# kostas1515/iif

Measured on AMD Instinct MI355X. Metric: images/sec ResNet50+IIF ImageNet-LT bs=256/GPU, higher is better.
Workload: dtype bf16

## Files before the change

iif_amd/_lib.py:

```python
import ctypes
import os

import torch

_HERE = os.path.dirname(os.path.abspath(__file__))
LIB_PATH = os.environ.get("IIF_AMD_LIB") or os.path.join(_HERE, "csrc", "libiif_amd.so")

IIF_F32, IIF_BF16 = 0, 1
VARIANT_CODE = {"raw": 0, "smooth": 1, "rel": 2, "normit": 3, "gombit": 4, "base2": 5, "base10": 6}
_ERR = {-1: "IIF_EINVAL (bad argument)", -2: "IIF_EUNSUPPORTED (shape/alignment)", -3: "IIF_ELAUNCH (HIP error)"}

_c = ctypes
_P, _I, _L, _F = _c.c_void_p, _c.c_int, _c.c_int64, _c.c_float

SIGNATURES = {
    "iif_build_table": [_P, _I, _I, _I, _P],
    "iif_set_cu_budget": [_I],
    "iif_get_cu_budget": [],
    "iif_persistent_grid_blocks": [_I],
    "iif_ce_fwd_bwd": [_P, _I, _L, _P, _P, _P, _F, _P, _P, _L, _F, _I, _I, _P, _P, _P, _L, _P, _P, _P],
    "iif_sigmoid_focal_fwd_bwd": [_P, _I, _L, _P, _P, _F, _P, _F, _I, _F, _F, _I, _I, _P, _P, _P, _L, _P, _P, _P],
    "iif_scale_logits": [_P, _I, _L, _P, _I, _I, _P, _L, _P],
    "iif_softmax": [_P, _I, _L, _P, _I, _I, _P, _L, _P],
    "iif_topk_hits": [_P, _I, _L, _P, _P, _I, _I, _P, _I, _P, _P],
    "iif_eval_accumulate": [_P, _I, _L, _P, _P, _I, _I, _P, _I, _P, _I, _P, _P, _P, _P],
    "iif_scale_by_device_scalar": [_P, _I, _L, _P, _P, _P],
    "iif_mix_rows": [_P, _I, _P, _F, _I, _L, _P, _P],
    "iif_conv_igemm": [_P, _P, _P, _P, _P, _P, _P],
    "iif_conv_wgrad": [_P, _P, _P, _P, _P, _L, _I, _P],
    "iif_conv_wgrad_plan": [_P, _I, _L, _I, _P],
    "iif_conv_igemm_bnstats": [_P, _P, _P, _P, _P, _P, _P, _L, _P, _P],
    "iif_bn_finalize_stats": [_P, _I, _L, _I, _P, _P, _F, _F, _P, _P, _P, _P, _L, _P],
    "iif_bn_finalize_stats_fused": [_P, _I, _L, _I, _P, _P, _F, _F, _P, _P, _P, _P, _L, _P, _P],
    "iif_bn_finalize_stats_sums": [_P, _I, _L, _I, _P, _P, _F, _F, _P, _P, _P, _P, _L, _P, _P, _I, _I, _P, _P],
    "iif_bn_backward_partials_fused": [_P, _P, _P, _I, _L, _I, _P, _P, _P, _I, _P, _P, _P, _P, _L, _P, _P],
    "iif_bn_partial_sums": [_P, _I, _I, _P, _P],
    "iif_bn_stats_sums": [_P, _I, _L, _I, _P, _P, _L, _P],
    "iif_bn_backward_sums": [_P, _P, _P, _P, _I, _L, _I, _P, _P, _P, _L, _P],
    "iif_bn_backward_apply_sums": [_P, _P, _P, _P, _I, _L, _I, _P, _P, _P, _P, _c.c_double, _P, _P, _P, _P, _P, _P],
    "iif_bn_workspace_bytes": [_L, _I],
    "iif_bn_forward_stats": [_P, _I, _L, _I, _P, _P, _F, _F, _P, _P, _P, _P, _L, _P],
    "iif_bn_apply": [_P, _I, _L, _I, _P, _P, _P, _I, _P, _P, _P],
    "iif_bn_backward": [_P, _P, _P, _P, _I, _L, _I, _P, _P, _P, _P, _P, _P, _P, _L, _P],
    "iif_maxpool_forward": [_P, _I, _I, _I, _I, _I, _I, _I, _I, _P, _P, _P],
    "iif_maxpool_backward": [_P, _P, _I, _I, _I, _I, _I, _I, _I, _I, _P, _P],
    "iif_avgpool_forward": [_P, _I, _I, _I, _I, _P, _P],
    "iif_avgpool_backward": [_P, _I, _I, _I, _I, _P, _P],
    "iif_im2col_nchw": [_P, _I, _I, _I, _I, _I, _I, _I, _I, _I, _I, _P, _P],
    "iif_cast": [_P, _I, _P, _I, _L, _P],
    "iif_weight_transpose": [_P, _I, _I, _I, _I, _I, _I, _P, _P],
    "iif_shortcut_a_forward": [_P, _I, _I, _I, _I, _I, _I, _P, _P],
    "iif_shortcut_a_backward_acc": [_P, _I, _I, _I, _I, _I, _I, _P, _P],
    "iif_colsum_f32": [_P, _I, _I, _L, _P, _P],
    "iif_sgd_step": [_P, _P, _P, _L, _F, _P, _F, _F, _I, _F, _P],
    "iif_stream_plan": [_I, _L, _I, _I, _P],
    "iif_rmsprop_step": [_P, _P, _P, _P, _P, _L, _F, _P, _F, _F, _F, _F, _I, _F, _P],
    "iif_group_pack": [_P, _I, _I, _I, _I, _I, _I, _I, _I, _P, _P],
    "iif_group_pack_batched": [_P, _I, _I, _I, _P],
    "iif_wgrad1x1_stacked": [_P, _P, _P, _L, _I, _I, _I, _I, _P, _P, _L, _I, _P],
    "iif_group_unpack_grad": [_P, _I, _I, _I, _I, _I, _I, _P, _P],
    "iif_space_to_depth_nchw": [_P, _I, _I, _I, _I, _I, _I, _P, _P],
    "iif_stem_s2d_pack": [_P, _I, _I, _I, _I, _I, _I, _P, _P],
    "iif_stem_s2d_unpack_grad": [_P, _I, _I, _I, _I, _I, _P, _P],
    "iif_se_squeeze": [_P, _I, _I, _I, _I, _P, _P],
    "iif_se_apply": [_P, _I, _I, _I, _I, _P, _P, _P, _P, _P, _P, _P],
    "iif_se_backward_sums": [_P, _P, _P, _I, _I, _I, _I, _P, _P, _P],
    "iif_se_backward_form": [_P, _I, _I, _I, _I, _P, _P, _P, _P],
    "iif_se_excite_forward": [_P, _P, _I, _I, _I, _I, _P, _I, _P, _I, _P, _P, _P, _P],
    "iif_se_excite_backward": [_P, _P, _P, _I, _I, _I, _I, _P, _I, _P, _I, _P, _P, _P, _P, _P, _P, _P, _I, _P, _I, _P],
    "iif_rownorm_forward": [_P, _P, _I, _I, _L, _F, _F, _F, _P, _L, _P, _P],
    "iif_rownorm_backward": [_P, _P, _P, _P, _I, _I, _L, _L, _F, _F, _F, _P, _L, _P],
    "iif_weight_transpose_batched": [_P, _P, _I, _I, _I, _P, _P],
    "iif_conv_igemm_masked_res": [_P, _P, _P, _P, _P, _P, _P],
    "iif_conv_reload_env": [],
    "iif_conv_igemm_stats_only": [_P, _P, _P, _P, _L, _P, _P],
    "iif_conv_igemm_bn_relu": [_P, _P, _P, _P, _P, _P, _P, _P],
    "iif_conv_fwdbn_ok": [_P],
    "iif_conv_affine_ok": [_P, _I, _I],
    "iif_conv_affine_route": [_P, _I, _I, _I],
    "iif_conv_route": [_P, _c.c_uint, _I, _P, _I],
    "iif_conv_igemm_affine": [_P, _P, _P, _P, _P, _P, _P, _P, _P],
    "iif_bn_fold": [_P, _I, _F, _P],
    "iif_conv_igemm_stats_acc": [_P, _P, _P, _P, _L, _P, _P],
    "iif_conv_igemm_bn_relu2": [_P, _P, _P, _P, _P, _P, _P, _P, _P],
    "iif_conv_igemm_dgrad_masksum": [_P, _P, _P, _P, _P, _P, _P, _P, _P, _P, _L, _P, _P],
    "iif_conv_pro_ok": [_P, _I],
    "iif_conv_igemm_bnstats_pro": [_P, _P, _P, _P, _P, _P, _P, _P, _P, _L, _P, _P],
    "iif_conv_dgrad_rx_ok": [_P, _I],
    "iif_conv_igemm_dgrad_masksum_rx": [_P, _P, _P, _P, _P, _P, _P, _I, _P, _I, _P, _P, _P, _L, _P, _P],
    "iif_conv_dgrad_rx_pg_ok": [_P, _I],
    "iif_conv_igemm_dgrad_masksum_rx_pg": [_P, _P, _P, _P, _P, _P, _P, _I, _P, _I, _P, _P, _P, _L, _P, _P, _L, _I, _P, _P],
    "iif_slab_sum": [_P, _L, _I, _I, _I, _I, _P, _P],
    "iif_conv_igemm_dgrad2_bnbwd": [_P, _P, _P, _I, _P, _P, _P, _P, _P, _P, _P, _L, _P, _P],
    "iif_bn3_algebra_prep": [_P, _I, _P, _I, _P, _I, _P, _P, _I, _I, _L, _P, _P, _P, _P, _I, _P, _P, _L, _P, _P, _P],
    "iif_bn3_algebra_prep_scratch_floats": [_I, _I],
    "iif_bn3_algebra_dw": [_P, _I, _P, _I, _P, _I, _P, _P, _I, _I, _P, _I, _P],
    "iif_conv_pack_fragments": [_P, _P, _I, _I, _P, _P],
    "iif_conv_pack_fragments_g16": [_P, _P, _I, _I, _P, _P],
    "iif_conv3x3_frag_ok": [_P],
    "iif_mask_gather": [_P, _I, _P, _I, _I, _I, _P, _P, _P],
    "iif_mask_bce_fwd_bwd": [_P, _I, _P, _P, _I, _I, _I, _F, _P, _P, _P, _P, _P],
    "iif_class_accumulate": [_P, _P, _I, _I, _P, _P, _P],
    "iif_fasa_update": [_P, _P, _I, _I, _L, _I, _F, _P, _P, _P, _P],
    "iif_fasa_generate": [_P, _P, _P, _P, _P, _P, _I, _I, _P, _P, _P, _P, _P],
    "iif_fasa_update_rows": [_P, _P, _I, _I, _L, _I, _F, _P, _P, _P, _P, _P],
    "iif_fasa_generate_padded": [_P, _P, _P, _P, _P, _P, _I, _I, _I, _F, _P, _P, _P, _P, _P],
    "iif_head_loss_cums_fwd": [_P, _I, _L, _P, _P, _P, _P, _L, _F, _I, _I, _P, _L, _P, _P, _P, _P, _P, _P, _P, _P, _P],
    "iif_conv_igemm_dgrad_bnbwd": [_P, _P, _P, _P, _P, _P, _P, _P, _P, _P, _L, _P, _P],
    "iif_bn_backward_partials": [_P, _P, _P, _I, _L, _I, _P, _P, _P, _I, _P, _P, _P, _P, _L, _P],
    "iif_maxpool_bn_forward": [_P, _I, _P, _I, _I, _I, _I, _I, _I, _I, _P, _P, _P, _P],
    "iif_bn_backward_relu_recompute": [_P, _P, _I, _L, _I, _P, _P, _P, _P, _P, _P, _L, _P],
    "iif_bn_backward_relu_recompute_pooled": [_P, _P, _I, _L, _I, _P, _P, _P, _P, _P, _P, _L, _P, _P, _L, _P],
    "iif_bn_backward_pool_fused": [_P, _P, _P, _P, _I, _I, _I, _I, _I, _I, _I, _P, _P, _P, _P, _P, _P, _L, _P],
    "iif_rowmap_forward": [_P, _I, _I, _I, _L, _I, _F, _F, _P, _I, _L, _P, _P],
    "iif_rowmap_backward": [_P, _I, _P, _P, _I, _I, _I, _L, _L, _I, _F, _F, _P, _I, _L, _P],
    "iif_transpose_f32": [_P, _I, _I, _L, _P, _L, _P],
    "iif_dot_window_f32": [_P, _P, _I, _I, _L, _L, _F, _P, _P, _P],
    "iif_cifar_augment": [_P, _L, _P, _P, _L, _L, _c.c_uint64, _L, _L, _c.c_uint32, _P, _P, _P, _P, _P],
    "iif_lt_augment": [_P, _L, _P, _P, _L, _I, _P, _c.c_uint32, _P, _P],
    "iif_lt_augment_policy": [_P, _L, _P, _P, _L, _I, _P, _P, _P, _P],
    "iif_jpeg_decode": [_P, _L, _P, _L, _P, _L, _P, _L, _I, _P, _P],
    "iif_seesaw_fwd_bwd": [_P, _I, _L, _P, _P, _P, _I, _F, _F, _F, _F, _I, _F, _I, _I, _P, _P, _P, _P, _L, _P, _P, _P],
    "iif_seesaw_activation": [_P, _I, _L, _I, _I, _P, _L, _P],
    "iif_seesaw_accuracy": [_P, _I, _L, _P, _I, _I, _P, _P, _P],
    "iif_seesaw_scale_grad": [_P, _L, _I, _I, _P, _P, _I, _P, _L, _P],
    "iif_bce_det_fwd_bwd": [_P, _I, _L, _P, _P, _L, _P, _P, _P, _F, _I, _I, _P, _P, _P, _L, _P, _P],
    "iif_bbox_reg_fwd": [_P, _I, _L, _P, _I, _I, _P, _P, _F, _F, _L, _I, _P, _P, _P, _P, _P],
    "iif_bbox_reg_scatter_grad": [_P, _P, _I, _I, _I, _P, _P, _I, _L, _P],
    "iif_head_loss_fwd": [_P, _I, _L, _P, _P, _P, _P, _L, _F, _I, _I, _P, _L, _P, _P, _P, _P, _P, _P],
    "iif_head_loss_bwd": [_P, _I, _L, _P, _P, _F, _P, _P],
    "iif_head_bce_loss_fwd": [_P, _I, _L, _P, _P, _P, _L, _F, _I, _I, _P, _L, _P, _P, _P, _P, _P],
    "iif_seesaw_head_fwd": [_P, _I, _L, _P, _P, _P, _F, _F, _F, _F, _I, _I, _P, _L, _P, _P, _P, _P, _P, _P],
    "iif_seesaw_head_bwd": [_P, _L, _I, _I, _P, _P, _P, _F, _P, _L, _P],
    "iif_bbox_overlaps": [_P, _L, _L, _P, _L, _L, _I, _I, _F, _P, _P],
    "iif_max_iou_assign": [_P, _L, _L, _P, _L, _L, _P, _L, _L, _F, _F, _F, _F, _F, _I, _I, _I, _P, _P, _P, _P, _P, _L, _P],
    "iif_bbox2delta": [_P, _L, _P, _L, _L, _P, _P, _P, _P],
    "iif_delta2bbox": [_P, _L, _P, _L, _L, _I, _P, _P, _F, _I, _F, _I, _F, _F, _P, _P],
    "iif_random_sample": [_P, _P, _L, _L, _L, _c.c_double, _P, _P, _P, _P, _P, _L, _P],
    "iif_anchor_targets": [_P, _L, _L, _P, _P, _L, _P, _L, _L, _P, _P, _L, _F, _I, _P, _P, _P, _P, _P, _P, _P],
    "iif_roi_targets": [_P, _L, _L, _P, _P, _P, _L, _L, _P, _P, _P, _L, _L, _I, _L, _F, _I, _P, _P, _P, _P, _P, _P, _P, _P, _P],
    "iif_roi_stage_targets": [_P, _I, _P, _L, _L, _L, _P, _P, _L, _F, _F, _F, _F, _I, _I, _I, _L, _L, _c.c_double, _L, _F, _I, _P, _P,
                              _P, _P, _P, _P, _P, _P, _P, _P, _P, _P, _P, _P],
    "iif_refine_bboxes": [_P, _L, _P, _P, _L, _I, _I, _P, _P, _I, _L, _P, _P, _P, _F, _I, _F, _I, _P, _P, _P],
    "iif_grid_anchors": [_P, _P, _P],
    "iif_grid_valid_flags": [_P, _P, _P, _P],
    "iif_rpn_stage_workspace_bytes": [_I, _L, _L],
    "iif_rpn_stage_targets": [_P, _P, _I, _P, _I, _F, _P, _P, _F, _F, _F, _F, _I, _I, _L, _L, _c.c_double, _P, _P, _P, _P, _P, _P, _P,
                              _P, _P, _L, _P],
    "iif_rpn_stage_dense": [_P, _I, _P, _P, _P, _P, _L, _L, _L, _F, _P, _P, _P, _P, _P],
    "iif_rpn_loss_fwd": [_P, _P, _I, _P, _P, _P, _P, _L, _L, _P, _F, _F, _F, _F, _P, _P, _P],
    "iif_rpn_loss_bwd": [_P, _P, _I, _P, _P, _P, _P, _L, _L, _P, _F, _F, _F, _F, _P, _P, _P],
    "iif_rpn_sampled_pixels": [_P, _I, _P, _P, _P, _P, _L, _L, _P, _P, _P],
    "iif_rpn_head_sampled_workspace_bytes": [_I, _I, _I, _I],
    "iif_rpn_head_sampled_bwd": [_P, _P, _I, _I, _P, _P, _P, _P, _P, _P, _I, _I, _P, _P, _P, _P, _P, _P, _P, _L, _P],
    "iif_roi_extract_forward": [_P, _I, _I, _I, _P, _L, _L, _I, _I, _I, _I, _F, _F, _P, _I, _P, _P],
    "iif_roi_extract_backward": [_P, _I, _I, _I, _P, _L, _L, _I, _I, _I, _I, _F, _F, _P, _I, _P, _L, _P],
    "iif_mask_targets": [_P, _I, _P, _L, _P, _L, _I, _I, _I, _P, _P],
    "iif_paste_masks": [_P, _I, _I, _P, _P, _L, _L, _I, _I, _I, _I, _I, _F, _P, _P],
    "iif_rle_workspace_bytes": [_L, _I, _I],
    "iif_paste_rle_count": [_P, _I, _I, _P, _P, _L, _L, _I, _I, _I, _I, _I, _F, _P, _L, _P, _P],
    "iif_paste_rle_fill": [_P, _I, _I, _P, _P, _L, _L, _I, _I, _I, _I, _I, _F, _P, _L, _P, _L, _P, _P, _P],
    "iif_mask_rle_count": [_P, _L, _L, _L, _I, _I, _P, _L, _P, _P],
    "iif_mask_rle_fill": [_P, _L, _L, _L, _I, _I, _P, _L, _P, _L, _P, _P, _P],
    "iif_rle_to_string": [_P, _L, _P, _L, _P],
    "iif_mask_predict_fwd": [_P, _I, _P, _L, _P, _P, _P, _I, _I, _I, _I, _P, _P, _P, _P, _P, _P],
    "iif_mask_predict_bwd_input": [_P, _P, _P, _L, _P, _I, _I, _I, _I, _P, _I, _P],
    "iif_mask_predict_bwd_weight": [_P, _I, _P, _P, _P, _I, _I, _I, _I, _P, _P, _P, _P],
    "iif_mask_predict_loss_fwd": [_P, _I, _P, _L, _P, _P, _P, _I, _I, _I, _I, _I, _P, _P, _P, _P, _P],
    "iif_mask_predict_loss_bwd_input": [_P, _P, _P, _P, _L, _P, _I, _I, _I, _I, _P, _I, _P],
    "iif_mask_predict_loss_bwd_weight": [_P, _I, _P, _P, _P, _P, _I, _I, _I, _I, _P, _P, _P, _P],
    "iif_normed_mask_predict_fwd": [_P, _I, _P, _L, _P, _P, _P, _I, _I, _I, _I, _F, _F, _F, _I, _P, _P, _P, _P, _P, _P, _P, _P],
    "iif_normed_mask_predict_bwd_input": [_P, _I, _P, _P, _P, _P, _P, _P, _L, _P, _I, _I, _I, _I, _F, _F, _P, _P],
    "iif_normed_mask_predict_bwd_weight": [_P, _I, _P, _P, _P, _P, _P, _L, _P, _I, _I, _I, _I, _F, _F, _P, _P, _P, _P],
    "iif_mask_tail_fwd": [_P, _I, _P, _P, _P, _L, _P, _P, _P, _I, _I, _I, _I, _I, _I, _P, _P, _P, _P, _P, _P],
    "iif_mask_tail_bwd_rows": [_P, _I, _P, _P, _P, _P, _P, _I, _I, _I, _I, _I, _I, _P, _P, _P],
    "iif_mask_tail_bwd_input": [_P, _P, _P, _P, _L, _P, _P, _I, _I, _I, _I, _I, _I, _P, _I, _P],
    "iif_mask_tail_splits": [_I, _I, _I],
    "iif_mask_tail_bwd_params": [_P, _I, _P, _P, _P, _L, _P, _P, _I, _I, _I, _I, _I, _I, _P, _P, _P, _P],
    "iif_mask_tail_bwd_classes": [_P, _P, _I, _I, _I, _P, _P, _P],
    "iif_mask_tail_loss_fwd": [_P, _I, _P, _P, _P, _L, _P, _P, _P, _I, _I, _I, _I, _I, _I, _I, _P, _P, _P, _P, _P],
    "iif_mask_tail_loss_bwd_rows": [_P, _I, _P, _P, _P, _P, _P, _P, _I, _I, _I, _I, _I, _I, _P, _P, _P],
    "iif_mask_tail_loss_bwd_input": [_P, _P, _P, _P, _P, _L, _P, _P, _I, _I, _I, _I, _I, _I, _P, _I, _P],
    "iif_mask_tail_loss_bwd_params": [_P, _I, _P, _P, _P, _P, _L, _P, _P, _I, _I, _I, _I, _I, _I, _P, _P, _P, _P],
    "iif_nms": [_P, _L, _P, _P, _L, _I, _F, _I, _F, _L, _P, _P, _P, _P, _L, _P],
    "iif_rpn_proposals": [_P, _I, _I, _P, _I, _I, _F, _F, _I, _P, _P, _F, _I, _F, _I, _P, _P, _P, _P, _P, _P, _P, _P, _L, _P],
    "iif_multiclass_nms": [_P, _L, _I, _P, _L, _P, _P, _I, _L, _L, _F, _F, _I, _L, _L, _P, _P, _P, _P, _P, _P, _L, _P],
}



class ConvDesc(ctypes.Structure):
    _fields_ = [(k, ctypes.c_int32) for k in ("n", "hs", "ws", "cs", "hd", "wd", "cd", "r", "s", "stride", "pad",
                                               "transposed", "ldw", "dtype", "dst_dtype", "groups")] + [("wgt_frag", ctypes.c_void_p),
                                                                                                          ("wgt_frag_kind", ctypes.c_int32)]


class RoiLevel(ctypes.Structure):
    _fields_ = [("ptr", ctypes.c_void_p), ("H", ctypes.c_int32), ("W", ctypes.c_int32), ("spatial_scale", ctypes.c_float)]


class MaskImage(ctypes.Structure):
    _fields_ = [("ptr", ctypes.c_void_p), ("G", ctypes.c_int32), ("H", ctypes.c_int32), ("W", ctypes.c_int32),
                ("ld_row", ctypes.c_int64), ("ld_mask", ctypes.c_int64)]


class RoiImage(ctypes.Structure):
    _fields_ = [("gt_bboxes", ctypes.c_void_p), ("ld_gt", ctypes.c_int64), ("gt_labels", ctypes.c_void_p), ("G", ctypes.c_int32),
                ("img_index", ctypes.c_int32)]


def roi_images(gt_bboxes_list, gt_labels_list=None):
    B = len(gt_bboxes_list)
    images = (RoiImage * B)()
    held = []
    for b, g in enumerate(gt_bboxes_list):
        G = int(g.shape[0])
        g = g.detach()
        if G and (g.stride(1) != 1 or (G > 1 and g.stride(0) < 4)):
            g = g.contiguous()
        held.append(g)
        l = None
        if gt_labels_list is not None:
            l = gt_labels_list[b].reshape(-1).to(torch.int64).contiguous()
            held.append(l)
        images[b].gt_bboxes = ptr(g) if G else None
        images[b].ld_gt = g.stride(0) if G > 1 else 4
        images[b].gt_labels = ptr(l) if (G and l is not None) else None
        images[b].G = G
        images[b].img_index = b
    return images, held


class RpnGrid(ctypes.Structure):
    _fields_ = [("num_levels", ctypes.c_int32)] + [(k, ctypes.c_int32 * 8) for k in ("W", "H", "num_base", "stride_w", "stride_h")] + [
        ("base", ctypes.c_float * 4 * 16 * 8)]


class RpnLossLevel(ctypes.Structure):
    _fields_ = [(k, ctypes.c_void_p) for k in ("scores", "deltas", "grad_scores", "grad_deltas")] + [
        (k, ctypes.c_int64 * 4) for k in ("score_strides", "delta_strides", "grad_score_strides", "grad_delta_strides")]


class RpnHeadLevel(ctypes.Structure):
    _fields_ = [(k, ctypes.c_void_p) for k in ("feat", "grad_feat", "grad_scores", "grad_deltas")] + [
        (k, ctypes.c_int64 * 4) for k in ("feat_strides", "grad_feat_strides", "grad_score_strides", "grad_delta_strides")]


class RpnLevel(ctypes.Structure):
    _fields_ = [("scores", ctypes.c_void_p), ("deltas", ctypes.c_void_p), ("anchors", ctypes.c_void_p),
                ("score_strides", ctypes.c_int64 * 4), ("delta_strides", ctypes.c_int64 * 4), ("ld_anchors", ctypes.c_int64),
                ("A", ctypes.c_int32), ("H", ctypes.c_int32), ("W", ctypes.c_int32), ("reserved", ctypes.c_int32)]


class PackDesc(ctypes.Structure):
    _fields_ = [("src_off", ctypes.c_int64), ("dst_off", ctypes.c_int64)] + [(k, ctypes.c_int32) for k in (
        "rows", "taps", "k", "ld", "block_start", "reserved")]


_lib = None


class IIFNativeError(RuntimeError):
    pass


def lib():
    global _lib
    if _lib is None:
        if not os.path.exists(LIB_PATH):
            raise IIFNativeError(
                "libiif_amd.so not found at %s — build it with `python -c 'import __graft_entry__ as g; g.build()'` "
                "or `make -C iif_amd/csrc`; iif_amd has no CPU/PyTorch fallback." % LIB_PATH)
        l = ctypes.CDLL(LIB_PATH)
        l.iif_version.restype = _c.c_char_p
        l.iif_version.argtypes = []
        for name, argtypes in SIGNATURES.items():
            fn = getattr(l, name)
            fn.argtypes = argtypes
            fn.restype = _L if name in ("iif_bn_workspace_bytes", "iif_bn3_algebra_prep_scratch_floats", "iif_rle_workspace_bytes",
# ... 44 lines not shown
```

iif_amd/csrc/common.h:

```cpp
#pragma once
#include <hip/hip_runtime.h>
#include <stdint.h>
#include <type_traits>
#include "../../include/iif_amd.h"

#define IIF_WAVE 64

#define IIF_LAUNCH_CHECK()                          \
    do {                                            \
        hipError_t e__ = hipGetLastError();         \
        if (e__ != hipSuccess) return IIF_ELAUNCH;  \
    } while (0)

constexpr long long kDmaRange = 0x7f000000LL;

enum { IIF_ROUTE_NONE = 0, IIF_ROUTE_TILE = 1, IIF_ROUTE_TILE_2STAGE = 2, IIF_ROUTE_TILE_GENERAL = 3, IIF_ROUTE_TILE256 = 4,
       IIF_ROUTE_HALO = 5, IIF_ROUTE_FRAG = 6, IIF_ROUTE_FRAG_G16 = 7, IIF_ROUTE_STREAM1X1 = 8, IIF_ROUTE_REGW1X1 = 9,
       IIF_ROUTE_REGW3X3 = 10, IIF_ROUTE_REGSTAGE = 11, IIF_ROUTE_STEM = 12, IIF_ROUTE_TILE_MC = 13 };

typedef __attribute__((ext_vector_type(4))) float f32x4;
typedef __attribute__((ext_vector_type(4))) unsigned int u32x4;
typedef __attribute__((ext_vector_type(2))) unsigned int u32x2;
typedef __attribute__((ext_vector_type(8))) short s16x8;
typedef __attribute__((ext_vector_type(8))) __bf16 bf16x8;
// ... 13 lines not shown
__device__ __forceinline__ float wave_max(float v) {
#pragma unroll
    for (int o = 32; o > 0; o >>= 1) v = fmaxf(v, __shfl_xor(v, o, 64));
    return v;
}
__device__ __forceinline__ float wave_sum(float v) {
#pragma unroll
    for (int o = 32; o > 0; o >>= 1) v += __shfl_xor(v, o, 64);
    return v;
}
__device__ __forceinline__ int wave_sum_i(int v) {
#pragma unroll
    for (int o = 32; o > 0; o >>= 1) v += __shfl_xor(v, o, 64);
    return v;
}

static inline hipStream_t as_stream(void* s) { return (hipStream_t)s; }
static inline int64_t cdiv64(int64_t a, int64_t b) { return (a + b - 1) / b; }
static inline bool aligned(const void* p, int a) { return (reinterpret_cast<uintptr_t>(p) % a) == 0; }
static inline bool aligned_to(const void* p, unsigned n) { return aligned(p, (int)n); }


struct ConvCall {
    const iif_conv_desc* d; const void* src; const void* wgt; void* dst; const void* res; const unsigned char* res_bits; const float* bias;
    float* bn_partial; int64_t bn_cap; int32_t* n_partials; void* stream;
    const void* bw_x; const unsigned char* bw_bits; const float* bw_stats;
    int mask_store; const void* src2; int cs2; const float* sbias; int no_store;
    const float* aff; const float* aff2; unsigned char* relu_out;
    int aff_any;
    const void* rx_src2; const void* rx_w3; int rx_k2, rx_ldw3;
    const float* pro_stats; void* pro_out; unsigned char* pro_bits; float* pro_csum;
    float* pg_slab; long long pg_cap; int pg_ld; int* pg_count;
};

struct ConvSel {
    int N, Hs, Ws, Cs, Hd, Wd, Cd, R, S, sshift, pad, transposed, ldw, M, groups, spitch, dpitch, Cs2, esz;
    bool outf32;
    long long src_bytes, wgt_bytes;
    bool res, res_bits, bias, bn_partial, bw_x, bw_bits, bw_stats, src2, sbias, aff, aff2, relu_out, rx_src2, rx_w3, pro_stats, pg_slab,
         pg_count, wfrag;
    bool res_is_dst, pg_unaligned;
    int mask_store, no_store, wfrag_kind, rx_k2, rx_ldw3, pg_ld, bn_row0;
    long long bn_cap, pg_cap;
    int ntaps, in_shift, scatter;
};

struct ConvRoute {
    int family;
    int inst;
    int cls;
    int mtiles, ntiles;
    unsigned grid, grid_y, block;
    int rows, slabs;
};

inline int iif_claim_rows(const ConvSel& a, ConvRoute* r, int rows) {
    r->rows = 0;
    if (!a.bn_partial) return IIF_OK;
    if ((long long)(a.bn_row0 + rows) * 2 * a.dpitch > a.bn_cap) return IIF_EINVAL;
    r->rows = rows;
    return IIF_OK;
}


bool iif_stem4x4_geometry(const ConvSel& a);
int iif_stem4x4_select(const ConvSel& a, ConvRoute* r);
int iif_stem4x4_launch(const ConvRoute& r, const ConvCall& c, const ConvSel& a, hipStream_t st);

enum { IIF_REGW_PLAIN = 0, IIF_REGW_FWDBN = 2, IIF_REGW_STATS = 3 };
bool iif_dense1x1(const ConvSel& a);
bool iif_regw1x1_ok(int M, int K, int N, int epi);
bool iif_regw1x1_rx_ok(int M, int K, int N, int k2);
bool iif_regw1x1_pg_ok(int M, int K, int N, int k2);
bool iif_regw1x1_pro_ok(int M, int K, int N);
bool iif_regw1x1_fwdbn_ok(int M, int K, int N);
int iif_regw1x1_select(const ConvSel& a, int mode, ConvRoute* r);
int iif_regw1x1_launch(const ConvRoute& r, const ConvCall& c, const ConvSel& a, hipStream_t st);
int iif_regw3x3_select(const ConvSel& a, ConvRoute* r);
int iif_regw3x3_launch(const ConvRoute& r, const ConvCall& c, const ConvSel& a, const signed char* tap_dy, const signed char* tap_dx,
                       const unsigned char* tap_w, hipStream_t st);

struct ConvSwitches {
    bool no_stream, force_stream, regstage, no_v2, no_halo, force_halo, v2_force, no_regw, no_regw_fwdbn, no_bm256_2src,
         regw_k512_cw16, regw_no_x2, regw_k512_no_epi;
    static ConvSwitches read();
};
extern ConvSwitches g_sw;

int iif_persistent_cus();
int iif_persistent_grid(int unit);
```

iif_amd/csrc/conv_igemm.hip:

```cpp
#include <stdlib.h>

#include "common.h"
#ifndef IIF_CONV_AUX_SRC
#define IIF_CONV_AUX_SRC 0
#endif

namespace {

template <typename T> struct ET;
template <> struct ET<unsigned short> { static constexpr int PE = 8, KE = 32; };
template <> struct ET<float> { static constexpr int PE = 4, KE = 16; };

struct ConvArgs {
    const unsigned char* src; const unsigned char* wgt; unsigned char* dst; const unsigned char* res;
    const unsigned char* wfrag;
    int wfrag_kind;
    const float* bias;
    const unsigned char* res_bits;
    const unsigned char* bw_x; const unsigned char* bw_bits; const float* bw_stats;
    int mask_store;
    const unsigned char* src2; int Cs2;
    const float* sbias;
    const unsigned char* rx_src2; const unsigned char* rx_w3; int rx_k2, rx_ldw3;
    float* pg_slab; long long pg_cap; int pg_ld; int* pg_count;
// ... 1853 lines not shown
    if (d->n <= 0 || d->hs <= 0 || d->ws <= 0 || d->cs <= 0 || d->hd <= 0 || d->wd <= 0 || d->cd <= 0 ||
        d->r <= 0 || d->s <= 0 || d->pad < 0)
        return IIF_EINVAL;
    if (d->stride != 1 && d->stride != 2) return IIF_EUNSUPPORTED;
    if (d->dtype != IIF_F32 && d->dtype != IIF_BF16) return IIF_EINVAL;
    if (d->dst_dtype != d->dtype && d->dst_dtype != IIF_F32) return IIF_EINVAL;
    const int pe = d->dtype == IIF_F32 ? 4 : 8;
    if (d->cs % pe != 0 || d->ldw % pe != 0 || d->ldw < d->r * d->s * d->cs + (a->src2 ? a->Cs2 : 0)) return IIF_EUNSUPPORTED;
    const bool bf16 = d->dtype == IIF_BF16 && d->dst_dtype == IIF_BF16;
    if (aff_any) {
        if (!affine_geometry_ok(d) || a->bias || a->bn_partial || a->res_bits || a->bw_x) return IIF_EUNSUPPORTED;
    } else if (a->src2 || a->sbias || a->mask_store || a->no_store || a->aff || a->pro_stats) {
        if (!bf16 || d->r != 1 || d->s != 1 || d->stride != 1 || d->pad != 0 || d->groups > 1 || (d->cd % 8) || a->bias || (d->cs % 32))
            return IIF_EUNSUPPORTED;
        if (a->src2 && ((a->Cs2 % 32) || a->Cs2 <= 0 || src2_unaligned)) return IIF_EUNSUPPORTED;
        if (a->mask_store && (!a->bw_bits || !a->bn_partial)) return IIF_EINVAL;
        if (a->no_store && (!a->bn_partial || a->res || a->bw_x)) return IIF_EINVAL;
        if (a->aff && (a->bn_partial || a->res_bits || a->bw_x || a->no_store)) return IIF_EINVAL;
    }
    if (unaligned) return IIF_EUNSUPPORTED;
    if ((int64_t)d->n * d->hd * d->wd > 0x7fffff00LL || (int64_t)d->n * d->hs * d->ws > 0x7fffff00LL) return IIF_EUNSUPPORTED;
    sel_geometry(d, a);
    if (a->bn_partial && !(bf16 && (d->cd % 8) == 0 && !a->bias && (a->bw_x || a->mask_store || !a->res) && !g_sw.regstage &&
                           a->src_bytes < kDmaRange))
        return IIF_EUNSUPPORTED;
    if (a->groups > 65535) return IIF_EUNSUPPORTED;
    return select_conv(*a, p);
}

ConvSel sel_of(const ConvCall& c) {
    ConvSel a{};
    a.res = c.res; a.res_bits = c.res_bits; a.bias = c.bias; a.bn_partial = c.bn_partial;
    a.bw_x = c.bn_partial && c.bw_x; a.bw_bits = c.bn_partial && c.bw_bits; a.bw_stats = c.bn_partial && c.bw_stats;
    a.src2 = c.src2; a.sbias = c.sbias; a.aff = c.aff; a.aff2 = c.aff2; a.relu_out = c.relu_out;
    a.rx_src2 = c.rx_src2; a.rx_w3 = c.rx_w3; a.pro_stats = c.pro_stats; a.pg_slab = c.pg_slab; a.pg_count = c.pg_count;
    a.res_is_dst = c.res == c.dst; a.pg_unaligned = reinterpret_cast<uintptr_t>(c.pg_slab) & 15;
    a.mask_store = c.mask_store; a.no_store = c.no_store; a.Cs2 = c.cs2; a.rx_k2 = c.rx_k2; a.rx_ldw3 = c.rx_ldw3; a.pg_ld = c.pg_ld;
    a.bn_cap = c.bn_cap; a.pg_cap = c.pg_cap;
    return a;
}

int conv_entry(const ConvCall& c) {
    const iif_conv_desc* d = c.d;
    if (!d || !c.src || !c.wgt || !c.dst) return IIF_EINVAL;
    if (c.n_partials) *c.n_partials = 0;
    if (c.pg_count) *c.pg_count = 0;
    ConvSel s = sel_of(c);
    ConvPlan p;
    const bool unaligned = (reinterpret_cast<uintptr_t>(c.src) | reinterpret_cast<uintptr_t>(c.wgt) | reinterpret_cast<uintptr_t>(c.dst) |
                            reinterpret_cast<uintptr_t>(c.res)) & 15;
    if (const int rc = conv_select(d, &s, unaligned, reinterpret_cast<uintptr_t>(c.src2) & 15, c.aff_any, &p)) return rc;
    hipStream_t st = as_stream(c.stream);
    for (int i = 0; i < p.n; ++i) {
        const ConvRoute& r = p.r[i];
        const int rc = d->dtype == IIF_BF16 ? (s.outf32 ? launch_route<unsigned short, true>(c, s, r, st)
                                                        : launch_route<unsigned short, false>(c, s, r, st))
                                            : launch_route<float, true>(c, s, r, st);
        if (rc != IIF_OK) return rc;
        s.bn_row0 += r.rows;
        if (c.n_partials) *c.n_partials = s.bn_row0;
        if (c.pg_count) *c.pg_count = r.slabs;
    }
    return IIF_OK;
}

}

ConvSwitches g_sw = ConvSwitches::read();
ConvSwitches ConvSwitches::read() {
    ConvSwitches c;
    c.no_stream = getenv("IIF_CONV_NO_STREAM1X1") != nullptr;
    c.force_stream = getenv("IIF_CONV_STREAM1X1_FORCE") != nullptr;
    c.regstage = getenv("IIF_CONV_REGSTAGE") != nullptr;
    c.no_v2 = getenv("IIF_CONV_NO_V2") != nullptr;
    c.no_halo = getenv("IIF_CONV_NO_HALO") != nullptr;
    c.v2_force = getenv("IIF_CONV_V2_FORCE") != nullptr;
    c.force_halo = getenv("IIF_CONV_HALO_FORCE") != nullptr;
    c.no_regw = getenv("IIF_CONV_NO_REGW") != nullptr;
    c.no_regw_fwdbn = getenv("IIF_CONV_NO_REGW_FWDBN") != nullptr;
    c.no_bm256_2src = getenv("IIF_CONV_NO_BM256_2SRC") != nullptr;
    c.regw_k512_cw16 = getenv("IIF_REGW_K512_CW16") != nullptr;
    c.regw_no_x2 = getenv("IIF_REGW_NO_X2") != nullptr;
    c.regw_k512_no_epi = getenv("IIF_REGW_K512_NO_EPI") != nullptr;
    return c;
}

extern "C" int iif_conv_pack_fragments(const void* src_base, const iif_pack_desc* table, int n_desc, int total_blocks,
                                       void* dst_base, void* stream) {
    if (!src_base || !table || !dst_base || n_desc <= 0 || total_blocks <= 0) return IIF_EINVAL;
    if ((reinterpret_cast<uintptr_t>(src_base) | reinterpret_cast<uintptr_t>(dst_base)) & 15) return IIF_EUNSUPPORTED;
    hipLaunchKernelGGL(pack_fragments_kernel, dim3((unsigned)total_blocks), dim3(256), 0, as_stream(stream),
                       (const unsigned short*)src_base, table, n_desc, (unsigned short*)dst_base);
    IIF_LAUNCH_CHECK();
    return IIF_OK;
}

extern "C" int iif_conv_pack_fragments_g16(const void* src_base, const iif_pack_desc* table, int n_desc, int total_blocks,
                                           void* dst_base, void* stream) {
    if (!src_base || !table || !dst_base || n_desc <= 0 || total_blocks <= 0) return IIF_EINVAL;
    if ((reinterpret_cast<uintptr_t>(src_base) | reinterpret_cast<uintptr_t>(dst_base)) & 15) return IIF_EUNSUPPORTED;
    hipLaunchKernelGGL(pack_fragments_g16_kernel, dim3((unsigned)total_blocks), dim3(256), 0, as_stream(stream),
                       (const unsigned short*)src_base, table, n_desc, (unsigned short*)dst_base);
    IIF_LAUNCH_CHECK();
    return IIF_OK;
}

extern "C" int iif_conv_reload_env(void) {
    g_sw = ConvSwitches::read();
    return IIF_OK;
}

namespace {
bool query_dense1x1(const iif_conv_desc* d, int transposed, ConvSel* a) {
    if (!d || d->dtype != IIF_BF16 || d->dst_dtype != IIF_BF16) return false;
    *a = ConvSel{};
    sel_geometry(d, a);
    return iif_dense1x1(*a) && a->transposed == transposed;
}
}

extern "C" int iif_conv3x3_frag_ok(const iif_conv_desc* d) {
    if (!d || g_sw.no_v2 || g_sw.regstage) return 0;
    if (d->dtype != IIF_BF16 || d->dst_dtype != IIF_BF16 || d->r != 3 || d->s != 3 || d->stride != 1 || d->pad != 1) return 0;
    if (d->hs != d->hd || d->ws != d->wd) return 0;
    const int g = d->groups > 1 ? d->groups : 1;
    if (g > 1 && (d->cs != 64 || d->cd != 64)) return 0;
    if ((int64_t)d->n * d->hs * d->ws * d->cs * g * 2 >= kDmaRange) return 0;
    return v2_geometry_ok(d->n, d->hd, d->wd, d->cs, d->cd, g) ? 1 : 0;
}

extern "C" int iif_conv_dgrad_rx_ok(const iif_conv_desc* d, int c2) {
    ConvSel a;
    return query_dense1x1(d, 1, &a) && iif_regw1x1_rx_ok(a.M, a.Cs, a.Cd, c2) ? 1 : 0;
}

extern "C" int iif_conv_dgrad_rx_pg_ok(const iif_conv_desc* d, int c2) {
    ConvSel a;
    return query_dense1x1(d, 1, &a) && iif_regw1x1_pg_ok(a.M, a.Cs, a.Cd, c2) ? 1 : 0;
}

extern "C" int iif_conv_fwdbn_ok(const iif_conv_desc* d) {
    ConvSel a;
    return query_dense1x1(d, 0, &a) && !g_sw.no_regw_fwdbn && iif_regw1x1_fwdbn_ok(a.M, a.Cs, a.Cd) ? 1 : 0;
}

extern "C" int iif_conv_pro_ok(const iif_conv_desc* d, int stats_only) {
    ConvSel a;
    if (!query_dense1x1(d, 0, &a)) return 0;
    return (stats_only ? (!g_sw.no_regw_fwdbn && iif_regw1x1_fwdbn_ok(a.M, a.Cs, a.Cd)) : iif_regw1x1_pro_ok(a.M, a.Cs, a.Cd)) ? 1 : 0;
}

extern "C" int iif_conv_affine_ok(const iif_conv_desc* d, int has_res, int has_res_affine) {
    if (has_res_affine && !has_res) return 0;
    return affine_geometry_ok(d) ? 1 : 0;
}

extern "C" int iif_conv_affine_route(const iif_conv_desc* d, int has_res, int has_res_affine, int has_relu_bits) {
    if (!iif_conv_affine_ok(d, has_res, has_res_affine)) return IIF_ROUTE_NONE;
    ConvSel a{};
    a.aff = true; a.res = has_res; a.aff2 = has_res_affine; a.relu_out = has_relu_bits;
    ConvPlan p;
    return conv_select(d, &a, false, false, 1, &p) == IIF_OK ? p.r[0].family : IIF_ROUTE_NONE;
}

extern "C" int iif_conv_route(const iif_conv_desc* d, unsigned operands, int cs2, int32_t* out, int cap) {
    if (!d || cap < 0 || (cap > 0 && !out)) return IIF_EINVAL;
// ... 201 lines not shown
```

iif_amd/csrc/conv_wgrad.hip:

```cpp
#include <stdlib.h>
#include <type_traits>

#include "common.h"
#include "wgrad_plan.h"
#ifndef IIF_WG_AUX_X
#define IIF_WG_AUX_X 0
#endif
#ifndef IIF_WG_AUX_Y
#define IIF_WG_AUX_Y 0
#endif

namespace {

struct WgArgs {
    const unsigned char* x; const unsigned char* dy; float* out;
    int N, Hs, Ws, Cs, Hd, Wd, Cd, R, S, sshift, pad, ldw, M, K;
    int ktiles, ntiles, steps_per_split, nsteps, nsplits;
    int xpitch, ypitch, groups;
    int64_t slab;
};

template <typename T> struct WT;
template <> struct WT<unsigned short> {
    static constexpr int PE = 8, ROWS = 32;
// ... 139 lines not shown
                const unsigned char* base = Y + (4 * g + q) * PY + (wk * (BC / 2) + kj * 16 + 4 * p) * 2;
                yp[kj].lo = tr_read(base); yp[kj].hi = tr_read(base + 16 * PY);
            }
            tr_fence<0>();
#pragma unroll
            for (int ni = 0; ni < 4; ++ni) xf[ni] = tr_join(xp[ni]);
#pragma unroll
            for (int kj = 0; kj < KJ; ++kj) yf[kj] = tr_join(yp[kj]);
#pragma unroll
            for (int ni = 0; ni < 4; ++ni)
#pragma unroll
                for (int kj = 0; kj < KJ; ++kj)
                    acc[ni][kj] = __builtin_amdgcn_mfma_f32_16x16x32_bf16(
                        __builtin_bit_cast(bf16x8, xf[ni]), __builtin_bit_cast(bf16x8, yf[kj]), acc[ni][kj], 0, 0, 0);
        } else {
#pragma unroll
            for (int qq = 0; qq < 4; ++qq) {
                float xf[4], yf[KJ];
#pragma unroll
                for (int ni = 0; ni < 4; ++ni)
                    xf[ni] = *reinterpret_cast<const float*>(X + (4 * qq + g) * PX + (wn * 64 + ni * 16 + li) * 4);
#pragma unroll
                for (int kj = 0; kj < KJ; ++kj)
                    yf[kj] = *reinterpret_cast<const float*>(Y + (4 * qq + g) * PY + (wk * (BC / 2) + kj * 16 + li) * 4);
#pragma unroll
                for (int ni = 0; ni < 4; ++ni)
#pragma unroll
                    for (int kj = 0; kj < KJ; ++kj)
                        acc[ni][kj] = __builtin_amdgcn_mfma_f32_16x16x4f32(xf[ni], yf[kj], acc[ni][kj], 0, 0, 0);
            }
        }
        if (more) store_step((step + 1 - step0) & 1);
        __syncthreads();
    }

    float* out = a.out + (int64_t)split * a.slab;
#pragma unroll
    for (int kj = 0; kj < KJ; ++kj) {
        const int k = k0 + wk * (BC / 2) + kj * 16 + li;
        if (k >= a.Cd) continue;
#pragma unroll
        for (int ni = 0; ni < 4; ++ni) {
            const int n = n0 + wn * 64 + ni * 16 + g * 4;
            if (n >= a.K) continue;
            *reinterpret_cast<f32x4*>(out + (int64_t)k * a.ldw + n) = acc[ni][kj];
        }
    }
}

typedef __attribute__((address_space(3))) void lds_void_w;

#ifdef IIF_CONV_STAMPS
__device__ unsigned long long* g_wstamps = nullptr;
#define IIF_WSTAMP(var)                                                                            \
    do {                                                                                           \
        __builtin_amdgcn_sched_barrier(0);                                                         \
        asm volatile("s_memtime %0\n\ts_waitcnt lgkmcnt(0)" : "=s"(var)::"memory");               \
        __builtin_amdgcn_sched_barrier(0);                                                         \
    } while (0)
#endif

template <typename T, int COLS> struct Swz {
    static constexpr int RB = COLS * (int)sizeof(T);
    static __device__ __forceinline__ int logical(int p, int row) {
        if constexpr (sizeof(T) == 2) {
            const int key = RB >= 256 ? (row & 7) : ((row >> 1) & 3);
            return (((p >> 1) ^ key) << 1) | (p & 1);
        } else {
            return (((p >> 2) ^ (row & 1)) << 2) | (p & 3);
        }
    }
    static __device__ __forceinline__ int addr(int row, int colb) {
        if constexpr (sizeof(T) == 2) {
            const int key = RB >= 256 ? (row & 7) : ((row >> 1) & 3);
            return row * RB + ((((colb >> 5) ^ key)) << 5) + (colb & 31);
        } else {
            return row * RB + ((((colb >> 6) ^ (row & 1))) << 6) + (colb & 63);
        }
    }
};

template <int N> __device__ __forceinline__ void wait_vmcnt() { asm volatile("s_waitcnt vmcnt(%0)" ::"n"(N) : "memory"); }

template <typename T, int BC, int WK = 2, int NST = 3>
__global__ void __launch_bounds__(128 * WK) conv_wgrad_dma_kernel(WgArgs a, unsigned x_bytes, unsigned dy_bytes) {
    constexpr int PE = WT<T>::PE, ROWS = WT<T>::ROWS;
    constexpr int BNW = 128;
    constexpr int NWV = 2 * WK;
    constexpr int CW = BC / WK;
    using SX = Swz<T, BNW>;
    using SY = Swz<T, BC>;
    constexpr int XB = ROWS * SX::RB, YB = ROWS * SY::RB, STAGE = XB + YB;
    constexpr int LPRX = SX::RB / 16, RPIX = 64 / LPRX, NIX = ROWS / RPIX / NWV;
    constexpr int LPRY = SY::RB / 16, RPIY = 64 / LPRY, NIY = ROWS / RPIY / NWV;
    constexpr int LPS = NIX + NIY;
    constexpr int KJ = CW / 16;
    constexpr unsigned OOB = 0xfffffff0u;
    static_assert((NIX == 1 || NIX == 2) && (NIY == 1 || NIY == 2), "tile geometry");
    static_assert(NST >= 3 && NST <= 7 && (NST - 2) * LPS <= 63, "ring depth");
    __shared__ __attribute__((aligned(1024))) unsigned char smem[NST * STAGE];

    const int tid = threadIdx.x, lane = tid & 63;
    const int wave = __builtin_amdgcn_readfirstlane(tid >> 6);
    const int wn = wave / WK, wk = wave % WK;
    const int tiles = a.ktiles * a.ntiles;
    const int xcd = blockIdx.x & 7, jj = blockIdx.x >> 3;
    const int split = (jj / tiles) * 8 + xcd, tile = jj % tiles;
    if (split >= a.nsplits) return;
    const int kt = tile % a.ktiles, ntile = tile / a.ktiles;
    const int k0 = kt * BC, n0 = ntile * BNW;
    const int step0 = split * a.steps_per_split;
    int step1 = step0 + a.steps_per_split;
    if (step1 > a.nsteps) step1 = a.nsteps;

    const auto rs_x = __builtin_amdgcn_make_buffer_rsrc(const_cast<unsigned char*>(a.x), 0, x_bytes, 0x00020000);
    const auto rs_y = __builtin_amdgcn_make_buffer_rsrc(const_cast<unsigned char*>(a.dy), 0, dy_bytes, 0x00020000);
    const int grp = blockIdx.y;
    const unsigned gx = (unsigned)(grp * a.Cs) * (unsigned)sizeof(T), gy = (unsigned)(grp * a.Cd) * (unsigned)sizeof(T);

    int xr[NIX], py[NIX], px[NIX], pb[NIX], pm[NIX], ttr[NIX], tts[NIX], tch[NIX];
    bool nval[NIX];
    const int HW = a.Hd * a.Wd, HWs = a.Hs * a.Ws;
#pragma unroll
    for (int i = 0; i < NIX; ++i) {
        xr[i] = RPIX * (NIX * wave + i) + lane / LPRX;
        const int lc = SX::logical(lane % LPRX, xr[i]);
        const int ncol = n0 + lc * PE;
        nval[i] = ncol < a.K;
        const int tap = ncol / a.Cs;
        tch[i] = ncol - tap * a.Cs;
        ttr[i] = tap / a.S; tts[i] = tap - ttr[i] * a.S;
        const int m = step0 * ROWS + xr[i];
        pm[i] = m;
        const int n = m / HW, rem = m - n * HW;
        py[i] = rem / a.Wd; px[i] = rem - py[i] * a.Wd; pb[i] = n * HWs;
    }
    int yr[NIY];
    unsigned ycol[NIY];
#pragma unroll
    for (int i = 0; i < NIY; ++i) {
        yr[i] = RPIY * (NIY * wave + i) + lane / LPRY;
        const int lc = SY::logical(lane % LPRY, yr[i]);
        const int kcol = k0 + lc * PE;
        ycol[i] = kcol < a.Cd ? (unsigned)kcol * (unsigned)sizeof(T) : OOB;
    }

    auto issue = [&](int stage, int step) {
        unsigned char* X = smem + stage * STAGE;
        unsigned char* Y = X + XB;
#pragma unroll
        for (int i = 0; i < NIX; ++i) {
            const int ys = (py[i] << a.sshift) - a.pad + ttr[i], xs = (px[i] << a.sshift) - a.pad + tts[i];
            const bool ok = nval[i] && pm[i] < a.M && (unsigned)ys < (unsigned)a.Hs && (unsigned)xs < (unsigned)a.Ws;
            const unsigned off = ok ? ((unsigned)(pb[i] + ys * a.Ws + xs) * (unsigned)a.xpitch + (unsigned)tch[i]) * (unsigned)sizeof(T) + gx : OOB;
            __builtin_amdgcn_raw_ptr_buffer_load_lds(rs_x, (lds_void_w*)(X + (NIX * wave + i) * 1024), 16, off, 0, 0, IIF_WG_AUX_X);
        }
#pragma unroll
        for (int i = 0; i < NIY; ++i) {
            const int m = step * ROWS + yr[i];
            const unsigned off = (ycol[i] != OOB && m < a.M) ? (unsigned)m * (unsigned)a.ypitch * (unsigned)sizeof(T) + ycol[i] + gy : OOB;
            __builtin_amdgcn_raw_ptr_buffer_load_lds(rs_y, (lds_void_w*)(Y + (NIY * wave + i) * 1024), 16, off, 0, 0, IIF_WG_AUX_Y);
        }
    };
    auto advance = [&]() {
#pragma unroll
        for (int i = 0; i < NIX; ++i) {
            pm[i] += ROWS;
            px[i] += ROWS;
            while (px[i] >= a.Wd) {
                px[i] -= a.Wd;
                if (++py[i] == a.Hd) { py[i] = 0; pb[i] += HWs; }
            }
        }
    };

    f32x4 acc[4][KJ];
#pragma unroll
    for (int ni = 0; ni < 4; ++ni)
#pragma unroll
        for (int kj = 0; kj < KJ; ++kj) acc[ni][kj] = f32x4{0.f, 0.f, 0.f, 0.f};

    const int g = lane >> 4, li = lane & 15;
    const int nst = step1 - step0;
#pragma unroll
    for (int s_ = 0; s_ < NST - 1; ++s_)
        if (s_ < nst) {
            if (s_ > 0) advance();
            issue(s_, step0 + s_);
        }
    int stage = 0;
#ifdef IIF_CONV_STAMPS
    unsigned long long w_wait = 0, w_issue = 0, w_rest = 0, w0, w1, w2, w3, wb;
    IIF_WSTAMP(wb); w3 = wb;
#endif
    for (int t = 0; t < nst; ++t) {
#ifdef IIF_CONV_STAMPS
        IIF_WSTAMP(w0); w_rest += w0 - w3;
#endif
        {
            const int rem = nst - 1 - t;
            if (rem >= NST - 2) wait_vmcnt<(NST - 2) * LPS>();
            else if (NST > 3 && rem == 1) wait_vmcnt<LPS>();
            else if (NST > 4 && rem == 2) wait_vmcnt<2 * LPS>();
            else if (NST > 5 && rem == 3) wait_vmcnt<3 * LPS>();
            else if (NST > 6 && rem == 4) wait_vmcnt<4 * LPS>();
            else wait_vmcnt<0>();
        }
        __builtin_amdgcn_s_barrier();
#ifdef IIF_CONV_STAMPS
        IIF_WSTAMP(w1);
#endif
        if (t + NST - 1 < nst) { advance(); issue(stage == 0 ? NST - 1 : stage - 1, step0 + t + NST - 1); }
#ifdef IIF_CONV_STAMPS
        IIF_WSTAMP(w2); w_wait += w1 - w0; w_issue += w2 - w1; w3 = w2;
#endif
        const unsigned char* X = smem + stage * STAGE;
        const unsigned char* Y = X + XB;
        if constexpr (sizeof(T) == 2) {
            const int q = li >> 2, p = li & 3;
            TrPair xp[4], yp[KJ];
            s16x8 yf[KJ];
#pragma unroll
            for (int kj = 0; kj < KJ; ++kj) {
                const int colb = (wk * CW + kj * 16 + 4 * p) * 2;
                yp[kj].lo = tr_read(Y + SY::addr(4 * g + q, colb)); yp[kj].hi = tr_read(Y + SY::addr(16 + 4 * g + q, colb));
            }
#pragma unroll
            for (int ni = 0; ni < 4; ++ni) {
                const int colb = (wn * 64 + ni * 16 + 4 * p) * 2;
                xp[ni].lo = tr_read(X + SX::addr(4 * g + q, colb)); xp[ni].hi = tr_read(X + SX::addr(16 + 4 * g + q, colb));
            }
#pragma unroll
            for (int ni = 0; ni < 4; ++ni) {
                if (ni == 0) tr_fence<6>(); else if (ni == 1) tr_fence<4>(); else if (ni == 2) tr_fence<2>(); else tr_fence<0>();
                if (ni == 0) {
#pragma unroll
                    for (int kj = 0; kj < KJ; ++kj) yf[kj] = tr_join(yp[kj]);
                }
                const s16x8 xf = tr_join(xp[ni]);
#pragma unroll
                for (int kj = 0; kj < KJ; ++kj)
                    acc[ni][kj] = __builtin_amdgcn_mfma_f32_16x16x32_bf16(
                        __builtin_bit_cast(bf16x8, xf), __builtin_bit_cast(bf16x8, yf[kj]), acc[ni][kj], 0, 0, 0);
            }
        } else {
#pragma unroll
            for (int qq = 0; qq < 4; ++qq) {
                float xf[4], yf[KJ];
#pragma unroll
                for (int ni = 0; ni < 4; ++ni)
                    xf[ni] = *reinterpret_cast<const float*>(X + SX::addr(4 * qq + g, (wn * 64 + ni * 16 + li) * 4));
#pragma unroll
                for (int kj = 0; kj < KJ; ++kj)
                    yf[kj] = *reinterpret_cast<const float*>(Y + SY::addr(4 * qq + g, (wk * CW + kj * 16 + li) * 4));
#pragma unroll
                for (int ni = 0; ni < 4; ++ni)
#pragma unroll
                    for (int kj = 0; kj < KJ; ++kj)
                        acc[ni][kj] = __builtin_amdgcn_mfma_f32_16x16x4f32(xf[ni], yf[kj], acc[ni][kj], 0, 0, 0);
            }
        }
        stage = stage == NST - 1 ? 0 : stage + 1;
    }

#ifdef IIF_CONV_STAMPS
    IIF_WSTAMP(w0); w_rest += w0 - w3;
    if (g_wstamps && blockIdx.x < 512 && lane == 0 && wave < 4) {
        unsigned long long* o = g_wstamps + ((int64_t)blockIdx.x * 4 + wave) * 8;
        o[0] = w_wait; o[1] = 0; o[2] = w_issue; o[3] = w_rest; o[4] = 0; o[5] = w0 - wb; o[6] = (unsigned long long)nst; o[7] = wb;
    }
#endif
    float* out = a.out + (int64_t)split * a.slab + (int64_t)grp * a.Cd * a.ldw;
#pragma unroll
    for (int kj = 0; kj < KJ; ++kj) {
        const int k = k0 + wk * CW + kj * 16 + li;
        if (k >= a.Cd) continue;
#pragma unroll
        for (int ni = 0; ni < 4; ++ni) {
            const int n = n0 + wn * 64 + ni * 16 + g * 4;
            if (n >= a.K) continue;
            *reinterpret_cast<f32x4*>(out + (int64_t)k * a.ldw + n) = acc[ni][kj];
        }
    }
}

struct W1Args {
    const unsigned char* x; const unsigned char* dy; float* out;
    int M, Cs, Cd, ldw, ktiles, ntiles, steps_per_split, nsteps, nsplits;
    int64_t slab;
    const unsigned char* dy2; int Cd1, Cd2;
};

template <int OFF> __device__ __forceinline__ s16x4 tr_read_at(unsigned a) {
    s16x4 v;
    asm volatile("ds_read_b64_tr_b16 %0, %1 offset:%2" : "=v"(v) : "v"(a), "n"(OFF) : "memory");
    return v;
}

template <int BC, int BNW, int NWV>
__device__ __forceinline__ void wgrad1x1_body(const W1Args& a, unsigned x_bytes, unsigned dy_bytes) {
    constexpr int NWN = BNW / 64, WK = NWV / NWN, CW = BC / WK, KJ = CW / 16;
    using SX = Swz<unsigned short, BNW>;
    using SY = Swz<unsigned short, BC>;
    constexpr int RBX = SX::RB, RBY = SY::RB;
    constexpr int XB = 32 * RBX, YB = 32 * RBY, STAGE = XB + YB;
    constexpr int NPX = XB / 1024, NPY = YB / 1024;
    constexpr bool YPAD = NPY < NWV;
    constexpr int NIX = NPX / NWV, NIY = YPAD ? 1 : NPY / NWV, LPS = NIX + NIY;
    constexpr int LPRX = RBX / 16, RPIX = 64 / LPRX, LPRY = RBY / 16, RPIY = 64 / LPRY;
    constexpr unsigned OOB = 0xfffffff0u;
    static_assert(NIX >= 1 && NIY >= 1 && NIX * NWV == NPX && (YPAD || NIY * NWV == NPY) && KJ >= 1, "tile geometry");
    static_assert(2 * STAGE + 16 * RBY < 65536 && 2 * STAGE + 16 * RBX < 65536, "fragment reads use 16-bit immediates");
    __shared__ __attribute__((aligned(1024))) unsigned char smem[3 * STAGE + (YPAD ? 1024 : 0)];

    const int tid = threadIdx.x, lane = tid & 63;
    const int wave = __builtin_amdgcn_readfirstlane(tid >> 6);
    const int wn = wave / WK, wk = wave % WK;
    const int tiles = a.ktiles * a.ntiles;
    const int xcd = blockIdx.x & 7, jj = blockIdx.x >> 3;
    const int split = (jj / tiles) * 8 + xcd, tile = jj % tiles;
    if (split >= a.nsplits) return;
    const int k0 = (tile % a.ktiles) * BC, n0 = (tile / a.ktiles) * BNW;
    const int step0 = split * a.steps_per_split;
    int step1 = step0 + a.steps_per_split;
    if (step1 > a.nsteps) step1 = a.nsteps;
    const int nst = step1 - step0;

    const auto rs_x = __builtin_amdgcn_make_buffer_rsrc(const_cast<unsigned char*>(a.x), 0, x_bytes, 0x00020000);
    const bool second = a.dy2 != nullptr && k0 >= a.Cd1;
    const int ycols = a.dy2 == nullptr ? a.Cd : (second ? a.Cd2 : a.Cd1);
    const int yk0 = second ? k0 - a.Cd1 : k0;
    const auto rs_y = __builtin_amdgcn_make_buffer_rsrc(const_cast<unsigned char*>(second ? a.dy2 : a.dy), 0,
                                                        second ? (unsigned)a.M * (unsigned)a.Cd2 * 2u : dy_bytes, 0x00020000);

    unsigned offx[NIX], incx[NIX], offy[NIY], incy[NIY];
#pragma unroll
    for (int i = 0; i < NIX; ++i) {
        const int r = RPIX * (NIX * wave + i) + lane / LPRX;
        const int col = n0 + SX::logical(lane % LPRX, r) * 8;
        const bool ok = col < a.Cs;
        offx[i] = ok ? ((unsigned)(step0 * 32 + r) * (unsigned)a.Cs + (unsigned)col) * 2u : OOB;
        incx[i] = ok ? 64u * (unsigned)a.Cs : 0u;
    }
#pragma unroll
    for (int i = 0; i < NIY; ++i) {
        const int r = RPIY * (NIY * wave + i) + lane / LPRY;
        const int col = yk0 + SY::logical(lane % LPRY, r) * 8;
        const bool ok = col < ycols && (!YPAD || wave < NPY);
        offy[i] = ok ? ((unsigned)(step0 * 32 + r) * (unsigned)ycols + (unsigned)col) * 2u : OOB;
        incy[i] = ok ? 64u * (unsigned)ycols : 0u;
    }
    auto issue = [&](auto stage_c) {
        constexpr int S = decltype(stage_c)::value;
#pragma unroll
        for (int i = 0; i < NIX; ++i) {
            __builtin_amdgcn_raw_ptr_buffer_load_lds(rs_x, (lds_void_w*)(smem + S * STAGE + (NIX * wave + i) * 1024), 16, offx[i], 0, 0, IIF_WG_AUX_X);
            offx[i] += incx[i];
        }
#pragma unroll
        for (int i = 0; i < NIY; ++i) {
            unsigned char* dst = smem + S * STAGE + XB + (NIY * wave + i) * 1024;
            if (YPAD && wave >= NPY) dst = smem + 3 * STAGE;
            __builtin_amdgcn_raw_ptr_buffer_load_lds(rs_y, (lds_void_w*)dst, 16, offy[i], 0, 0, IIF_WG_AUX_Y);
            offy[i] += incy[i];
        }
    };

    const int g = lane >> 4, li = lane & 15, q = li >> 2, pp = li & 3;
    unsigned xo[4], yo[KJ];
    const unsigned sbase = (unsigned)(unsigned long long)(lds_cu8*)smem;
#pragma unroll
    for (int ni = 0; ni < 4; ++ni) xo[ni] = sbase + (unsigned)SX::addr(4 * g + q, (wn * 64 + ni * 16 + 4 * pp) * 2);
#pragma unroll
    for (int kj = 0; kj < KJ; ++kj) yo[kj] = sbase + (unsigned)(XB + SY::addr(4 * g + q, (wk * CW + kj * 16 + 4 * pp) * 2));

    f32x4 acc[4][KJ];
#pragma unroll
    for (int ni = 0; ni < 4; ++ni)
#pragma unroll
        for (int kj = 0; kj < KJ; ++kj) acc[ni][kj] = f32x4{0.f, 0.f, 0.f, 0.f};

    using S0 = std::integral_constant<int, 0>;
    using S1 = std::integral_constant<int, 1>;
    using S2 = std::integral_constant<int, 2>;
    auto step = [&](auto stage_c, auto refill_c, int t) {
        constexpr int S = decltype(stage_c)::value;
        if (t + 1 < nst) wait_vmcnt<LPS>(); else wait_vmcnt<0>();
        __builtin_amdgcn_s_barrier();
        if (t + 2 < nst) issue(refill_c);
        TrPair xp[4], yp[KJ];
        s16x8 yf[KJ];
#pragma unroll
        for (int kj = 0; kj < KJ; ++kj) {
            yp[kj].lo = tr_read_at<S * STAGE>(yo[kj]); yp[kj].hi = tr_read_at<S * STAGE + 16 * RBY>(yo[kj]);
        }
#pragma unroll
        for (int ni = 0; ni < 4; ++ni) {
            xp[ni].lo = tr_read_at<S * STAGE>(xo[ni]); xp[ni].hi = tr_read_at<S * STAGE + 16 * RBX>(xo[ni]);
        }
#pragma unroll
        for (int ni = 0; ni < 4; ++ni) {
            if (ni == 0) tr_fence<6>(); else if (ni == 1) tr_fence<4>(); else if (ni == 2) tr_fence<2>(); else tr_fence<0>();
            if (ni == 0) {
#pragma unroll
                for (int kj = 0; kj < KJ; ++kj) yf[kj] = tr_join(yp[kj]);
            }
            const s16x8 xf = tr_join(xp[ni]);
#pragma unroll
            for (int kj = 0; kj < KJ; ++kj)
                acc[ni][kj] = __builtin_amdgcn_mfma_f32_16x16x32_bf16(__builtin_bit_cast(bf16x8, xf), __builtin_bit_cast(bf16x8, yf[kj]),
                                                                      acc[ni][kj], 0, 0, 0);
        }
    };
    if (nst > 0) issue(S0{});
    if (nst > 1) issue(S1{});
    for (int t = 0; t < nst; t += 3) {
        step(S0{}, S2{}, t);
        if (t + 1 < nst) step(S1{}, S0{}, t + 1);
        if (t + 2 < nst) step(S2{}, S1{}, t + 2);
    }

    float* out = a.out + (int64_t)split * a.slab;
#pragma unroll
    for (int kj = 0; kj < KJ; ++kj) {
        const int k = k0 + wk * CW + kj * 16 + li;
        if (k >= a.Cd) continue;
#pragma unroll
        for (int ni = 0; ni < 4; ++ni) {
            const int n = n0 + wn * 64 + ni * 16 + g * 4;
            if (n >= a.Cs) continue;
            *reinterpret_cast<f32x4*>(out + (int64_t)k * a.ldw + n) = acc[ni][kj];
        }
    }
}

__global__ void __launch_bounds__(512) wgrad1x1_256x128_kernel(W1Args a, unsigned xb, unsigned yb) { wgrad1x1_body<256, 128, 8>(a, xb, yb); }
__global__ void __launch_bounds__(256) wgrad1x1_128x128_kernel(W1Args a, unsigned xb, unsigned yb) { wgrad1x1_body<128, 128, 4>(a, xb, yb); }
__global__ void __launch_bounds__(256) wgrad1x1_64x128_kernel(W1Args a, unsigned xb, unsigned yb) { wgrad1x1_body<64, 128, 4>(a, xb, yb); }
__global__ void __launch_bounds__(256) wgrad1x1_64x64_kernel(W1Args a, unsigned xb, unsigned yb) { wgrad1x1_body<64, 64, 4>(a, xb, yb); }
__global__ void __launch_bounds__(512) wgrad1x1_64x256_kernel(W1Args a, unsigned xb, unsigned yb) { wgrad1x1_body<64, 256, 8>(a, xb, yb); }

struct WgHaloArgs {
    const unsigned char* x; const unsigned char* dy; float* out;
    int N, H, W, Cs, Cd, ldw;
    int ci_tiles, co_tiles, steps_per_split, nsteps, nsplits, HB;
    int grouped;
    int64_t slab;
};

template <int XB, int YB, int D>
__global__ void __launch_bounds__(256) conv3x3_wgrad_halo_kernel(WgHaloArgs a, unsigned x_bytes, unsigned dy_bytes) {
    constexpr int RB = 128;
    constexpr int XR = 32 * XB, YR = 32 * YB;
    constexpr unsigned OOB = 0xfffffff0u;
    using SW = Swz<unsigned short, 64>;
    __shared__ __attribute__((aligned(1024))) unsigned char smem[(XR + YR) * RB];
    unsigned char* const XS = smem;
    unsigned char* const YS = smem + XR * RB;

    const int tid = threadIdx.x, lane = tid & 63;
    const int wave = __builtin_amdgcn_readfirstlane(tid >> 6);
    const int tiles = a.ci_tiles * a.co_tiles;
    const int xcd = blockIdx.x & 7, jj = blockIdx.x >> 3;
    const int split = (jj / tiles) * 8 + xcd, tile = jj % tiles;
    if (split >= a.nsplits) return;
    const int ci0 = a.grouped ? tile * 64 : (tile % a.ci_tiles) * 64, co0 = a.grouped ? tile * 64 : (tile / a.ci_tiles) * 64;
    const int step0 = split * a.steps_per_split;
    int step1 = step0 + a.steps_per_split;
    if (step1 > a.nsteps) step1 = a.nsteps;
    const int nst = step1 - step0;
    const int Wp = a.W + 2, PV = (a.H + 2) * Wp, HW = a.H * a.W;
    const int V0 = step0 * 32, LEAD = a.HB >> 4;

    const auto rs_x = __builtin_amdgcn_make_buffer_rsrc(const_cast<unsigned char*>(a.x), 0, x_bytes, 0x00020000);
    const auto rs_y = __builtin_amdgcn_make_buffer_rsrc(const_cast<unsigned char*>(a.dy), 0, dy_bytes, 0x00020000);

    const int lrow = 8 * wave + (lane >> 3);
    struct Cur { int n, yp, xp; };
    auto start = [&](int v) {
        Cur c; const int t = v + PV; c.n = t / PV - 1; const int rem = t - (c.n + 1) * PV; c.yp = rem / Wp; c.xp = rem - c.yp * Wp;
        return c;
    };
    auto advance = [&](Cur& c) {
        c.xp += 32;
        while (c.xp >= Wp) { c.xp -= Wp; if (++c.yp == a.H + 2) { c.yp = 0; ++c.n; } }
    };
    Cur cx = start(V0 - a.HB + lrow), cy = start(V0 + lrow);
    int xblk = 0, yblk = 0;
    auto issue_x = [&]() {
        const int prow = (xblk * 32 + lrow) & (XR - 1);
        const int lc = SW::logical(lane & 7, prow);
        const bool ok = (unsigned)cx.n < (unsigned)a.N && (unsigned)(cx.yp - 1) < (unsigned)a.H && (unsigned)(cx.xp - 1) < (unsigned)a.W;
        const unsigned off = ok ? ((unsigned)(cx.n * HW + (cx.yp - 1) * a.W + cx.xp - 1) * (unsigned)a.Cs + (unsigned)(ci0 + lc * 8)) * 2u : OOB;
        __builtin_amdgcn_raw_ptr_buffer_load_lds(rs_x, (lds_void_w*)(XS + ((xblk * 32 + 8 * wave) & (XR - 1)) * RB), 16, off, 0, 0, IIF_WG_AUX_X);
        advance(cx); ++xblk;
    };
    auto issue_y = [&]() {
        const int prow = (yblk * 32 + lrow) & (YR - 1);
        const int lc = SW::logical(lane & 7, prow);
        const bool ok = (unsigned)cy.n < (unsigned)a.N && (unsigned)(cy.yp - 1) < (unsigned)a.H && (unsigned)(cy.xp - 1) < (unsigned)a.W;
        const unsigned off = ok ? ((unsigned)(cy.n * HW + (cy.yp - 1) * a.W + cy.xp - 1) * (unsigned)a.Cd + (unsigned)(co0 + lc * 8)) * 2u : OOB;
        __builtin_amdgcn_raw_ptr_buffer_load_lds(rs_y, (lds_void_w*)(YS + ((yblk * 32 + 8 * wave) & (YR - 1)) * RB), 16, off, 0, 0, IIF_WG_AUX_Y);
        advance(cy); ++yblk;
    };

    f32x4 acc[9][4];
#pragma unroll
    for (int t = 0; t < 9; ++t)
#pragma unroll
        for (int kj = 0; kj < 4; ++kj) acc[t][kj] = f32x4{0.f, 0.f, 0.f, 0.f};

    for (int j = 0; j < LEAD; ++j) issue_x();
#pragma unroll
    for (int j = 0; j < D; ++j) { issue_x(); issue_y(); }

    const int g = lane >> 4, li = lane & 15, q = li >> 2, p = li & 3;
    int xo[9], yo[4];
#pragma unroll
    for (int tap = 0; tap < 9; ++tap)
        xo[tap] = SW::addr((a.HB + 4 * g + q + (tap / 3 - 1) * Wp + (tap % 3 - 1)) & (XR - 1), (16 * wave + 4 * p) * 2);
#pragma unroll
    for (int kj = 0; kj < 4; ++kj) yo[kj] = SW::addr(4 * g + q, (16 * kj + 4 * p) * 2);
#ifdef IIF_CONV_STAMPS
    unsigned long long w_wait = 0, w_issue = 0, w_rest = 0, w0, w1, w2, w3, wb;
    IIF_WSTAMP(wb); w3 = wb;
#endif
    for (int t = 0; t < nst; ++t) {
#ifdef IIF_CONV_STAMPS
        IIF_WSTAMP(w0); w_rest += w0 - w3;
#endif
        asm volatile("s_waitcnt vmcnt(%0)" ::"n"(2 * (D - 1)) : "memory");
        __builtin_amdgcn_s_barrier();
#ifdef IIF_CONV_STAMPS
        IIF_WSTAMP(w1);
#endif
        issue_x(); issue_y();
#ifdef IIF_CONV_STAMPS
        IIF_WSTAMP(w2); w_wait += w1 - w0; w_issue += w2 - w1; w3 = w2;
#endif
        const int xs = t * (32 * RB), ys = t * (32 * RB);
        TrPair yp[4], xp[9];
        s16x8 yf[4];
#pragma unroll
        for (int kj = 0; kj < 4; ++kj) {
            yp[kj].lo = tr_read(YS + ((yo[kj] + ys) & (YR * RB - 1))); yp[kj].hi = tr_read(YS + ((yo[kj] + ys + 16 * RB) & (YR * RB - 1)));
        }
#pragma unroll
        for (int tap = 0; tap < 9; ++tap) {
            xp[tap].lo = tr_read(XS + ((xo[tap] + xs) & (XR * RB - 1))); xp[tap].hi = tr_read(XS + ((xo[tap] + xs + 16 * RB) & (XR * RB - 1)));
        }
#pragma unroll
        for (int tap = 0; tap < 9; ++tap) {
            if (tap == 0) tr_fence<15>(); else if (tap == 1) tr_fence<14>(); else if (tap == 2) tr_fence<12>();
            else if (tap == 3) tr_fence<10>(); else if (tap == 4) tr_fence<8>(); else if (tap == 5) tr_fence<6>();
            else if (tap == 6) tr_fence<4>(); else if (tap == 7) tr_fence<2>(); else tr_fence<0>();
            if (tap == 0) {
#pragma unroll
                for (int kj = 0; kj < 4; ++kj) yf[kj] = tr_join(yp[kj]);
            }
            const s16x8 xf = tr_join(xp[tap]);
#pragma unroll
            for (int kj = 0; kj < 4; ++kj)
                acc[tap][kj] = __builtin_amdgcn_mfma_f32_16x16x32_bf16(__builtin_bit_cast(bf16x8, xf), __builtin_bit_cast(bf16x8, yf[kj]),
                                                                        acc[tap][kj], 0, 0, 0);
        }
    }
    asm volatile("s_waitcnt vmcnt(0)" ::: "memory");
#ifdef IIF_CONV_STAMPS
    IIF_WSTAMP(w0); w_rest += w0 - w3;
    if (g_wstamps && blockIdx.x < 512 && lane == 0 && wave < 4) {
        unsigned long long* o = g_wstamps + ((int64_t)blockIdx.x * 4 + wave) * 8;
        o[0] = w_wait; o[1] = 0; o[2] = w_issue; o[3] = w_rest; o[4] = 0; o[5] = w0 - wb; o[6] = (unsigned long long)nst; o[7] = wb;
    }
#endif

    float* out = a.out + (int64_t)split * a.slab;
#pragma unroll
    for (int kj = 0; kj < 4; ++kj) {
        const int k = co0 + kj * 16 + li;
#pragma unroll
        for (int tap = 0; tap < 9; ++tap) {
            const int n = a.grouped ? tap * 64 + wave * 16 + g * 4 : tap * a.Cs + ci0 + wave * 16 + g * 4;
            *reinterpret_cast<f32x4*>(out + (int64_t)k * a.ldw + n) = acc[tap][kj];
        }
    }
}

struct WgStemArgs {
    const unsigned char* x; const unsigned char* dy; float* out;
    int N, H, W, ldw, steps_per_split, nsteps, nsplits, LB, LEAD;
    int64_t slab;
};

__global__ void __launch_bounds__(256) conv4x4_s2d_wgrad_kernel(WgStemArgs a, unsigned x_bytes, unsigned dy_bytes) {
    constexpr int XRB = 32, YRB = 128;
    constexpr int XR = 512, YR = 128;
    constexpr int D = 2;
    constexpr unsigned OOB = 0xfffffff0u;
    using SW = Swz<unsigned short, 64>;
    __shared__ __attribute__((aligned(1024))) unsigned char smem[XR * XRB + YR * YRB];
    unsigned char* const XS = smem;
    unsigned char* const YS = smem + XR * XRB;

    const int tid = threadIdx.x, lane = tid & 63;
    const int wave = __builtin_amdgcn_readfirstlane(tid >> 6);
    const int xcd = blockIdx.x & 7, jj = blockIdx.x >> 3;
    const int split = jj * 8 + xcd;
    if (split >= a.nsplits) return;
    const int step0 = split * a.steps_per_split;
    int step1 = step0 + a.steps_per_split;
    if (step1 > a.nsteps) step1 = a.nsteps;
    const int nst = step1 - step0;
    const int Wp = a.W + 3, Hp = a.H + 3, PV = Hp * Wp, HW = a.H * a.W;
    const int V0 = step0 * 32;

    const auto rs_x = __builtin_amdgcn_make_buffer_rsrc(const_cast<unsigned char*>(a.x), 0, x_bytes, 0x00020000);
    const auto rs_y = __builtin_amdgcn_make_buffer_rsrc(const_cast<unsigned char*>(a.dy), 0, dy_bytes, 0x00020000);

    struct Cur { int n, yp, xp; };
    auto start = [&](int v) {
        const int t = v + 32 * PV;
        Cur c; c.n = t / PV - 32; const int rem = t - (c.n + 32) * PV; c.yp = rem / Wp; c.xp = rem - c.yp * Wp;
        return c;
    };
    auto advance = [&](Cur& c) {
        c.xp += 32;
        while (c.xp >= Wp) { c.xp -= Wp; if (++c.yp == Hp) { c.yp = 0; ++c.n; } }
    };
    const int xrow = lane >> 1, yrow = 8 * wave + (lane >> 3);
    Cur cx = start(V0 - 32 * a.LB + xrow), cy = start(V0 + yrow);
    int xblk = 0, yblk = 0;
    auto issue_x = [&]() {
        const bool ok = (unsigned)cx.n < (unsigned)a.N && (unsigned)(cx.yp - 2) < (unsigned)a.H && (unsigned)(cx.xp - 2) < (unsigned)a.W;
        const unsigned off = ok ? ((unsigned)(cx.n * HW + (cx.yp - 2) * a.W + cx.xp - 2) * 16u + (unsigned)((lane & 1) * 8)) * 2u : OOB;
        __builtin_amdgcn_raw_ptr_buffer_load_lds(rs_x, (lds_void_w*)(XS + ((xblk * 32) & (XR - 1)) * XRB), 16, off, 0, 0, IIF_WG_AUX_X);
        advance(cx); ++xblk;
    };
    auto issue_y = [&]() {
        const int prow = (yblk * 32 + yrow) & (YR - 1);
        const int lc = SW::logical(lane & 7, prow);
        const bool ok = (unsigned)cy.n < (unsigned)a.N && (unsigned)(cy.yp - 2) < (unsigned)a.H && (unsigned)(cy.xp - 2) < (unsigned)a.W;
        const unsigned off = ok ? ((unsigned)(cy.n * HW + (cy.yp - 2) * a.W + cy.xp - 2) * 64u + (unsigned)(lc * 8)) * 2u : OOB;
        __builtin_amdgcn_raw_ptr_buffer_load_lds(rs_y, (lds_void_w*)(YS + ((yblk * 32 + 8 * wave) & (YR - 1)) * YRB), 16, off, 0, 0, IIF_WG_AUX_Y);
        advance(cy); ++yblk;
    };

    f32x4 acc[4][4];
#pragma unroll
    for (int t = 0; t < 4; ++t)
#pragma unroll
        for (int kj = 0; kj < 4; ++kj) acc[t][kj] = f32x4{0.f, 0.f, 0.f, 0.f};

    if (wave == 0) for (int j = 0; j < a.LEAD; ++j) issue_x();
#pragma unroll
    for (int j = 0; j < D; ++j) { if (wave == 0) issue_x(); issue_y(); }

    const int g = lane >> 4, li = lane & 15, q = li >> 2, p = li & 3;
    int xo[4], yo[4];
#pragma unroll
    for (int s_ = 0; s_ < 4; ++s_)
        xo[s_] = ((32 * a.LB + 4 * g + q + (wave - 2) * Wp + (s_ - 2)) & (XR - 1)) * XRB + 4 * p * 2;
#pragma unroll
    for (int kj = 0; kj < 4; ++kj) yo[kj] = SW::addr(4 * g + q, (16 * kj + 4 * p) * 2);
    for (int t = 0; t < nst; ++t) {
        if (wave == 0) asm volatile("s_waitcnt vmcnt(%0)" ::"n"(2 * (D - 1)) : "memory");
        else asm volatile("s_waitcnt vmcnt(%0)" ::"n"(D - 1) : "memory");
        __builtin_amdgcn_s_barrier();
        if (wave == 0) issue_x();
        issue_y();
        const int xs = t * (32 * XRB), ys = t * (32 * YRB);
        TrPair yp[4], xp[4];
        s16x8 yf[4];
#pragma unroll
        for (int kj = 0; kj < 4; ++kj) {
            yp[kj].lo = tr_read(YS + ((yo[kj] + ys) & (YR * YRB - 1))); yp[kj].hi = tr_read(YS + ((yo[kj] + ys + 16 * YRB) & (YR * YRB - 1)));
        }
#pragma unroll
        for (int s_ = 0; s_ < 4; ++s_) {
            xp[s_].lo = tr_read(XS + ((xo[s_] + xs) & (XR * XRB - 1))); xp[s_].hi = tr_read(XS + ((xo[s_] + xs + 16 * XRB) & (XR * XRB - 1)));
        }
#pragma unroll
        for (int s_ = 0; s_ < 4; ++s_) {
            if (s_ == 0) tr_fence<6>(); else if (s_ == 1) tr_fence<4>(); else if (s_ == 2) tr_fence<2>(); else tr_fence<0>();
            if (s_ == 0) {
#pragma unroll
                for (int kj = 0; kj < 4; ++kj) yf[kj] = tr_join(yp[kj]);
            }
            const s16x8 xf = tr_join(xp[s_]);
#pragma unroll
            for (int kj = 0; kj < 4; ++kj)
                acc[s_][kj] = __builtin_amdgcn_mfma_f32_16x16x32_bf16(__builtin_bit_cast(bf16x8, xf), __builtin_bit_cast(bf16x8, yf[kj]),
                                                                       acc[s_][kj], 0, 0, 0);
        }
    }
    asm volatile("s_waitcnt vmcnt(0)" ::: "memory");

    float* out = a.out + (int64_t)split * a.slab;
#pragma unroll
    for (int kj = 0; kj < 4; ++kj) {
        const int k = kj * 16 + li;
#pragma unroll
        for (int s_ = 0; s_ < 4; ++s_) {
            const int n = (wave * 4 + s_) * 16 + g * 4;
            *reinterpret_cast<f32x4*>(out + (int64_t)k * a.ldw + n) = acc[s_][kj];
        }
    }
}

#ifdef IIF_NT_SLABS
#define IIF_SLAB_LD(p) __builtin_nontemporal_load(reinterpret_cast<const f32x4*>(p))
#else
#define IIF_SLAB_LD(p) (*reinterpret_cast<const f32x4*>(p))
#endif
__global__ void __launch_bounds__(256) wgrad_reduce_kernel(const float* ws, int splits, int chunk, int64_t slab, int Cd,
                                                           int ldw, int K, float* out, int64_t out_stride) {
    const int64_t total4 = (int64_t)Cd * ldw / 4;
    const int s0 = blockIdx.y * chunk;
    int s1 = s0 + chunk; if (s1 > splits) s1 = splits;
    float* dst = out + (int64_t)blockIdx.y * out_stride;
    for (int64_t i = (int64_t)blockIdx.x * 256 + threadIdx.x; i < total4; i += (int64_t)gridDim.x * 256) {
        const int64_t e = i * 4;
        const int n = (int)(e % ldw);
        if (n >= K) continue;
        f32x4 s = f32x4{0.f, 0.f, 0.f, 0.f};
        for (int j = s0; j < s1; j += 16) {
            f32x4 t[16];
#pragma unroll
            for (int q = 0; q < 16; ++q) t[q] = IIF_SLAB_LD(ws + (int64_t)(j + q < s1 ? j + q : s0) * slab + e);
#pragma unroll
            for (int q = 0; q < 16; ++q) {
                const f32x4 u = s + t[q];
                if (j + q < s1) s = (j + q == s0) ? t[q] : u;
            }
        }
        *reinterpret_cast<f32x4*>(dst + e) = s;
    }
}

using iif_plan::WgPlan;
using iif_plan::WgShape;

inline int reduce_slabs(float* ws, int64_t ws_bytes, int splits, int64_t slab, int rows, int ldw, int K, float* dw, hipStream_t st) {
    const iif_plan::ReducePlan r = iif_plan::reduce_plan(splits, slab, ws_bytes);
    const int blocks = r.blocks;
    if (r.stages == 2) {
        const int chunk = 16, nch = r.nch;
        float* stage = ws + (int64_t)splits * slab;
        hipLaunchKernelGGL(wgrad_reduce_kernel, dim3(blocks, nch), dim3(256), 0, st, ws, splits, chunk, slab, rows, ldw, K, stage, slab);
        IIF_LAUNCH_CHECK();
        hipLaunchKernelGGL(wgrad_reduce_kernel, dim3(blocks, 1), dim3(256), 0, st, stage, nch, nch, slab, rows, ldw, K, dw, (int64_t)0);
        IIF_LAUNCH_CHECK();
        return IIF_OK;
    }
    hipLaunchKernelGGL(wgrad_reduce_kernel, dim3(blocks, 1), dim3(256), 0, st, ws, splits, splits, slab, rows, ldw, K, dw, (int64_t)0);
    IIF_LAUNCH_CHECK();
    return IIF_OK;
}

inline WgShape shape_of(const WgArgs& a, int esz, int64_t x_bytes, int64_t dy_bytes, bool stacked = false, int cd2 = 0) {
    WgShape s{};
    s.N = a.N; s.Hs = a.Hs; s.Ws = a.Ws; s.Cs = a.Cs; s.Hd = a.Hd; s.Wd = a.Wd; s.Cd = a.Cd; s.R = a.R; s.S = a.S;
    s.sshift = a.sshift; s.pad = a.pad; s.ldw = a.ldw; s.M = a.M; s.K = a.K; s.groups = a.groups; s.xpitch = a.xpitch;
    s.ypitch = a.ypitch; s.esz = esz; s.cd2 = cd2; s.stacked = stacked; s.gram = a.x == a.dy && !stacked;
    s.x_bytes = x_bytes; s.dy_bytes = dy_bytes;
    return s;
}

inline int launch_wgrad_halo(const WgArgs& a, const WgPlan& p, float* dw, float* ws, int64_t ws_bytes, int64_t x_bytes,
                             int64_t dy_bytes, hipStream_t st) {
    WgHaloArgs h{};
    h.x = a.x; h.dy = a.dy; h.N = a.N; h.H = a.Hd; h.W = a.Wd; h.Cs = a.xpitch; h.Cd = a.ypitch; h.ldw = a.ldw;
    h.grouped = a.groups > 1;
    h.ci_tiles = p.ntiles; h.co_tiles = p.ktiles;
    h.HB = p.HB;
    h.nsteps = p.nsteps;
    const int splits = p.splits;
    h.steps_per_split = p.steps_per_split;
    h.slab = splits > 1 ? p.slab : 0;
    h.out = splits > 1 ? ws : dw;
    h.nsplits = splits;
    const dim3 grid((unsigned)p.blocks);
    hipLaunchKernelGGL((conv3x3_wgrad_halo_kernel<8, 4, 2>), grid, dim3(256), 0, st, h, (unsigned)x_bytes, (unsigned)dy_bytes);
    IIF_LAUNCH_CHECK();
    if (splits > 1) return reduce_slabs(ws, ws_bytes, splits, p.slab, p.rows, a.ldw, a.K, dw, st);
    return IIF_OK;
}

inline int launch_wgrad_stem(const WgArgs& a, const WgPlan& p, float* dw, float* ws, int64_t ws_bytes, int64_t x_bytes,
                             int64_t dy_bytes, hipStream_t st) {
    WgStemArgs h{};
    h.x = a.x; h.dy = a.dy; h.N = a.N; h.H = a.Hd; h.W = a.Wd; h.ldw = a.ldw;
    h.LB = p.LB;
    h.LEAD = p.LEAD;
    h.nsteps = p.nsteps;
    const int splits = p.splits;
    h.steps_per_split = p.steps_per_split;
    h.slab = splits > 1 ? p.slab : 0;
    h.out = splits > 1 ? ws : dw;
    h.nsplits = splits;
    hipLaunchKernelGGL(conv4x4_s2d_wgrad_kernel, dim3((unsigned)p.blocks), dim3(256), 0, st, h, (unsigned)x_bytes,
                       (unsigned)dy_bytes);
    IIF_LAUNCH_CHECK();
    if (splits > 1) return reduce_slabs(ws, ws_bytes, splits, p.slab, p.rows, a.ldw, a.K, dw, st);
    return IIF_OK;
}

inline int launch_wgrad_1x1(const WgArgs& g, const WgPlan& p, float* dw, float* ws, int64_t ws_bytes, int64_t x_bytes, int64_t dy_bytes,
                            hipStream_t st, const unsigned char* dy2 = nullptr, int cd2 = 0) {
    W1Args a{};
    a.x = g.x; a.dy = g.dy; a.M = g.M; a.Cs = g.Cs; a.Cd = g.Cd; a.ldw = g.ldw;
    a.dy2 = dy2; a.Cd1 = dy2 ? g.Cd - cd2 : g.Cd; a.Cd2 = cd2;
    const int bc = p.bc, bnw = p.bnw;
    a.ktiles = p.ktiles;
    a.ntiles = p.ntiles;
    a.nsteps = p.nsteps;
    const int splits = p.splits;
    const int64_t slab = p.slab;
    a.steps_per_split = p.steps_per_split;
    a.slab = splits > 1 ? slab : 0;
    a.out = splits > 1 ? ws : dw;
    a.nsplits = splits;
    const dim3 grid((unsigned)p.blocks);
    const unsigned xb = (unsigned)x_bytes, yb = (unsigned)dy_bytes;
    if (bc == 256) hipLaunchKernelGGL(wgrad1x1_256x128_kernel, grid, dim3(512), 0, st, a, xb, yb);
    else if (bc == 128) hipLaunchKernelGGL(wgrad1x1_128x128_kernel, grid, dim3(256), 0, st, a, xb, yb);
    else if (bnw == 256) hipLaunchKernelGGL(wgrad1x1_64x256_kernel, grid, dim3(512), 0, st, a, xb, yb);
    else if (bnw == 128) hipLaunchKernelGGL(wgrad1x1_64x128_kernel, grid, dim3(256), 0, st, a, xb, yb);
    else hipLaunchKernelGGL(wgrad1x1_64x64_kernel, grid, dim3(256), 0, st, a, xb, yb);
    IIF_LAUNCH_CHECK();
    if (splits > 1) return reduce_slabs(ws, ws_bytes, splits, slab, g.Cd, g.ldw, g.Cs, dw, st);
    return IIF_OK;
}

template <typename T>
int launch_wgrad(WgArgs a, float* dw, float* ws, int64_t ws_bytes, int splits_req, int64_t x_bytes, int64_t dy_bytes,
                 hipStream_t st) {
    if (!ws) ws_bytes = 0;
    const WgPlan p = iif_plan::wgrad_plan(shape_of(a, (int)sizeof(T), x_bytes, dy_bytes), ws_bytes, splits_req);
    if (p.rc != IIF_OK) return p.rc;
    if constexpr (sizeof(T) == 2) {
        if (p.family == IIF_WGRAD_NINETAP) return launch_wgrad_halo(a, p, dw, ws, ws_bytes, x_bytes, dy_bytes, st);
        if (p.family == IIF_WGRAD_STEM) return launch_wgrad_stem(a, p, dw, ws, ws_bytes, x_bytes, dy_bytes, st);
        if (p.family == IIF_WGRAD_1X1) return launch_wgrad_1x1(a, p, dw, ws, ws_bytes, x_bytes, dy_bytes, st);
    }
    const int bc = p.bc;
    a.ktiles = p.ktiles;
    a.ntiles = p.ntiles;
    a.nsteps = p.nsteps;
    const int tiles = p.tiles;
    const int splits = p.splits;
    const int64_t slab = p.slab;
    a.steps_per_split = p.steps_per_split;
    a.slab = splits > 1 ? slab : 0;
    a.out = splits > 1 ? ws : dw;
    a.nsplits = splits;
    const dim3 grid(tiles, splits);
    const dim3 grid1d((unsigned)(p.blocks / a.groups), (unsigned)a.groups);
    const bool dma = p.family == IIF_WGRAD_DMA;
    if (dma) {
        const unsigned xb = (unsigned)x_bytes, yb = (unsigned)dy_bytes;
        if (bc == 64) hipLaunchKernelGGL((conv_wgrad_dma_kernel<T, 64>), grid1d, dim3(256), 0, st, a, xb, yb);
        else if (bc == 256) {
            if constexpr (sizeof(T) == 2) hipLaunchKernelGGL((conv_wgrad_dma_kernel<T, 256, 4>), grid1d, dim3(512), 0, st, a, xb, yb);
        } else hipLaunchKernelGGL((conv_wgrad_dma_kernel<T, 128>), grid1d, dim3(256), 0, st, a, xb, yb);
    } else {
        if (bc == 64) hipLaunchKernelGGL((conv_wgrad_kernel<T, 64>), grid, dim3(256), 0, st, a);
        else hipLaunchKernelGGL((conv_wgrad_kernel<T, 128>), grid, dim3(256), 0, st, a);
    }
    IIF_LAUNCH_CHECK();
    if (splits > 1) return reduce_slabs(ws, ws_bytes, splits, slab, a.groups * a.Cd, a.ldw, a.K, dw, st);
    return IIF_OK;
}

int wgrad_args_of(const iif_conv_desc* d, int64_t workspace_bytes, WgArgs& a, int64_t& x_bytes, int64_t& dy_bytes) {
    if (d->n <= 0 || d->hs <= 0 || d->ws <= 0 || d->cs <= 0 || d->hd <= 0 || d->wd <= 0 || d->cd <= 0 ||
        d->r <= 0 || d->s <= 0 || d->pad < 0 || workspace_bytes < 0)
        return IIF_EINVAL;
    if (d->stride != 1 && d->stride != 2) return IIF_EUNSUPPORTED;
    if (d->dtype != IIF_F32 && d->dtype != IIF_BF16) return IIF_EINVAL;
    if (d->transposed) return IIF_EINVAL;
    const int pe = d->dtype == IIF_F32 ? 4 : 8;
    if (d->cs % pe != 0 || d->cd % pe != 0 || d->ldw % 4 != 0 || d->ldw < d->r * d->s * d->cs) return IIF_EUNSUPPORTED;
    const int64_t M = (int64_t)d->n * d->hd * d->wd;
    if (M > 0x7fffff00LL || (int64_t)d->n * d->hs * d->ws > 0x7fffff00LL) return IIF_EUNSUPPORTED;
    a.N = d->n; a.Hs = d->hs; a.Ws = d->ws; a.Cs = d->cs; a.Hd = d->hd; a.Wd = d->wd; a.Cd = d->cd;
    a.R = d->r; a.S = d->s; a.sshift = d->stride - 1; a.pad = d->pad; a.ldw = d->ldw; a.M = (int)M;
    a.K = d->r * d->s * d->cs;
    a.groups = d->groups > 1 ? d->groups : 1;
    a.xpitch = a.groups * d->cs; a.ypitch = a.groups * d->cd;
    if (a.groups > 65535) return IIF_EUNSUPPORTED;
    const int64_t esz = d->dtype == IIF_F32 ? 4 : 2;
    x_bytes = (int64_t)d->n * d->hs * d->ws * a.xpitch * esz;
    dy_bytes = M * a.ypitch * esz;
    return IIF_OK;
}

int stacked_args_of(int64_t m, int cs, int cd1, int cd2, int ldw, int64_t workspace_bytes, WgArgs& a) {
    if (m <= 0 || cs <= 0 || cd1 <= 0 || cd2 <= 0 || workspace_bytes < 0) return IIF_EINVAL;
    if (cs % 8 || cd1 % 128 || cd2 % 8 || ldw % 4 || ldw < cs) return IIF_EUNSUPPORTED;
    if (m > 0x7fffff00LL || m * cs * 2 >= 0x7f000000LL || m * cd1 * 2 >= 0x7f000000LL || m * cd2 * 2 >= 0x7f000000LL) return IIF_EUNSUPPORTED;
    a.N = 1; a.Hs = 1; a.Ws = (int)m; a.Cs = cs; a.Hd = 1; a.Wd = (int)m; a.Cd = cd1 + cd2;
    a.R = 1; a.S = 1; a.sshift = 0; a.pad = 0; a.ldw = ldw; a.M = (int)m; a.K = cs; a.groups = 1;
    a.xpitch = cs; a.ypitch = cd1;
    return IIF_OK;
}

}

extern "C" int iif_conv_wgrad(const iif_conv_desc* d, const void* x, const void* dy, float* dw, void* workspace,
                              int64_t workspace_bytes, int splits, void* stream) {
    if (!d || !x || !dy || !dw) return IIF_EINVAL;
    WgArgs a{};
    int64_t x_bytes = 0, dy_bytes = 0;
    const int rc = wgrad_args_of(d, workspace_bytes, a, x_bytes, dy_bytes);
    if (rc != IIF_OK) return rc;
    if ((reinterpret_cast<uintptr_t>(x) | reinterpret_cast<uintptr_t>(dy) | reinterpret_cast<uintptr_t>(dw) |
         reinterpret_cast<uintptr_t>(workspace)) & 15)
        return IIF_EUNSUPPORTED;
    a.x = (const unsigned char*)x; a.dy = (const unsigned char*)dy;
    hipStream_t st = as_stream(stream);
    if (d->dtype == IIF_BF16)
        return launch_wgrad<unsigned short>(a, dw, (float*)workspace, workspace_bytes, splits, x_bytes, dy_bytes, st);
    return launch_wgrad<float>(a, dw, (float*)workspace, workspace_bytes, splits, x_bytes, dy_bytes, st);
}

extern "C" int iif_wgrad1x1_stacked(const void* x, const void* dy, const void* dy2, int64_t m, int cs, int cd1, int cd2, int ldw,
                                    float* out, void* workspace, int64_t workspace_bytes, int splits, void* stream) {
    if (!x || !dy || !dy2 || !out) return IIF_EINVAL;
    WgArgs a{};
    const int rc = stacked_args_of(m, cs, cd1, cd2, ldw, workspace_bytes, a);
    if (rc != IIF_OK) return rc;
    if ((reinterpret_cast<uintptr_t>(x) | reinterpret_cast<uintptr_t>(dy) | reinterpret_cast<uintptr_t>(dy2) |
         reinterpret_cast<uintptr_t>(out) | reinterpret_cast<uintptr_t>(workspace)) & 15)
        return IIF_EUNSUPPORTED;
    a.x = (const unsigned char*)x; a.dy = (const unsigned char*)dy;
    if (!workspace) workspace_bytes = 0;
    const WgPlan p = iif_plan::wgrad_plan(shape_of(a, 2, m * cs * 2, m * cd1 * 2, true, cd2), workspace_bytes, splits);
    return launch_wgrad_1x1(a, p, out, (float*)workspace, workspace_bytes, m * cs * 2, m * cd1 * 2, as_stream(stream),
                            (const unsigned char*)dy2, cd2);
}

extern "C" int iif_conv_wgrad_plan(const iif_conv_desc* d, int cd2, int64_t workspace_bytes, int splits, int32_t* out) {
    if (!d || !out || cd2 < -1) return IIF_EINVAL;
    WgArgs a{};
    int64_t x_bytes = 0, dy_bytes = 0;
    int rc = wgrad_args_of(d, workspace_bytes, a, x_bytes, dy_bytes);
    if (rc != IIF_OK) return rc;
    const bool stacked = cd2 > 0;
    if (stacked) {
        if (d->dtype != IIF_BF16 || d->r != 1 || d->s != 1 || d->stride != 1 || d->pad != 0 || a.groups != 1 || d->hs != d->hd ||
            d->ws != d->wd)
            return IIF_EUNSUPPORTED;
        rc = stacked_args_of(a.M, d->cs, d->cd, cd2, d->ldw, workspace_bytes, a);
        if (rc != IIF_OK) return rc;
        x_bytes = (int64_t)a.M * d->cs * 2; dy_bytes = (int64_t)a.M * d->cd * 2;
    }
    WgShape s = shape_of(a, d->dtype == IIF_F32 ? 4 : 2, x_bytes, dy_bytes, stacked, stacked ? cd2 : 0);
    s.gram = cd2 == -1;
    if (s.gram && (d->cs != d->cd || d->hs != d->hd || d->ws != d->wd)) return IIF_EINVAL;
    const WgPlan p = iif_plan::wgrad_plan(s, workspace_bytes, splits);
    if (p.rc != IIF_OK) return p.rc;
    out[0] = p.family; out[1] = p.bc; out[2] = p.bnw; out[3] = p.tiles; out[4] = p.nsteps; out[5] = p.splits;
    out[6] = p.steps_per_split; out[7] = (int32_t)p.blocks; out[8] = p.stages; out[9] = p.nch;
    return IIF_OK;
}

extern "C" int iif_slab_sum(float* slabs, int64_t slab_floats, int n, int rows, int ld, int cols, float* out, void* stream) {
    if (!slabs || !out || n < 1 || rows < 1 || ld < cols || cols < 1 || (ld & 3) || (cols & 3)) return IIF_EINVAL;
    if ((reinterpret_cast<uintptr_t>(slabs) | reinterpret_cast<uintptr_t>(out)) & 15) return IIF_EINVAL;
    const int64_t slab = (int64_t)rows * ld;
    if ((int64_t)n * slab > slab_floats) return IIF_EINVAL;
    return reduce_slabs(slabs, slab_floats * 4, n, slab, rows, ld, cols, out, (hipStream_t)stream);
}

#ifdef IIF_CONV_STAMPS
extern "C" int iif_debug_set_wgrad_stamps(unsigned long long* buf) {
    return hipMemcpyToSymbol(HIP_SYMBOL(g_wstamps), &buf, sizeof(buf)) == hipSuccess ? IIF_OK : IIF_ELAUNCH;
}
#endif
```

iif_amd/ops.py:

```python
import collections
import ctypes

import torch

from . import _lib
from ._lib import ConvDesc, check, dtype_code, lib, ptr, require_gpu, stream_ptr


def _desc(n, hs, ws, cs, hd, wd, cd, r, s, stride, pad, transposed, ldw, dtype, dst_dtype, groups=1, w_frag=None):
    kind = 0
    if isinstance(w_frag, tuple):
        w_frag, kind = w_frag
    return ConvDesc(n, hs, ws, cs, hd, wd, cd, r, s, stride, pad, transposed, ldw, dtype, dst_dtype, groups,
                    ptr(w_frag) if w_frag is not None else None, kind)


def conv_out_hw(h, w, r, s, stride, pad):
    return (h + 2 * pad - r) // stride + 1, (w + 2 * pad - s) // stride + 1


def conv_forward(x, w, r, s, stride, pad, out=None, out_dtype=None, bias=None, res=None, groups=1, out_hw=None, w_frag=None):
    require_gpu(x, w, bias, res)
    n, h, wd_, cin = x.shape
    cout, ldw = w.shape
# ... 42 lines not shown
    if rc < 0:
        check(rc, "iif_conv_route")
    return [ConvLaunch(CONV_ROUTES[out[9 * i]], *out[9 * i + 1:9 * i + 9]) for i in range(rc)]


def conv_forward_affine(x, w, r, s, stride, pad, out, affine, res=None, res_affine=None, relu_bits=None, groups=1, w_frag=None):
    require_gpu(x, w, out, affine, res, res_affine, relu_bits)
    n, h, wd_, cin = x.shape
    cout, ldw = w.shape
    ho, wo = out.shape[1], out.shape[2]
    d = _desc(n, h, wd_, cin // groups, ho, wo, cout // groups, r, s, stride, pad, 0, ldw, dtype_code(x), dtype_code(out),
              groups, w_frag)
    check(lib().iif_conv_igemm_affine(ctypes.byref(d), ptr(x), ptr(w), ptr(out), ptr(res), ptr(res_affine), ptr(affine),
                                      ptr(relu_bits), stream_ptr()), "iif_conv_igemm_affine")
    return out


def bn_fold_table(entries, device):
    import struct
    blob = b""
    for (g, b, rm, rv, st) in entries:
        require_gpu(g, b, rm, rv, st)
        c = g.numel()
        assert b.numel() == c and rm.numel() == c and rv.numel() == c and st.numel() == 4 * c and st.is_contiguous()
        blob += struct.pack("<QQQQQii", g.data_ptr(), b.data_ptr(), rm.data_ptr(), rv.data_ptr(), st.data_ptr(), c, 0)
    return torch.frombuffer(bytearray(blob), dtype=torch.uint8).to(device)


def bn_fold(table, n_layers, eps=1e-5):
    check(lib().iif_bn_fold(ptr(table), n_layers, float(eps), stream_ptr()), "iif_bn_fold")


def conv_forward_bnstats(x, w, r, s, stride, pad, out, partial, groups=1, w_frag=None):
    n, h, wd_, cin = x.shape
    cout, ldw = w.shape
    ho, wo = out.shape[1], out.shape[2]
    d = _desc(n, h, wd_, cin // groups, ho, wo, cout // groups, r, s, stride, pad, 0, ldw, dtype_code(x), dtype_code(out),
              groups, w_frag)
    nt = ctypes.c_int32(0)
    check(lib().iif_conv_igemm_bnstats(ctypes.byref(d), ptr(x), ptr(w), ptr(out), 0, 0, ptr(partial), partial.numel(),
                                       ctypes.byref(nt), stream_ptr()), "iif_conv_igemm_bnstats")
    return nt.value


def bn_finalize_stats(partial, n_partials, m, c, gamma, beta, running_mean, running_var, stats, eps=1e-5, momentum=0.1,
                      scratch=None, tickets=None, extra_sums=None):
    if extra_sums is not None:
        rows2, n2, c2, out2 = extra_sums
        check(lib().iif_bn_finalize_stats_sums(ptr(partial), n_partials, m, c, ptr(gamma), ptr(beta), eps, momentum,
                                               ptr(running_mean), ptr(running_var), ptr(stats), ptr(scratch),
                                               0 if scratch is None else scratch.numel(), ptr(tickets), ptr(rows2), n2, c2, ptr(out2),
                                               stream_ptr()), "iif_bn_finalize_stats_sums", tickets)
        return stats
    if tickets is not None:
        check(lib().iif_bn_finalize_stats_fused(ptr(partial), n_partials, m, c, ptr(gamma), ptr(beta), eps, momentum,
                                                ptr(running_mean), ptr(running_var), ptr(stats), ptr(scratch),
                                                0 if scratch is None else scratch.numel(), ptr(tickets), stream_ptr()),
              "iif_bn_finalize_stats_fused", tickets)
        return stats
    check(lib().iif_bn_finalize_stats(ptr(partial), n_partials, m, c, ptr(gamma), ptr(beta), eps, momentum,
                                      ptr(running_mean), ptr(running_var), ptr(stats), ptr(scratch),
                                      0 if scratch is None else scratch.numel(), stream_ptr()),
          "iif_bn_finalize_stats")
    return stats


def conv_dgrad(dy, wt, r, s, stride, pad, in_hw, out=None, res=None, groups=1, res_bits=None, w_frag=None):
    require_gpu(dy, wt, res)
    n, ho, wo, cout = dy.shape
    cin, ldw = wt.shape
    h, w_ = in_hw
    if out is None:
        out = torch.empty((n, h, w_, cin), dtype=dy.dtype, device=dy.device)
    d = _desc(n, ho, wo, cout // groups, h, w_, cin // groups, r, s, stride, pad, 1, ldw, dtype_code(dy), dtype_code(out),
              groups, w_frag)
    if res_bits is not None:
        check(lib().iif_conv_igemm_masked_res(ctypes.byref(d), ptr(dy), ptr(wt), ptr(out), ptr(res), ptr(res_bits),
                                              stream_ptr()), "iif_conv_igemm_masked_res")
        return out
    check(lib().iif_conv_igemm(ctypes.byref(d), ptr(dy), ptr(wt), ptr(out), ptr(res), 0, stream_ptr()), "iif_conv_igemm(dgrad)")
    return out


def conv_wgrad(x, dy, r, s, stride, pad, ldw=None, out=None, workspace=None, splits=0, groups=1):
    require_gpu(x, dy, out, workspace)
    n, h, w_, cin = x.shape
    _, ho, wo, cout = dy.shape
    k = r * s * (cin // groups)
    ldw = ldw or k
    if out is None:
        out = torch.zeros((cout, ldw), dtype=torch.float32, device=x.device)
    elif not out.is_contiguous() or out.numel() < cout * ldw:
        raise ValueError("conv_wgrad: out must be a contiguous float32 [Cout, ldw] tensor (rows are written with pitch ldw)")
    d = _desc(n, h, w_, cin // groups, ho, wo, cout // groups, r, s, stride, pad, 0, ldw, dtype_code(x), _lib.IIF_F32, groups)
    wsb = 0 if workspace is None else workspace.numel() * workspace.element_size()
    check(lib().iif_conv_wgrad(ctypes.byref(d), ptr(x), ptr(dy), ptr(out), ptr(workspace), wsb, splits, stream_ptr()),
          "iif_conv_wgrad")
    return out


WGRAD_FAMILIES = ("regstage", "dma", "1x1", "ninetap", "stem")
WgradPlan = collections.namedtuple("WgradPlan", "family bc bnw tiles nsteps splits steps_per_split blocks stages chunks")


def conv_wgrad_plan(n, hs, ws, cs, hd, wd, cd, r, s, stride, pad, ldw, dtype, groups=1, workspace_bytes=0, splits=0, cd2=0):
    d = _desc(n, hs, ws, cs, hd, wd, cd, r, s, stride, pad, 0, ldw, _lib.IIF_F32 if dtype == torch.float32 else _lib.IIF_BF16,
              _lib.IIF_F32, groups)
    out = (ctypes.c_int32 * 10)()
    check(lib().iif_conv_wgrad_plan(ctypes.byref(d), cd2, workspace_bytes, splits, ctypes.addressof(out)), "iif_conv_wgrad_plan")
    return WgradPlan(WGRAD_FAMILIES[out[0]], *out[1:])


def wgrad1x1_stacked(x2d, dy2d, dy2_2d, out, workspace, splits=0):
    require_gpu(x2d, dy2d, dy2_2d, out, workspace)
    m, cs = x2d.shape
    cd1, cd2 = dy2d.shape[1], dy2_2d.shape[1]
    if not out.is_contiguous() or out.shape[0] < cd1 + cd2:
        raise ValueError("wgrad1x1_stacked: out must be a contiguous float32 [cd1 + cd2, ldw] tensor")
    wsb = 0 if workspace is None else workspace.numel() * workspace.element_size()
    check(lib().iif_wgrad1x1_stacked(ptr(x2d), ptr(dy2d), ptr(dy2_2d), m, cs, cd1, cd2, out.shape[1], ptr(out), ptr(workspace), wsb,
                                     splits, stream_ptr()), "iif_wgrad1x1_stacked")
    return out


def bn_workspace(m, c, device):
    nbytes = lib().iif_bn_workspace_bytes(m, c)
    return torch.empty(nbytes, dtype=torch.uint8, device=device)


def bn_forward_stats(x2d, gamma, beta, running_mean, running_var, stats, ws, eps=1e-5, momentum=0.1):
    m, c = x2d.shape
    check(lib().iif_bn_forward_stats(ptr(x2d), dtype_code(x2d), m, c, ptr(gamma), ptr(beta), eps, momentum,
                                     ptr(running_mean), ptr(running_var), ptr(stats), ptr(ws), ws.numel(),
                                     stream_ptr()), "iif_bn_forward_stats")
    return stats


def bn_apply(x2d, stats, y2d, relu=True, residual=None, residual_stats=None, relu_bits=None):
    m, c = x2d.shape
    check(lib().iif_bn_apply(ptr(x2d), dtype_code(x2d), m, c, ptr(stats), ptr(residual), ptr(residual_stats),
                             1 if relu else 0, ptr(y2d), ptr(relu_bits), stream_ptr()), "iif_bn_apply")
    return y2d


def bn_backward(gy, y_mask, x2d, stats, gamma, dgamma, dbeta, dx, ws, gmasked=None, relu_bits=None):
    m, c = x2d.shape
    check(lib().iif_bn_backward(ptr(gy), ptr(y_mask), ptr(relu_bits), ptr(x2d), dtype_code(x2d), m, c, ptr(stats),
                                ptr(gamma), ptr(dgamma), ptr(dbeta), ptr(dx), ptr(gmasked), ptr(ws), ws.numel(),
                                stream_ptr()), "iif_bn_backward")
    return dx


def bn_partial_sums(partial, n_partials, c, sums):
    check(lib().iif_bn_partial_sums(ptr(partial), n_partials, c, ptr(sums), stream_ptr()), "iif_bn_partial_sums")
    return sums


def bn_stats_sums(x2d, sums, ws):
    m, c = x2d.shape
    check(lib().iif_bn_stats_sums(ptr(x2d), dtype_code(x2d), m, c, ptr(sums), ptr(ws), ws.numel(), stream_ptr()), "iif_bn_stats_sums")
    return sums


def bn_backward_sums(gy, y_mask, x2d, stats, sums, ws, relu_bits=None):
    m, c = x2d.shape
    check(lib().iif_bn_backward_sums(ptr(gy), ptr(y_mask), ptr(relu_bits), ptr(x2d), dtype_code(x2d), m, c, ptr(stats), ptr(sums),
                                     ptr(ws), ws.numel(), stream_ptr()), "iif_bn_backward_sums")
    return sums


def bn_backward_apply_sums(gy, y_mask, x2d, stats, gamma, local_sums, total_sums, total_count, dgamma, dbeta, dx, coef, gmasked=None,
                           relu_bits=None):
    m, c = x2d.shape
    check(lib().iif_bn_backward_apply_sums(ptr(gy), ptr(y_mask), ptr(relu_bits), ptr(x2d), dtype_code(x2d), m, c, ptr(stats), ptr(gamma),
                                           ptr(local_sums), ptr(total_sums), float(total_count), ptr(dgamma), ptr(dbeta), ptr(dx),
                                           ptr(gmasked), ptr(coef), stream_ptr()), "iif_bn_backward_apply_sums")
    return dx


def maxpool_forward(x, k, stride, pad):
    n, h, w, c = x.shape
    ho, wo = (h + 2 * pad - k) // stride + 1, (w + 2 * pad - k) // stride + 1
    y = torch.empty((n, ho, wo, c), dtype=x.dtype, device=x.device)
    idx = torch.empty((n, ho, wo, c), dtype=torch.uint8, device=x.device)
    check(lib().iif_maxpool_forward(ptr(x), dtype_code(x), n, h, w, c, k, stride, pad, ptr(y), ptr(idx),
                                    stream_ptr()), "iif_maxpool_forward")
    return y, idx


def maxpool_backward(gy, idx, in_shape, k, stride, pad, out=None):
    n, h, w, c = in_shape
    dx = out if out is not None else torch.empty(in_shape, dtype=gy.dtype, device=gy.device)
    check(lib().iif_maxpool_backward(ptr(gy), ptr(idx), dtype_code(gy), n, h, w, c, k, stride, pad, ptr(dx),
                                     stream_ptr()), "iif_maxpool_backward")
    return dx


def avgpool_forward(x, out=None):
    n, h, w, c = x.shape
    y = out if out is not None else torch.empty((n, c), dtype=x.dtype, device=x.device)
    check(lib().iif_avgpool_forward(ptr(x), dtype_code(x), n, h * w, c, ptr(y), stream_ptr()), "iif_avgpool_forward")
# ... 441 lines not shown
```

iif_amd/resnet_engine.py:

```python
import math
import os
from typing import NamedTuple, Optional

import torch
import torch.nn as nn

from . import _lib, ops
from .loss_reduction import CE_WORKSPACE_WORDS

BN_EPS = 1e-5
BN_MOMENTUM = 0.1
S2D_CPAD = 16


def _round_up(v, m):
    return (v + m - 1) // m * m


class ConvParam(nn.Module):

    def __init__(self, cin, cout, k, stride, pad, groups=1):
        super().__init__()
        self.cin, self.cout, self.k, self.stride, self.pad, self.groups = cin, cout, k, stride, pad, groups
        self.cg = cin // groups
# ... 297 lines not shown
                if attr == "weight":
                    gv = gflat[:m.out_features]; m._g2d = gflat
                else:
                    gv = gflat.view(-1)[:m.out_features]; m._gb1d = gflat.view(-1)
            elif isinstance(m, CosNormParam):
                if attr == "weight":
                    gv = gflat[:m.out_features]; m._g2d = gflat
                else:
                    gv = gflat.view(-1)[:1]; m._gs1d = gflat.view(-1)
            elif isinstance(m, NormedLinearParam):
                if attr == "weight":
                    gv = gflat[:, :m.out_features]; m._g2d = gflat
                else:
                    gv = gflat.view(-1)[:m.out_features]
            else:
                gv = gflat.view(-1)
                if attr == "weight":
                    m._dgamma = gv
                else:
                    m._dbeta = gv
            self._grad_views.append(gv)
        self._param_list = [getattr(m, attr) for (m, attr, _, _) in specs]

    def _apply(self, fn, recurse=True):
        out = super()._apply(fn, recurse)
        dev = next(self.parameters()).device
        if next(self.parameters()).dtype != torch.float32:
            raise RuntimeError("NativeResNet keeps fp32 master weights; choose bf16 compute with compute_dtype=")
        self._flatten(dev)
        return out

    def _units(self):
        seq = [("stem", self.conv1, self.bn1)]
        for st in self._stages:
            for blk in st:
                seq.append(("block", blk))
        seq.append(("head", self._head))
        return seq

    def _plan(self, n, h, w):
        key = (n, h, w, self.compute_dtype)
        if key in self._plans:
            return self._plans[key]
        P = _Plan(self, n, h, w)
        self._plans[key] = P
        return P

    def forward(self, x):
        _lib.require_gpu(x)
        if x.dim() != 4 or x.shape[1] != 3:
            raise ValueError("expected an NCHW image batch [N,3,H,W], got %s" % (tuple(x.shape),))
        need_grad = torch.is_grad_enabled() and any(p.requires_grad for p in self._param_list)
        if need_grad:
            if not self.training:
                raise RuntimeError("NativeResNet: an eval-mode forward under autograd is not supported (the native backward "
                                   "is the training-mode one: batch statistics, transposed weights); wrap evaluation in "
                                   "torch.no_grad() as classification/train.py:97 does, or call model.train()")
            return _NetFunction.apply(self, x, *self._param_list)
        return self.run_forward(x, self.training).clone()

    def set_fused_eval(self, flag=True):
        self.fused_eval = bool(flag)
        return self

    def eval_route(self, n, h, w):
        return [(name, route) for (name, _, route) in _eval_routes(self, n, h, w)]

    def run_forward(self, x, training):
        self._join_side_work()
        plan = self._plan(x.shape[0], x.shape[2], x.shape[3])
        plan.forward(x, training)
        if training and not torch.is_grad_enabled():
            self._join_side_work()
        plan.generation += 1
        self._saved = plan if training else None
        return plan.logits[:, :self.num_classes]

    def _join_side_work(self):
        for plan in self._plans.values():
            ev = getattr(plan, "_prep_bwd_done", None)
            if ev is not None:
                torch.cuda.current_stream().wait_event(ev)
                plan._prep_bwd_done = None

    def state_dict(self, *args, **kwargs):
        self._join_side_work()
        return super().state_dict(*args, **kwargs)

    def load_state_dict(self, *args, **kwargs):
        self._join_side_work()
        return super().load_state_dict(*args, **kwargs)

    def run_backward(self, dlogits=None, reducer=None, generation=None):
        plan = self._saved
        if plan is None:
            raise RuntimeError("run_backward() without a preceding training-mode forward")
        if generation is not None and generation != (id(plan), plan.generation):
            raise RuntimeError("NativeResNet keeps the activations of ONE forward: backward() was called for a forward whose "
                               "activations a later forward has overwritten (gradient accumulation must run "
                               "forward -> backward per micro-batch)")
        if dlogits is not None:
            plan.dlogits[:, :self.num_classes].copy_(dlogits)
        plan.backward(reducer)

    def sgd_step(self, lr, momentum=0.9, weight_decay=1e-4, nesterov=False, grad_scale=1.0):
        self._join_side_work()
        self._claim_optimizer("sgd")
        lo = self.block_offsets()["head"] if self._head_only else 0
        ops.sgd_step(self._arena[lo:], self._grad_arena[lo:], self._mom_arena[lo:], lr, momentum, weight_decay, nesterov,
                     grad_scale)

    def rmsprop_step(self, lr, alpha=0.9, eps=0.0316, weight_decay=1e-4, momentum=0.9, centered=False, grad_scale=1.0):
        if not eps > 0:
            raise ValueError("rmsprop_step: eps must be > 0 (the arena's zero padding lanes would divide 0 by 0), got %r" % (eps,))
        self._join_side_work()
        self._claim_optimizer("rmsprop")
        self._alloc_rmsprop_state(centered)
        lo = self.block_offsets()["head"] if self._head_only else 0
        ops.rmsprop_step(self._arena[lo:], self._grad_arena[lo:], self._sq_arena[lo:], lr, alpha, eps, weight_decay, momentum,
                         momentum_buf=self._mom_arena[lo:],
                         grad_avg=self._gavg_arena[lo:] if centered else None, grad_scale=grad_scale)
        self._rms_steps[1 if self._head_only else 0] += 1

    def _claim_optimizer(self, kind):
        if self._optimizer_kind not in (None, kind):
            raise RuntimeError("this engine's optimizer state belongs to %s: a %s step would reuse its momentum arena with "
                               "another meaning (one NativeResNet serves one optimizer)" % (self._optimizer_kind, kind))
        self._optimizer_kind = kind

    def _alloc_rmsprop_state(self, centered):
        if self._sq_arena is None:
            self._sq_arena = torch.zeros_like(self._arena)
        if centered and self._gavg_arena is None:
            self._gavg_arena = torch.zeros_like(self._arena)

    def _rmsprop_param_steps(self):
        head = self.block_offsets()["head"]
        return [self._rms_steps[0] + (self._rms_steps[1] if self._offsets[(id(m), attr)][0] >= head else 0)
                for (m, attr, _, _) in self._param_specs()]

    def optimizer_state_dict(self, lr, momentum=0.9, weight_decay=1e-4, nesterov=False, initial_lr=None):
        if self._optimizer_kind == "rmsprop":
            raise RuntimeError("this engine has stepped with RMSprop: its state is rmsprop_state_dict(), not SGD's")
        views = self._arena_views(self._mom_arena)
        state = {i: {"momentum_buffer": v.detach().clone().contiguous().cpu()} for i, v in enumerate(views)}
        group = {"lr": lr, "momentum": momentum, "dampening": 0, "weight_decay": weight_decay, "nesterov": nesterov,
                 "maximize": False, "foreach": None, "differentiable": False, "fused": None,
                 "params": list(range(len(views)))}
        if initial_lr is not None:
            group["initial_lr"] = initial_lr
        return {"state": state, "param_groups": [group]}

    def rmsprop_state_dict(self, lr, alpha=0.9, eps=0.0316, weight_decay=1e-4, momentum=0.9, centered=False, initial_lr=None):
        if self._optimizer_kind == "sgd":
            raise RuntimeError("this engine has stepped with SGD: its state is optimizer_state_dict(), not RMSprop's")
        steps = self._rmsprop_param_steps()
        if any(steps) and centered and self._gavg_arena is None:
            raise RuntimeError("rmsprop_state_dict(centered=True) for an engine that stepped without centering")
        take = lambda a: [v.detach().clone().contiguous().cpu() for v in self._arena_views(a)] if any(steps) else None
        sq = take(self._sq_arena)
        mom = take(self._mom_arena) if momentum > 0 else None
        gavg = take(self._gavg_arena) if centered else None
        state = {}
        for i, k in enumerate(steps):
            if k == 0:
                continue
# ... 283 lines not shown
                    b["sc"] = E(n, last.ho, last.wo, blk.out_planes)
                if blk.se is not None:
                    Z = lambda *s: torch.zeros(s, dtype=torch.float32, device=dev)
                    c, hid = blk.se.c, blk.se.hidden
                    b["se"] = {"sums": Z(n, c), "q": Z(n, c), "h": Z(n, hid), "e": Z(n, c), "s1": Z(n, c), "s2": Z(n, c),
                               "o": Z(n, c), "w2t": Z(hid, c), "dz2": Z(n, c), "dz1": Z(n, hid)}
                self.blocks.append(b)
                cur = last.y
        self.final = cur
        head = net._head
        self.pooled = E(n, head.in_features)
        self.logits = torch.zeros((n, head.out_padded), dtype=torch.float32, device=dev)
        self.dlogits = torch.zeros((n, head.out_padded), dtype=torch.float32, device=dev)
        self.dlogits_t = torch.zeros((n, head.out_padded), dtype=dt, device=dev)
        self.loss_rows = torch.zeros(n, dtype=torch.float32, device=dev)
        self.loss_rescale = torch.ones(1, dtype=torch.float32, device=dev)
        self.loss_ticket = torch.zeros(CE_WORKSPACE_WORDS, dtype=torch.int32, device=dev)
        self.label_status = torch.zeros(1, dtype=torch.int32, device=dev)
        self.loss = torch.zeros((), dtype=torch.float32, device=dev)
        op, D = head.out_padded, head.in_features
        self.head_kind = ("linear" if isinstance(head, LinearParam) else
                          "norm" if isinstance(head, NormedLinearParam) else "cosine")
        F32 = lambda *s: torch.zeros(s, dtype=torch.float32, device=dev)
        if self.head_kind == "linear":
            self.head_wsrc = head._w2d
        else:
            self.head_wsrc = F32(op, D)
            self.head_wnorm = F32(op)
            self.head_ex = E(n, D)
            self.head_xnorm = F32(n)
            self.head_dwn = F32(op, D)
            self.head_dex = E(n, D)
            if self.head_kind == "norm":
                self.head_wT = F32(op, D)
                self.head_dwT = F32(op, D)
            if self.head_kind == "cosine" and head.lr_scale:
                self.head_s2 = F32(1)
        if self.head_kind == "linear" and dt != torch.float32:
            ho_, hr_, hp_ = net._offsets[(id(head), "weight")]
            self.head_w = self.lp_arena[ho_:ho_ + hr_ * hp_].view(hr_, hp_)
        else:
            self.head_w = self.head_wsrc if dt == torch.float32 else torch.empty((op, D), dtype=dt, device=dev)
        self.head_wt = None if self.head_kind == "linear" else torch.zeros((D, _round_up(op, 16)), dtype=dt, device=dev)
        self._finish_weight_plan()
        cmax = max(u.conv.cout for u in self.units)
        mmax = max(u.n * u.ho * u.wo for u in self.units)
        self.bn_ws = ops.bn_workspace(mmax, cmax, dev)
        self.bn_tickets = torch.zeros(64, dtype=torch.int32, device=dev)
        self.bn_tickets_side = torch.zeros(64, dtype=torch.int32, device=dev) if self.bn_tickets is not None else None
        self.bn_partial = torch.empty(max(((u.n * u.ho * u.wo + 127) // 128) * 2 * u.conv.cout for u in self.units),
                                      dtype=torch.float32, device=dev)
        self.bn_scratch = torch.empty(128 * cmax, dtype=torch.float32, device=dev)
        ds_units = [b["ds"] for b in self.blocks if "ds" in b]
        self.fwd_side = bool(ds_units) and dt == torch.bfloat16
        if self.fwd_side:
            self.bn_partial_side = torch.empty(max(((u.n * u.ho * u.wo + 127) // 128) * 2 * u.conv.cout for u in ds_units),
                                               dtype=torch.float32, device=dev)
            self.bn_scratch_side = torch.empty(128 * max(u.conv.cout for u in ds_units), dtype=torch.float32, device=dev)
        self.bw_partial = torch.empty(max(((u.n * u.ho * u.wo + 127) // 128 + 8) * 2 * u.conv.cout for u in self.units),
                                      dtype=torch.float32, device=dev)
        self.fuse_bwd = dt == torch.bfloat16 and not os.environ.get("IIF_NO_BWD_FUSE")
        self._bw_ready = None
        self.wg_lag = int(os.environ.get("IIF_WG_LAG", "2"))
        wmax = max(max(u.conv.cout * (u.dwp.shape[1] if u.dwp is not None else u.conv.ldw) for u in self.units),
                   head.out_padded * head.in_features)
        self.wg_ws = torch.empty(min(16 * wmax * 4, 512 << 20), dtype=torch.uint8, device=dev)
        self._grad_pool = {}
        self._bwd_ready = False
        side = os.environ.get("IIF_SIDE_STREAMS")
        if os.environ.get("IIF_NO_WGRAD_STREAM"):
            side = "0"
        if side is None:
            per_unit = sum(u.n * u.ho * u.wo * u.conv.cout for u in self.units) / max(len(self.units), 1)
            side = "1" if per_unit >= 5e6 else "0"
        self.wg_stream = None
        if dev.type == "cuda" and side != "0":
            self.wg_stream = torch.cuda.Stream(device=dev)
        self._wg_events = {}
        self.wg_streams = []
        if self.wg_stream is not None:
            nws = int(os.environ.get("IIF_WG_STREAMS", "1"))
            self.wg_streams = [self.wg_stream] + [torch.cuda.Stream(device=dev) for _ in range(max(nws, 1) - 1)]
        self.wg_wss = [self.wg_ws] + [torch.empty_like(self.wg_ws) for _ in self.wg_streams[1:]]
        self._wg_rr = 0
        self.stem_wgrad_main = self.wg_stream is not None
        self.wg_ws_stem = (torch.empty(64 << 20, dtype=torch.uint8, device=dev)
                           if (self.stem_wgrad_main and self.stem_s2d) else None)
        self.ds_stream = None
        if self.wg_stream is not None and ds_units and dt == torch.bfloat16 and not os.environ.get("IIF_NO_BWD_SIDE"):
            self.ds_stream = torch.cuda.Stream(device=dev)
            self.bn_ws_ds = ops.bn_workspace(max(u.n * u.ho * u.wo for u in ds_units), max(u.conv.cout for u in ds_units), dev)
        self.standard_routes = False
        table = _train_routes(net, n, h, w, dt, self.wg_stream is not None, self.ds_stream is not None)
        assert len(table) == len(self.blocks)
        self._c3_routes = {b["units"][-1]: r for b, (_, r) in zip(self.blocks, table)}
        F = lambda *sh: torch.zeros(sh, dtype=torch.float32, device=dev)
        self.c3 = {}
        self.ds_alg = {}
        for b in self.blocks:
            u3 = b["units"][-1]
            r, cv3 = self._c3_routes[u3], u3.conv
            S = self.c3[u3] = _Conv3State(self.bw_partial)
            if r.prologue:
                S.u2 = b["units"][1]
            if r.csum_rows:
                S.rows = F(((u3.n * u3.ho * u3.wo + 127) // 128 + 8) * 2 * cv3.cin)
                S.sums = F(2, cv3.cin)
            if r.gram == "producer":
                S.slabs = torch.empty((256 + 17) * (cv3.cout + cv3.cin) * cv3.ldw, dtype=torch.float32, device=dev)
            if r.ds_algebra:
                du = b["ds"]
                cv = du.conv
                C, c = cv.cout, cv.cin
                self.ds_alg[id(du)] = {
                    "P": F(C, cv.ldw), "coef": F(3, C), "bias": F(c), "wt": torch.zeros((c, C + c), dtype=dt, device=dev),
                    "scr": torch.empty(ops.lib().iif_bn3_algebra_prep_scratch_floats(C, c), dtype=torch.float32, device=dev),
                    "tickets": torch.zeros(64, dtype=torch.int32, device=dev), "gram": F(c, cv.ldw), "csum": F(2, c),
                    "rows": torch.empty(self.bw_partial.numel(), dtype=torch.float32, device=dev),
                    "ws": torch.empty(64 << 20, dtype=torch.uint8, device=dev),
                    "ws_sum": ops.bn_workspace(du.n * du.ho * du.wo, c, dev)}
                S.g_rows = self.ds_alg[id(du)]["rows"]
        self.a3 = None
        alg = [u for u, r in self._c3_routes.items() if r.backward != "standard"]
        if alg:
            cm = max(u.conv.cin for u in alg)
            Cm = max(u.conv.cout for u in alg)
            ldm = max(u.conv.ldw for u in alg)
            self.a3 = [{"P": F(Cm + cm, ldm), "coef": F(3, Cm), "bias": F(cm),
                        "wt": torch.zeros(cm * (Cm + cm), dtype=dt, device=dev),
                        "scr": torch.empty(max(ops.lib().iif_bn3_algebra_prep_scratch_floats(u.conv.cout, u.conv.cin)
                                               for u in alg), dtype=torch.float32, device=dev),
                        "tickets": torch.zeros(64, dtype=torch.int32, device=dev)}
                       for _ in range(self.wg_lag)]
            self.a3g = [{"gram": F(cm, ldm), "csum": F(2, cm), "ws_gram": torch.empty(64 << 20, dtype=torch.uint8, device=dev),
                         "ws_sum": ops.bn_workspace(max(u.n * u.ho * u.wo for u in alg), cm, dev), "ev": None, "ev_csum": None,
                         "csum_fwd": None}
                        for _ in range(self.wg_lag + 1)]
            self.a3_ws = torch.empty(64 << 20, dtype=torch.uint8, device=dev)

    def _route(self, u):
        r = self._c3_routes.get(u, _STANDARD)
        if self.standard_routes:
            keep = r.prologue and r.forward != "nostore"
            r = _Route(prologue=keep, csum_rows=keep and r.csum_rows)
        return r

    def _closing(self, pred):
        return {u for u, r in self._c3_routes.items() if pred(r)}

    alg3_units = property(lambda self: self._closing(lambda r: r.backward != "standard"))
    rx_units = property(lambda self: self._closing(lambda r: r.backward == "rx"))
    twopass_units = property(lambda self: self._closing(lambda r: r.forward == "twopass"))
    nostore_units = property(lambda self: self._closing(lambda r: r.forward == "nostore"))
    pg_units = property(lambda self: self._closing(lambda r: r.gram == "producer"))
    pro_units = property(lambda self: {u: (self.c3[u].u2, self.c3[u].rows) for u, r in self._c3_routes.items() if r.prologue})

    def _finish_weight_plan(self):
        net, entries, views, off = self.net, [], [], 0
        for u in self.units:
            cv = u.conv
            if cv.groups > 1 or u.is_patch_gemm:
                continue
            ldwt = _round_up(cv.k * cv.k * cv.cout, 16)
            entries.append((net._offsets[(id(cv), "weight")][0], off, cv.cout, cv.cin, cv.k * cv.k, cv.ldw, ldwt))
            views.append((u, off, cv.cin, ldwt))
            off += _round_up(cv.cin * ldwt, 64)
# ... 373 lines not shown
            _lib.check(_lib.lib().iif_maxpool_bn_forward(_lib.ptr(u.x), _lib.dtype_code(u.x), _lib.ptr(u.stats), u.n, u.ho, u.wo,
                                                         u.conv.cout, 3, 2, 1, _lib.ptr(self.pool_out), _lib.ptr(self.pool_idx),
                                                         _lib.ptr(None), _lib.stream_ptr()), "iif_maxpool_bn_forward")
        else:
            self._eval_unit(u, routes[id(u.conv)])
            if net.style == "imagenet":
                self._maxpool_fwd(u.y)
        for b in self.blocks:
            units = b["units"]
            last = units[-1]
            for uu in units[:-1]:
                self._eval_unit(uu, routes[id(uu.conv)])
            if "se" in b:
                self._conv_raw(last)
                self._se_forward(b, last, False, folded=True)
                continue
            if "ds" in b:
                du = b["ds"]
                self._conv_raw(du)
                self._eval_unit(last, routes[id(last.conv)], res=du.x, res_affine=du.stats)
            elif "sc" in b:
                ops.shortcut_a_forward(b["inp"], b["blk"].out_planes, out=b["sc"])
                self._eval_unit(last, routes[id(last.conv)], res=b["sc"])
            else:
                self._eval_unit(last, routes[id(last.conv)], res=b["inp"])
        self._head_forward()

    def _se_forward(self, b, last, training, folded=False):
        se, P = b["blk"].se, b["se"]
        w1, w2 = se.excitation[0]._w2d, se.excitation[2]._w2d
        ops.se_squeeze(last.x, P["sums"])
        ops.transpose_f32(w2[:, :se.hidden], P["w2t"])
        ops.se_excite_forward(P["sums"], last.stats, last.ho * last.wo, w1, P["w2t"], P["q"], P["h"], P["e"])
        res, rstats = b["inp"], None
        if "ds" in b:
            du = b["ds"]
            if folded:
                self._conv_raw(du)
            else:
                self._conv_bn(du, training)
            res, rstats = du.x, du.stats
        elif "sc" in b:
            ops.shortcut_a_forward(b["inp"], b["blk"].out_planes, out=b["sc"])
            res = b["sc"]
        ops.se_apply(last.x, last.stats, P["e"], last.y, last.bits, residual=res, residual_stats=rstats)

    def _se_backward(self, b, last, g, par):
        se, P = b["blk"].se, b["se"]
        l1, l2 = se.excitation[0], se.excitation[2]
        hw = last.ho * last.wo
        ops.se_backward_sums(g, last.bits, last.x, P["s1"], P["s2"])
        ops.se_excite_backward(P["s1"], P["s2"], last.stats, hw, l1._w2d, P["w2t"], P["e"], P["h"], P["q"], P["dz2"], P["dz1"],
                               P["o"], l1._g2d, l2._g2d)
        m = last.n * hw
        G = self._gbuf(("dx", m, last.conv.cout, par), (m, last.conv.cout)).view(last.n, last.ho, last.wo, last.conv.cout)
        return ops.se_backward_form(g, P["e"], P["o"], G)

    def _maxpool_fwd(self, y):
        n, h, w, c = y.shape
        _lib.check(_lib.lib().iif_maxpool_forward(_lib.ptr(y), _lib.dtype_code(y), n, h, w, c, 3, 2, 1,
                                                  _lib.ptr(self.pool_out), _lib.ptr(self.pool_idx), _lib.stream_ptr()),
                   "iif_maxpool_forward")

    def _gbuf(self, key, shape):
        t = self._grad_pool.get(key)
        if t is None or tuple(t.shape) != tuple(shape):
            t = torch.empty(shape, dtype=self.dt, device=self.dev)
            self._grad_pool[key] = t
        return t

    def _wgrad_async(self, fn, after=None):
        if self.wg_stream is None:
            fn(self.wg_ws, 0)
            return
        ev = torch.cuda.Event()
        ev.record()
        k = self._wg_rr
        self._wg_rr = (k + 1) % len(self.wg_streams)
        st = self.wg_streams[k]
        with torch.cuda.stream(st):
            st.wait_event(ev)
            if after is not None:
                st.wait_event(after)
            fn(self.wg_wss[k], -len(self.wg_streams) if len(self.wg_streams) > 1 else 0)

    def _wgrad_fence(self, tag):
        if self.wg_stream is None:
            return
        evs = []
        for st in self.wg_streams:
            ev = torch.cuda.Event()
            ev.record(st)
            evs.append(ev)
        self._wg_events[tag] = evs
        old = self._wg_events.pop(tag + self.wg_lag - 1, None)
        if old is not None:
            for ev in old:
                torch.cuda.current_stream().wait_event(ev)

    def _stem_wgrad(self, u, dx4):
        cv = u.conv
        if u.s2d:
            if self.stem_wgrad_main:
                ops.conv_wgrad(u.src, dx4, 4, 4, 1, 2, ldw=u.dwp.shape[1], out=u.dwp, workspace=self.wg_ws_stem)
                ops.stem_s2d_unpack_grad(u.dwp, cv.cout, cv.cin, cv.k, S2D_CPAD, cv._g2d)
                return

            def stem(ws, sp):
                ops.conv_wgrad(u.src, dx4, 4, 4, 1, 2, ldw=u.dwp.shape[1], out=u.dwp, workspace=ws, splits=sp)
                ops.stem_s2d_unpack_grad(u.dwp, cv.cout, cv.cin, cv.k, S2D_CPAD, cv._g2d)
            self._wgrad_async(stem)
        else:
            self._wgrad_async(lambda ws, sp: ops.conv_wgrad(u.src, dx4, 1, 1, 1, 0, ldw=cv.ldw, out=cv._g2d, workspace=ws, splits=sp))

    def stem_activation(self):
        u = self.stem
        if self.pool_fused:
            x2 = u.x.view(-1, u.conv.cout)
            ops.bn_apply(x2, u.stats, u.y.view(x2.shape), relu=True)
        return u.y

    def _unit_backward(self, u, gy, mask, gmasked=None, dgrad_out=None, dgrad_res=None, need_dgrad=True, par=0,
                       keep_gy=False, mask_bits=None, dgrad_res_bits=None, fuse_up=None, ws=None, dxkey="dx"):
        cv, bn = u.conv, u.bn
        m = u.n * u.ho * u.wo
        g2 = gy.view(m, cv.cout)
        bits = mask_bits if mask_bits is not None else (None if mask is None else u.bits)
        ws = self.bn_ws if ws is None else ws
        ready = None
        if ws is self.bn_ws:
            ready, self._bw_ready = self._bw_ready, None
        by_algebra = ready is not None and ready[0] is u and len(ready) == 3
        assert by_algebra or not self.fuse_bwd or self._route(u).forward == "stored", "standard BN backward of a never-stored output"
        sync = self.net._sync_bn
        if sync is not None:
            group, world = sync
            side = ws is not self.bn_ws
            local = self._sync_sums(cv.cout, side, 1)
            if ready is not None and ready[0] is u and gmasked is None:
                ops.bn_partial_sums(self.bw_partial, ready[1], cv.cout, local)
            else:
                ops.bn_backward_sums(g2, None if (mask is None or bits is not None) else mask.view(m, cv.cout), u.x.view(m, cv.cout), u.stats,
                                     local, ws, relu_bits=bits)
            total = self._sync_sums(cv.cout, side, 2)
            total.copy_(local)
            torch.distributed.all_reduce(total, group=group)
            dx = self._gbuf((dxkey, m, cv.cout, par), (m, cv.cout)) if (gmasked is not None or keep_gy) else g2
            coef = self._sync_coef(cv.cout, side)
            ops.bn_backward_apply_sums(g2, None if (mask is None or bits is not None) else mask.view(m, cv.cout), u.x.view(m, cv.cout),
                                       u.stats, bn.weight, local, total, float(m) * world, bn._dgamma, bn._dbeta, dx, coef,
                                       gmasked=None if gmasked is None else gmasked.view(m, cv.cout), relu_bits=bits)
        elif by_algebra:
            return self._bn3_algebra(u, gy, ready[1], par, self._cur_block, dgrad_out, fuse_up, ready[2])
        elif ready is not None and ready[0] is u and gmasked is None:
            dx = self._gbuf((dxkey, m, cv.cout, par), (m, cv.cout)) if keep_gy else g2
            ops.bn_backward_partials(g2, bits, u.x.view(m, cv.cout), u.stats, bn.weight, self.bw_partial, ready[1],
                                     bn._dgamma, bn._dbeta, dx, ws, tickets=self.bn_tickets)
        elif gmasked is not None or keep_gy:
            dx = self._gbuf((dxkey, m, cv.cout, par), (m, cv.cout))
            ops.bn_backward(g2, None if mask is None else mask.view(m, cv.cout), u.x.view(m, cv.cout), u.stats, bn.weight,
                            bn._dgamma, bn._dbeta, dx, ws,
                            gmasked=None if gmasked is None else gmasked.view(m, cv.cout), relu_bits=bits)
        else:
            dx = g2
            ops.bn_backward(g2, None if mask is None else mask.view(m, cv.cout), u.x.view(m, cv.cout), u.stats, bn.weight,
                            bn._dgamma, bn._dbeta, dx, ws, relu_bits=bits)
        dx4 = dx.view(u.n, u.ho, u.wo, cv.cout)
        if u.is_patch_gemm:
            self._stem_wgrad(u, dx4)
            return None
        if u.groups > 1:
            def grouped(ws, sp):
                ops.conv_wgrad(u.src, dx4, cv.k, cv.k, cv.stride, cv.pad, ldw=u.dwp.shape[1], out=u.dwp,
                               workspace=ws, groups=u.groups, splits=sp)
                ops.group_unpack_grad(u.dwp, cv.cout, cv.cg, cv.chunk, cv.k * cv.k, cv._g2d)
            self._wgrad_async(grouped)
        else:
            self._wgrad_async(lambda ws, sp: ops.conv_wgrad(u.src, dx4, cv.k, cv.k, cv.stride, cv.pad, ldw=cv.ldw, out=cv._g2d,
                                                            workspace=ws, splits=sp))
        if not need_dgrad:
            return None
        if (fuse_up is not None and self.fuse_bwd and (u.groups == 1 or cv.stride == 1) and dgrad_out is not None
                and _dma_ok(dx4)):
            up, up_bits = fuse_up
            route = self._route(up)
            if route.backward != "standard" and cv.k == 1 and cv.stride == 1 and up_bits is not None:
                S = self.c3[up]
                rows = S.g_rows
                if route.backward == "rx":
                    if route.gram == "producer":
                        nt, S.slab_count = ops.conv_dgrad_masksum_rx_pg(dx4, u.wt, (u.hi, u.wi), dgrad_out, up_bits, rows, up.src, up.w,
                                                                        up.stats, S.slabs, up.conv.ldw, res=dgrad_res, res_bits=dgrad_res_bits)
                    else:
                        nt = ops.conv_dgrad_masksum_rx(dx4, u.wt, (u.hi, u.wi), dgrad_out, up_bits, rows, up.src, up.w, up.stats,
                                                       res=dgrad_res, res_bits=dgrad_res_bits)
                    self._bw_ready = (up, nt, rows)
                    return dgrad_out
                nt = ops.conv_dgrad_masksum(dx4, u.wt, (u.hi, u.wi), dgrad_out, up_bits, rows, res=dgrad_res,
                                            res_bits=dgrad_res_bits, up_x=None if route.backward == "pure" else up.x,
                                            up_stats=None if route.backward == "pure" else up.stats)
                self._bw_ready = (up, nt, rows)
                return dgrad_out
            nt = ops.conv_dgrad_bnbwd(dx4, u.wt, cv.k, cv.k, cv.stride, cv.pad, (u.hi, u.wi), dgrad_out, up.x, up_bits, up.stats,
                                      self.bw_partial, res=dgrad_res, res_bits=dgrad_res_bits, w_frag=u.wtf, groups=u.groups)
            self._bw_ready = (up, nt)
            return dgrad_out
        return ops.conv_dgrad(dx4, u.wt, cv.k, cv.k, cv.stride, cv.pad, (u.hi, u.wi), out=dgrad_out, res=dgrad_res,
                              groups=u.groups, res_bits=dgrad_res_bits, w_frag=u.wtf)

    def _bn3_gram_async(self, u, bi):
        A = self.a3g[bi % (self.wg_lag + 1)]
        cv = u.conv
        a2 = u.src
        A["csum_fwd"] = None
        route, S = self._route(u), self.c3[u]
        stacked = route.gram in ("stacked", "producer")
        if route.csum_rows and S.rows_count > 0:
            A["csum_fwd"] = S.sums
            if stacked:
                A["ev"] = A["ev_csum"] = None
                return

        def csum():
            if A["csum_fwd"] is None:
                ops.bn_stats_sums(a2.view(-1, cv.cin), A["csum"].view(-1)[:2 * cv.cin].view(2, cv.cin), A["ws_sum"])

        def gram():
            if not stacked:
                ops.conv_wgrad(a2, a2, 1, 1, 1, 0, ldw=cv.ldw, out=A["gram"].view(-1)[:cv.cin * cv.ldw].view(cv.cin, cv.ldw),
                               workspace=A["ws_gram"])
        st = self.ds_stream if self.ds_stream is not None else self.wg_stream
        if st is None:
            csum(); gram()
            A["ev"] = A["ev_csum"] = None
            return
        ev = torch.cuda.Event()
        ev.record()
        with torch.cuda.stream(st):
            st.wait_event(ev)
            csum()
            A["ev_csum"] = torch.cuda.Event()
            A["ev_csum"].record()
            gram()
            done = torch.cuda.Event()
            done.record()
        A["ev"] = done

    def _bn3_algebra(self, u, gt, nt, par, bi, dgrad_out, fuse_up, rows):
        cv, bn = u.conv, u.bn
        A, Ag = self.a3[par % self.wg_lag], self.a3g[bi % (self.wg_lag + 1)]
        C, c = cv.cout, cv.cin
        m = u.n * u.ho * u.wo
        g4 = gt.view(u.n, u.ho, u.wo, C)
        wb = u.w
        P = A["P"].view(-1)[:C * cv.ldw].view(C, cv.ldw)
        route, S = self._route(u), self.c3[u]
        pure = route.backward == "pure"
        if pure:
            ops.conv_wgrad(u.src, g4, 1, 1, 1, 0, ldw=cv.ldw, out=P, workspace=self.a3_ws)
        wt = A["wt"][:c * (C + c)].view(c, C + c)
        coef = A["coef"].view(-1)[:3 * C].view(3, C)
        csum_a2 = (Ag["csum_fwd"] if Ag.get("csum_fwd") is not None else Ag["csum"]).view(-1)[:c]
        gram_ev = Ag["ev"]
        if Ag.get("ev_csum") is not None:
            torch.cuda.current_stream().wait_event(Ag["ev_csum"])
        ops.bn3_algebra_prep(P if pure else None, wb, c, rows, nt, u.stats, bn.weight, m, coef, bn._dgamma, bn._dbeta, wt,
                             A["bias"][:c], A["scr"], A["tickets"], colsum2=csum_a2)

        stacked = route.gram in ("stacked", "producer")

        def finish_dw(ws, sp):
            gram = Ag["gram"].view(-1)[:c * cv.ldw].view(c, cv.ldw)
            if route.gram == "producer" and S.slab_count > 0:
                ext = A["P"].view(-1)[:(C + c) * cv.ldw].view(C + c, cv.ldw)
                ops.slab_sum(S.slabs, S.slab_count, C + c, cv.ldw, c, ext)
                S.slab_count = 0
                gram = ext[C:]
            elif stacked:
                ext = A["P"].view(-1)[:(C + c) * cv.ldw].view(C + c, cv.ldw)
                ops.wgrad1x1_stacked(u.src.view(m, c), gt.view(m, C), u.src.view(m, c), ext, ws, splits=sp)
                gram = ext[C:]
            elif not pure:
                ops.conv_wgrad(u.src, g4, 1, 1, 1, 0, ldw=cv.ldw, out=P, workspace=ws, splits=sp)
            ops.bn3_algebra_dw(P, wb, c, gram, csum_a2, coef, cv._g2d)
        if self.wg_stream is None:
            finish_dw(self.a3_ws, 0)
        else:
            self._wgrad_async(finish_dw, after=gram_ev)
        up, up_bits = fuse_up
        nt2 = ops.conv_dgrad2_bnbwd(g4, u.src, wt, A["bias"][:c], dgrad_out, up.x, up_bits, up.stats, self.bw_partial)
        self._bw_ready = (up, nt2)
        return dgrad_out

    def _ds_algebra(self, du, D, gt, x_in, nt, gin_ds):
        cv, bn = du.conv, du.bn
        C, c = cv.cout, cv.cin
        m = du.n * du.ho * du.wo
        g4 = gt.view(du.n, du.ho, du.wo, C)
        P = D["P"].view(-1)[:C * cv.ldw].view(C, cv.ldw)
        ops.bn_stats_sums(x_in.view(-1, c), D["csum"], D["ws_sum"])
        ops.conv_wgrad(x_in, g4, 1, 1, 1, 0, ldw=cv.ldw, out=P, workspace=D["ws"])
        coef = D["coef"]
        ops.bn3_algebra_prep(P, du.w, c, D["rows"], nt, du.stats, bn.weight, m, coef, bn._dgamma, bn._dbeta, D["wt"], D["bias"],
                             D["scr"], D["tickets"], colsum2=D["csum"].view(-1)[:c])
        ops.conv_dgrad2_bnbwd(g4, x_in, D["wt"], D["bias"], gin_ds)
        done = torch.cuda.Event()
        done.record()
        gram = D["gram"].view(-1)[:c * cv.ldw].view(c, cv.ldw)
        ops.conv_wgrad(x_in, x_in, 1, 1, 1, 0, ldw=cv.ldw, out=gram, workspace=D["ws"])
        ops.bn3_algebra_dw(P, du.w, c, gram, D["csum"].view(-1)[:c], coef, cv._g2d)
        return done

    def backward(self, reducer=None):
        offs = self.net.block_offsets() if reducer is not None else None
        self._bw_ready = None
        budget = 0
        if reducer is not None:
            reducer.begin()
            reducer.extra_streams = self.wg_streams + ([self.ds_stream] if self.ds_alg and self.ds_stream is not None else [])
            if reducer.world > 1 or reducer.force:
                budget = int(getattr(reducer, "cu_budget", 0))
        if budget:
            _lib.check(_lib.lib().iif_set_cu_budget(budget), "iif_set_cu_budget")
        try:
            self._backward(reducer, offs)
        finally:
            if budget:
                _lib.lib().iif_set_cu_budget(0)

    def _backward(self, reducer, offs):
        net = self.net
        head = net._head
        n = self.n
        pb = getattr(self, "_prep_bwd_done", None)
        if pb is not None:
            torch.cuda.current_stream().wait_event(pb)
            self._prep_bwd_done = None
        if self.wg_stream is not None:
            ev = torch.cuda.Event()
            ev.record()
            for st in self.wg_streams:
                st.wait_event(ev)
            if self.ds_stream is not None:
                self.ds_stream.wait_event(ev)
        op, D = head.out_padded, head.in_features
        if self.dt == torch.float32:
            dl = self.dlogits
        else:
            dl = ops.cast(self.dlogits, self.dlogits_t)
        dpooled = self._gbuf(("dpooled",), (n, 1, 1, D))
        if self.head_kind == "linear":
            def head_grads(ws, sp):
                ops.colsum_f32(self.dlogits, n, op, op, head._gb1d)
                ops.conv_wgrad(self.pooled.view(n, 1, 1, D), dl.view(n, 1, 1, op), 1, 1, 1, 0, ldw=D, out=head._g2d,
                               workspace=ws, splits=sp)
            self._wgrad_async(head_grads)
            ops.conv_dgrad(dl.view(n, 1, 1, op), self.head_wt, 1, 1, 1, 0, (1, 1), out=dpooled)
        else:
            ops.conv_wgrad(self.head_ex.view(n, 1, 1, D), dl.view(n, 1, 1, op), 1, 1, 1, 0, ldw=D, out=self.head_dwn,
                           workspace=self.wg_ws)
            if self.head_kind == "cosine":
                ops.rowmap_backward(head._w2d, self.head_wnorm, self.head_dwn, 1, 1.0, head._g2d, eps=0.0)
            else:
                ops.rowmap_backward(self.head_wT, self.head_wnorm, self.head_dwn, 1, 1.0, self.head_dwT)
                ops.transpose_f32(self.head_dwT, head._g2d)
            ops.conv_dgrad(dl.view(n, 1, 1, op), self.head_wt, 1, 1, 1, 0, (1, 1), out=self.head_dex.view(n, 1, 1, D))
            dp2 = dpooled.view(n, D)
            if self.head_kind == "norm":
                ops.rowmap_backward(self.pooled, self.head_xnorm, self.head_dex, 1, 1.0, dp2)
            elif head.lr_scale:
                ops.dot_window_f32(self.dlogits, self.logits, n, head.out_features, 2.0, head._gs1d, alpha_div=head._s1d)
                _lib.check(_lib.lib().iif_scale_by_device_scalar(_lib.ptr(self.head_dex), _lib.dtype_code(self.head_dex),
                                                                 self.head_dex.numel(), _lib.ptr(self.head_s2),
                                                                 _lib.ptr(self.head_dex), _lib.stream_ptr()), "iif_scale_by_device_scalar")
                ops.rowmap_backward(self.pooled, self.head_xnorm, self.head_dex, 0, 1.0, dp2)
            else:
                ops.rowmap_backward(self.pooled, self.head_xnorm, self.head_dex, 0, float(head.scale), dp2)
        fh, fw, fc = self.final.shape[1], self.final.shape[2], self.final.shape[3]
        if net._head_only:
            if self.wg_stream is not None:
                for st in self.wg_streams:
                    torch.cuda.current_stream().wait_stream(st)
                if self.ds_stream is not None:
                    torch.cuda.current_stream().wait_stream(self.ds_stream)
            if reducer is not None:
                reducer.finish_tail(offs["head"])
            return
        g = self._gbuf(("g", self.final.shape), self.final.shape)
        ops.avgpool_backward(dpooled.view(n, D), fh * fw, out=g.view(n, fh * fw, fc))
        if reducer is not None:
            reducer.gradients_ready_from(offs["head"])
        for bi in range(len(self.blocks) - 1, -1, -1):
            b = self.blocks[bi]
            units = b["units"]
            last = units[-1]
            inp = b["inp"]
            par = bi % self.wg_lag
            self._wgrad_fence(bi)
            self._cur_block = bi
            gin = self._gbuf(("gin", tuple(inp.shape), bi % (self.wg_lag + 1)), inp.shape)
            dkey = ("d", tuple(last.src.shape), len(units) - 1, par)
            lazy_mask = "se" not in b and "sc" not in b
            prev = self.blocks[bi - 1] if bi > 0 else None
            up_in = None
            if prev is not None and "se" not in prev and "sc" not in prev:
                up_in = (prev["units"][-1], prev["units"][-1].bits)
            inner = lambda ui: (units[ui - 1], units[ui - 1].bits)
            ds_done = gin_ds = None
            if "ds" in b and lazy_mask and self.ds_stream is not None:
                du = b["ds"]
                gin_ds = self._gbuf(("ginds", tuple(inp.shape), par), inp.shape)
                rdy = self._bw_ready
                D = self.ds_alg.get(id(du))
                by_algebra = D is not None and rdy is not None and rdy[0] is last and len(rdy) == 3
                by_algebra = by_algebra and rdy[2] is D["rows"]
                ev = torch.cuda.Event()
                ev.record()
                with torch.cuda.stream(self.ds_stream):
                    self.ds_stream.wait_event(ev)
                    if by_algebra:
                        ds_done = self._ds_algebra(du, D, g, inp, rdy[1], gin_ds)
                    else:
                        self._unit_backward(du, g, last.y, mask_bits=last.bits, keep_gy=True, dgrad_out=gin_ds, par=par,
                                            ws=self.bn_ws_ds, dxkey="dxds")
                        ds_done = torch.cuda.Event()
                        ds_done.record()
            if prev is not None and self._route(prev["units"][-1]).backward != "standard":
                self._bn3_gram_async(prev["units"][-1], bi - 1)
            if "se" in b:
                G = self._se_backward(b, last, g, par)
                d = self._unit_backward(last, G, None, par=par, dgrad_out=self._gbuf(dkey, last.src.shape),
                                        fuse_up=inner(len(units) - 1))
            elif lazy_mask:
                d = self._unit_backward(last, g, last.y, keep_gy=True, par=par, dgrad_out=self._gbuf(dkey, last.src.shape),
                                        fuse_up=inner(len(units) - 1))
            else:
                d = self._unit_backward(last, g, last.y, gmasked=g, par=par, dgrad_out=self._gbuf(dkey, last.src.shape),
                                        fuse_up=inner(len(units) - 1))
            for ui in range(len(units) - 2, 0, -1):
                uu = units[ui]
                d = self._unit_backward(uu, d, uu.y, par=par, fuse_up=inner(ui),
                                        dgrad_out=self._gbuf(("d", tuple(uu.src.shape), ui, par), uu.src.shape))
            first = units[0]
            if "ds" in b and ds_done is not None:
                torch.cuda.current_stream().wait_event(ds_done)
                self._unit_backward(first, d, first.y, dgrad_out=gin, dgrad_res=gin_ds, par=par, fuse_up=up_in)
            elif "ds" in b and lazy_mask:
                du = b["ds"]
                gin_ds = self._gbuf(("ginds", tuple(inp.shape), par), inp.shape)
                pending, self._bw_ready = self._bw_ready, None
                self._unit_backward(du, g, last.y, mask_bits=last.bits, keep_gy=True, dgrad_out=gin_ds, par=par, dxkey="dxds")
                self._bw_ready = pending
                self._unit_backward(first, d, first.y, dgrad_out=gin, dgrad_res=gin_ds, par=par, fuse_up=up_in)
            elif "ds" in b:
                self._unit_backward(first, d, first.y, dgrad_out=gin, par=par)
                self._unit_backward(b["ds"], g, None, dgrad_out=gin, dgrad_res=gin, par=par, fuse_up=up_in)
            elif "sc" in b:
                self._unit_backward(first, d, first.y, dgrad_out=gin, par=par)
                ops.shortcut_a_backward_acc(g, gin)
            elif lazy_mask:
                self._unit_backward(first, d, first.y, dgrad_out=gin, dgrad_res=g, dgrad_res_bits=last.bits, par=par,
                                    fuse_up=up_in)
            else:
                self._unit_backward(first, d, first.y, dgrad_out=gin, dgrad_res=g, par=par, fuse_up=up_in)
            g = gin
            if reducer is not None:
                reducer.gradients_ready_from(offs["blocks"][bi])
        u = self.stem
        g_pooled = g
        pool_bwd_fused = (net.style == "imagenet" and self.pool_fused and self.dt != torch.float32
                          and not os.environ.get("IIF_NO_POOL_BWD_FUSED"))
        if net.style == "imagenet" and not pool_bwd_fused:
            dy0 = self._gbuf(("dy0",), u.y.shape)
            _lib.check(_lib.lib().iif_maxpool_backward(_lib.ptr(g), _lib.ptr(self.pool_idx), _lib.dtype_code(g), u.n, u.ho,
                                                       u.wo, u.conv.cout, 3, 2, 1, _lib.ptr(dy0), _lib.stream_ptr()),
                       "iif_maxpool_backward")
            g = dy0
        if pool_bwd_fused:
            cv, bn = u.conv, u.bn
            dy0 = self._gbuf(("dy0",), u.y.shape)
            ph, pw = g_pooled.shape[1], g_pooled.shape[2]
            _lib.check(_lib.lib().iif_bn_backward_pool_fused(
                _lib.ptr(g_pooled), _lib.ptr(self.pool_idx), _lib.ptr(self.pool_x), _lib.ptr(u.x), _lib.dtype_code(u.x), u.n, u.ho, u.wo,
                cv.cout, ph, pw, _lib.ptr(u.stats), _lib.ptr(bn.weight), _lib.ptr(bn._dgamma), _lib.ptr(bn._dbeta), _lib.ptr(dy0),
                _lib.ptr(self.bn_ws), self.bn_ws.numel(), _lib.stream_ptr()), "iif_bn_backward_pool_fused")
            self._stem_wgrad(u, dy0)
        elif self.pool_fused:
            cv, bn = u.conv, u.bn
            m = u.n * u.ho * u.wo
            g2 = g.view(m, cv.cout)
            if self.dt == torch.float32:
                _lib.check(_lib.lib().iif_bn_backward_relu_recompute(_lib.ptr(g2), _lib.ptr(u.x), _lib.dtype_code(u.x), m, cv.cout,
                                                                     _lib.ptr(u.stats), _lib.ptr(bn.weight), _lib.ptr(bn._dgamma),
                                                                     _lib.ptr(bn._dbeta), _lib.ptr(g2), _lib.ptr(self.bn_ws),
                                                                     self.bn_ws.numel(), _lib.stream_ptr()),
                           "iif_bn_backward_relu_recompute")
            else:
                _lib.check(_lib.lib().iif_bn_backward_relu_recompute_pooled(
                    _lib.ptr(g2), _lib.ptr(u.x), _lib.dtype_code(u.x), m, cv.cout, _lib.ptr(u.stats), _lib.ptr(bn.weight),
                    _lib.ptr(bn._dgamma), _lib.ptr(bn._dbeta), _lib.ptr(g2), _lib.ptr(self.bn_ws), self.bn_ws.numel(), _lib.ptr(g_pooled),
                    _lib.ptr(self.pool_x), self.pool_x.numel() // cv.cout, _lib.stream_ptr()),
                    "iif_bn_backward_relu_recompute_pooled")
            self._stem_wgrad(u, g2.view(u.n, u.ho, u.wo, cv.cout))
        else:
            self._unit_backward(u, g, u.y, need_dgrad=False)
        if self.wg_stream is not None:
            for st in self.wg_streams:
                torch.cuda.current_stream().wait_stream(st)
            if self.ds_stream is not None:
                torch.cuda.current_stream().wait_stream(self.ds_stream)
            self._wg_events.clear()
        if reducer is not None:
            reducer.finish()


_DMA_LIMIT = int(os.environ.get("IIF_DMA_LIMIT", str(0x7f000000)))


def _dma_ok(t):
    return t.numel() * t.element_size() < _DMA_LIMIT


def _train_routes(net, n, h, w, dt, wg_stream, ds_stream):
    env = os.environ.get
    bf16 = dt == torch.bfloat16
    esz = 2 if bf16 else 4
    dma = lambda elems: elems * esz < _DMA_LIMIT
    dense1x1 = lambda cv: cv.k == 1 and cv.stride == 1 and cv.groups == 1
    algebra_ok = lambda cv, m: (dense1x1(cv) and cv.cin in (64, 128, 256) and cv.cout % 64 == 0 and cv.cout <= 4096
                                and dma(m * cv.cout) and m < (1 << 30))
    fuse_bwd = bf16 and not env("IIF_NO_BWD_FUSE")
    local_bn = net._sync_bn is None
    algebra_on = fuse_bwd and local_bn and not env("IIF_NO_BN3_ALGEBRA")
    pure_min = float(env("IIF_BN3_ALGEBRA_PURE_MIN_ELEMS", "9e7"))
    twopass_on, rx_on, nostore_on = bool(env("IIF_TWOPASS")), not env("IIF_NO_RX"), not env("IIF_NO_NOSTORE")
    prologue_on = fuse_bwd and local_bn and not env("IIF_NO_PROLOGUE")
    pro_max_k = int(env("IIF_PRO_MAX_K", "256"))
    stacked_on = wg_stream and not env("IIF_NO_GRAM_STACKED")
    pg_on = wg_stream and not env("IIF_NO_PG")
    ds_on = ds_stream and not env("IIF_NO_DS_ALGEBRA")

    c1 = net.conv1
    hh, ww = ops.conv_out_hw(h, w, c1.k, c1.k, c1.stride, c1.pad)
    if net.style == "imagenet":
        hh, ww = (hh + 2 - 3) // 2 + 1, (ww + 2 - 3) // 2 + 1
    blocks = [("layer%d.%d" % (si + 1, bi), blk) for si, st in enumerate(net._stages) for bi, blk in enumerate(st)]
    table = []
    for i, (name, blk) in enumerate(blocks):
        convs = [cv for (cv, _) in blk.units()]
        m_in = n * hh * ww
        for cv in convs:
            hh, ww = ops.conv_out_hw(hh, ww, cv.k, cv.k, cv.stride, cv.pad)
        cv3, m = convs[-1], n * hh * ww
        big = m * cv3.cout >= pure_min
        bottleneck = len(convs) == 3 and blk.se is None
        nxt = blocks[i + 1][1] if i + 1 < len(blocks) else None
        f = nxt.units()[0][0] if nxt is not None else None
        backward = "standard"
        if (algebra_on and bottleneck and (blk.downsample is not None or not blk.shortcut_a) and algebra_ok(cv3, m)
                and f is not None and nxt.se is None and dense1x1(f) and dma(m * f.cout)):
            if rx_on and ops.conv_dgrad_rx_ok(n, hh, ww, f.cout, f.cin, cv3.cin, dt):
                backward = "rx"
            else:
                backward = "pure" if big else "producer"
        alg = backward != "standard"
        forward = "stored"
        if alg and dma(m * cv3.cin):
            if twopass_on and big and blk.downsample is None:
                forward = "twopass"
            elif nostore_on and backward != "producer" and ops.conv_fwdbn_ok(n, hh, ww, cv3.cin, cv3.cout, dt):
                forward = "nostore"
        prologue = bool(prologue_on and bottleneck and dense1x1(cv3) and dma(m * cv3.cin) and forward != "twopass"
                        and cv3.cin <= pro_max_k and ops.conv_pro_ok(n, hh, ww, cv3.cin, cv3.cout, dt, forward == "nostore"))
        gram = "ahead" if alg else None
        if alg and backward != "pure" and cv3.cout % 128 == 0 and stacked_on:
            gram = "stacked"
            if (backward == "rx" and pg_on and cv3.ldw % 4 == 0 and cv3.ldw >= cv3.cin
                    and ops.conv_dgrad_rx_pg_ok(n, hh, ww, f.cout, f.cin, cv3.cin, dt)):
                gram = "producer"
        dcv = blk.downsample[0] if blk.downsample is not None else None
        ds_algebra = bool(ds_on and alg and dcv is not None and algebra_ok(dcv, m) and dma(m_in * dcv.cin))
        table.append((name, _Route(backward, forward, prologue, prologue and alg, gram, ds_algebra)))
    return table


def _eval_routes(net, n, h, w):
    dt = net.compute_dtype
    esz = 2 if dt == torch.bfloat16 else 4
    out = []
# ... 57 lines not shown
```

include/iif_amd.h:

```cpp
#ifndef IIF_AMD_H
#define IIF_AMD_H

#include <stdint.h>

#ifdef __cplusplus
extern "C" {
#endif

#define IIF_OK 0
#define IIF_EINVAL (-1)
#define IIF_EUNSUPPORTED (-2)
#define IIF_ELAUNCH (-3)

#define IIF_F32 0
#define IIF_BF16 1

#define IIF_RAW 0
#define IIF_SMOOTH 1
#define IIF_REL 2
#define IIF_NORMIT 3
#define IIF_GOMBIT 4
#define IIF_BASE2 5
#define IIF_BASE10 6

// ... 147 lines not shown
    int64_t feat_strides[4], grad_feat_strides[4], grad_score_strides[4], grad_delta_strides[4];
} iif_rpn_head_level;

int64_t iif_rpn_head_sampled_workspace_bytes(int slots, int ci, int co, int num_base);
int iif_rpn_head_sampled_bwd(const iif_rpn_grid* grid, const iif_rpn_head_level* levels, int B, int slots_n, const int32_t* owner,
                             const int32_t* slots, const float* w_conv, const float* b_conv, const float* w_cls, const float* w_reg,
                             int ci, int co, float* d_w_conv, float* d_b_conv, float* d_w_cls, float* d_b_cls, float* d_w_reg,
                             float* d_b_reg, void* d_workspace, int64_t workspace_bytes, void* stream);

int iif_scale_logits(const void* logits, int dtype, int64_t ld_logits, const float* table,
                     int B, int C, void* out, int64_t ld_out, void* stream);

int iif_softmax(const void* logits, int dtype, int64_t ld_logits, const float* table,
                int B, int C, float* out, int64_t ld_out, void* stream);

int iif_topk_hits(const void* logits, int dtype, int64_t ld_logits, const float* table,
                  const int64_t* targets, int B, int C, const int32_t* k_host, int nk,
                  int32_t* hits, void* stream);

int iif_eval_accumulate(const void* logits, int dtype, int64_t ld_logits, const float* table,
                        const int64_t* targets, int B, int C, const int32_t* k_host, int nk,
                        const double* bin_edges, int nb, int64_t* acc,
                        int64_t* pred_out, float* conf_out, void* stream);

int iif_scale_by_device_scalar(const void* x, int dtype, int64_t n, const float* d_scalar, void* out, void* stream);


int iif_seesaw_fwd_bwd(const void* cls_score, int dtype, int64_t ld_score, const int64_t* labels,
                       const float* label_weights, float* cum_samples, int update_counts,
                       float p, float q, float eps, float scale_cls, int div_by_pos, float scale_obj,
                       int N, int C, float* loss_rows_cls, float* loss_rows_obj, float* loss_out,
                       void* dscore, int64_t ld_dscore, int32_t* d_status, void* d_workspace, void* stream);
#define IIF_SEESAW_WORKSPACE_BYTES (4 * (4 + 2048 + 2 * 1024))

#define IIF_SEESAW_HEAD_WORKSPACE_BYTES (4 * (4 + 2048 + 4 + 4 * 1024))
int iif_seesaw_head_fwd(const void* cls_score, int dtype, int64_t ld_score, const int64_t* labels, const float* label_weights,
                        float* cum_samples, float p, float q, float eps, float loss_weight, int N, int C, void* dscore,
                        int64_t ld_dscore, float* loss_out, float* acc_out, float* avg_out, int32_t* d_status, void* d_workspace,
                        void* stream);

int iif_seesaw_head_bwd(const float* dscore, int64_t ld_dscore, int N, int C, const float* d_g_cls, const float* d_g_obj,
                        const float* d_avg, float loss_weight, float* out, int64_t ld_out, void* stream);

int iif_seesaw_activation(const void* cls_score, int dtype, int64_t ld_score, int N, int C,
                          float* out, int64_t ld_out, void* stream);

int iif_seesaw_accuracy(const void* cls_score, int dtype, int64_t ld_score, const int64_t* labels, int N, int C,
                        float* out, int32_t* d_workspace, void* stream);

int iif_seesaw_scale_grad(const float* dscore, int64_t ld_dscore, int N, int C, const float* g_cls, const float* g_obj,
                          int per_row, float* out, int64_t ld_out, void* stream);

int iif_mix_rows(const void* x, int dtype, const int64_t* perm, float lam, int B, int64_t n,
                 void* out, void* stream);


typedef struct iif_conv_desc {
    int32_t n, hs, ws, cs;
    int32_t hd, wd, cd;
    int32_t r, s;
    int32_t stride, pad;
    int32_t transposed;
    int32_t ldw;
    int32_t dtype;
    int32_t dst_dtype;
    int32_t groups;
    const void* wgt_frag;
    int32_t wgt_frag_kind;
} iif_conv_desc;

int iif_conv_igemm(const iif_conv_desc* d, const void* src, const void* wgt, void* dst,
                   const void* res, const float* bias, void* stream);

int iif_conv_igemm_bnstats(const iif_conv_desc* d, const void* src, const void* wgt, void* dst,
                           const void* res, const float* bias, float* bn_partial,
                           int64_t bn_partial_floats, int32_t* n_partials, void* stream);

int iif_conv_wgrad(const iif_conv_desc* d, const void* x, const void* dy, float* dw,
                   void* workspace, int64_t workspace_bytes, int splits, void* stream);

int iif_wgrad1x1_stacked(const void* x, const void* dy, const void* dy2, int64_t m, int cs, int cd1, int cd2,
                         int ldw, float* out, void* workspace, int64_t workspace_bytes, int splits,
                         void* stream);

#define IIF_WGRAD_REGSTAGE 0
#define IIF_WGRAD_DMA 1
#define IIF_WGRAD_1X1 2
#define IIF_WGRAD_NINETAP 3
#define IIF_WGRAD_STEM 4
int iif_conv_wgrad_plan(const iif_conv_desc* d, int cd2, int64_t workspace_bytes, int splits, int32_t* out);

int64_t iif_bn_workspace_bytes(int64_t m, int c);
int iif_bn_forward_stats(const void* x, int dtype, int64_t m, int c, const float* gamma,
                         const float* beta, float eps, float momentum, float* running_mean,
                         float* running_var, float* stats, void* workspace,
                         int64_t workspace_bytes, void* stream);
int iif_bn_apply(const void* x, int dtype, int64_t m, int c, const float* stats,
                 const void* residual, const float* residual_stats, int relu, void* y,
                 uint8_t* relu_bits, void* stream);
typedef struct iif_bn_fold_desc {
    const float* gamma; const float* beta; const float* running_mean; const float* running_var;
    float* stats;
    int32_t c, reserved;
} iif_bn_fold_desc;
int iif_bn_fold(const iif_bn_fold_desc* table, int n_layers, float eps, void* stream);
int iif_bn_finalize_stats(const float* partial, int n_partials, int64_t m, int c, const float* gamma,
                          const float* beta, float eps, float momentum, float* running_mean,
                          float* running_var, float* stats, float* scratch, int64_t scratch_floats,
                          void* stream);
int iif_bn_finalize_stats_fused(const float* partial, int n_partials, int64_t m, int c, const float* gamma,
                                const float* beta, float eps, float momentum, float* running_mean,
                                float* running_var, float* stats, float* scratch, int64_t scratch_floats,
                                int32_t* tickets, void* stream);
int iif_bn_finalize_stats_sums(const float* partial, int n_partials, int64_t m, int c, const float* gamma, const float* beta,
                               float eps, float momentum, float* running_mean, float* running_var, float* stats,
                               float* scratch, int64_t scratch_floats, int32_t* tickets, const float* partial2, int n_partials2,
                               int c2, float* sums2, void* stream);
int iif_bn_backward(const void* gy, const void* y_mask, const uint8_t* relu_bits, const void* x,
                    int dtype, int64_t m, int c, const float* stats, const float* gamma, float* dgamma,
                    float* dbeta, void* dx, void* gmasked, void* workspace, int64_t workspace_bytes,
                    void* stream);

int iif_maxpool_forward(const void* x, int dtype, int n, int h, int w, int c, int k, int stride,
                        int pad, void* y, uint8_t* argmax, void* stream);
int iif_maxpool_backward(const void* gy, const uint8_t* argmax, int dtype, int n, int h, int w, int c,
                         int k, int stride, int pad, void* dx, void* stream);

int iif_avgpool_forward(const void* x, int dtype, int n, int hw, int c, void* y, void* stream);
int iif_avgpool_backward(const void* gy, int dtype, int n, int hw, int c, void* dx, void* stream);

int iif_im2col_nchw(const float* img, int n, int cin, int h, int w, int r, int s, int stride, int pad,
                    int kp, int out_dtype, void* out, void* stream);

int iif_cast(const void* src, int src_dtype, void* dst, int dst_dtype, int64_t n, void* stream);

int iif_weight_transpose(const float* w, int cout, int cin, int rs, int ldw, int ldwt, int out_dtype,
                         void* wt, void* stream);

int iif_shortcut_a_forward(const void* x, int dtype, int n, int h, int w, int cin, int cout, void* y,
                           void* stream);
int iif_shortcut_a_backward_acc(const void* g, int dtype, int n, int h, int w, int cin, int cout,
                                void* dx, void* stream);

int iif_colsum_f32(const float* a, int rows, int cols, int64_t ld, float* out, void* stream);

int iif_sgd_step(float* params, const float* grads, float* momentum_buf, int64_t n, float lr,
                 const float* d_lr, float momentum, float weight_decay, int nesterov,
                 float grad_scale, void* stream);
#define IIF_PLAN_BN_STREAM 0
#define IIF_PLAN_GRID_STRIDE 1
#define IIF_PLAN_RMSPROP 2
#define IIF_PLAN_SE_STREAM 3
#define IIF_PLAN_STEM_POOL_ROWS 4
#define IIF_PLAN_POOL_FUSED 5
int iif_stream_plan(int family, int64_t work, int w, int cv, int32_t* out);

int iif_rmsprop_step(float* params, const float* grads, float* square_avg,
                     float* momentum_buf, float* grad_avg,
                     int64_t n, float lr, const float* d_lr, float alpha, float eps,
                     float weight_decay, float momentum, int centered,
                     float grad_scale, void* stream);

int iif_rowmap_forward(const void* x, int x_dtype, int rows, int cols, int64_t ldx, int mode,
                       float scale, float eps, void* out, int out_dtype, int64_t ldo, float* norms,
                       void* stream);
int iif_rowmap_backward(const void* x, int x_dtype, const float* norms, const void* g, int g_dtype,
// ... 356 lines not shown
```

Measured before the change: 15310.

## Defer split-K wgrad slab reduction into the next wgrad kernel's prologue

Instead of launching a separate reduce kernel after each split-K weight-gradient kernel, the pending slab reduction is carried forward and run inside the next wgrad kernel. Padding blocks do it directly, and the other blocks do it behind the initial DMA ring issue. Double-buffered workspaces via WgradChain keep the carried slabs from being overwritten, and explicit flushes are added before gradient reduction, the end of backward, and dependent unpack ops. The aim is to cut kernel launches and tail-idle time on the wgrad streams, at the cost of extra prologue work, more workspace memory and added ordering complexity.

```diff
diff --git a/iif_amd/_lib.py b/iif_amd/_lib.py
--- a/iif_amd/_lib.py
+++ b/iif_amd/_lib.py
@@ -29,6 +29,9 @@
     "iif_conv_igemm": [_P, _P, _P, _P, _P, _P, _P],
     "iif_conv_wgrad": [_P, _P, _P, _P, _P, _L, _I, _P],
     "iif_conv_wgrad_plan": [_P, _I, _L, _I, _P],
+    "iif_conv_wgrad_deferred": [_P, _P, _P, _P, _P, _L, _I, _P, _P, _P],
+    "iif_wgrad1x1_stacked_deferred": [_P, _P, _P, _L, _I, _I, _I, _I, _P, _P, _L, _I, _P, _P, _P],
+    "iif_wgrad_flush": [_P, _P],
     "iif_conv_igemm_bnstats": [_P, _P, _P, _P, _P, _P, _P, _L, _P, _P],
     "iif_bn_finalize_stats": [_P, _I, _L, _I, _P, _P, _F, _F, _P, _P, _P, _P, _L, _P],
     "iif_bn_finalize_stats_fused": [_P, _I, _L, _I, _P, _P, _F, _F, _P, _P, _P, _P, _L, _P, _P],
@@ -195,6 +198,11 @@
                                                                                                           ("wgt_frag_kind", ctypes.c_int32)]
 
 
+class SlabJob(ctypes.Structure):
+    _fields_ = [("ws", ctypes.c_void_p), ("dst", ctypes.c_void_p), ("slab", ctypes.c_int64)] + [
+        (k, ctypes.c_int32) for k in ("splits", "rows", "ldw", "K")]
+
+
 class RoiLevel(ctypes.Structure):
     _fields_ = [("ptr", ctypes.c_void_p), ("H", ctypes.c_int32), ("W", ctypes.c_int32), ("spatial_scale", ctypes.c_float)]
 
diff --git a/iif_amd/csrc/common.h b/iif_amd/csrc/common.h
--- a/iif_amd/csrc/common.h
+++ b/iif_amd/csrc/common.h
@@ -119,7 +119,7 @@
 
 struct ConvSwitches {
     bool no_stream, force_stream, regstage, no_v2, no_halo, force_halo, v2_force, no_regw, no_regw_fwdbn, no_bm256_2src,
-         regw_k512_cw16, regw_no_x2, regw_k512_no_epi;
+         regw_k512_cw16, regw_no_x2, regw_k512_no_epi, no_deferred_slabs;
     static ConvSwitches read();
 };
 extern ConvSwitches g_sw;
diff --git a/iif_amd/csrc/conv_igemm.hip b/iif_amd/csrc/conv_igemm.hip
--- a/iif_amd/csrc/conv_igemm.hip
+++ b/iif_amd/csrc/conv_igemm.hip
@@ -1959,6 +1959,7 @@
     c.regw_k512_cw16 = getenv("IIF_REGW_K512_CW16") != nullptr;
     c.regw_no_x2 = getenv("IIF_REGW_NO_X2") != nullptr;
     c.regw_k512_no_epi = getenv("IIF_REGW_K512_NO_EPI") != nullptr;
+    c.no_deferred_slabs = getenv("IIF_NO_DEFERRED_SLABS") != nullptr;
     return c;
 }
 
diff --git a/iif_amd/csrc/conv_wgrad.hip b/iif_amd/csrc/conv_wgrad.hip
--- a/iif_amd/csrc/conv_wgrad.hip
+++ b/iif_amd/csrc/conv_wgrad.hip
@@ -245,8 +245,61 @@
 
 template <int N> __device__ __forceinline__ void wait_vmcnt() { asm volatile("s_waitcnt vmcnt(%0)" ::"n"(N) : "memory"); }
 
+#ifdef IIF_NT_SLABS
+#define IIF_SLAB_LD(p) __builtin_nontemporal_load(reinterpret_cast<const f32x4*>(p))
+#else
+#define IIF_SLAB_LD(p) (*reinterpret_cast<const f32x4*>(p))
+#endif
+template <int W = 16>
+__device__ __forceinline__ f32x4 slab_sum_at(const float* ws, int s0, int s1, int64_t slab, int64_t e) {
+    f32x4 s = f32x4{0.f, 0.f, 0.f, 0.f};
+    for (int j = s0; j < s1; j += W) {
+        f32x4 t[W];
+#pragma unroll
+        for (int q = 0; q < W; ++q) t[q] = IIF_SLAB_LD(ws + (int64_t)(j + q < s1 ? j + q : s0) * slab + e);
+#pragma unroll
+        for (int q = 0; q < W; ++q) {
+            const f32x4 u = s + t[q];
+            if (j + q < s1) s = (j + q == s0) ? t[q] : u;
+        }
+    }
+    return s;
+}
+
+struct SlabJob {
+    const float* ws; float* dst; int64_t slab;
+    int splits, rows, ldw, K;
+};
+template <int NT, int W = 16>
+__device__ __forceinline__ void slab_job_run(const SlabJob& j) {
+    const int64_t total4 = (int64_t)j.rows * j.ldw / 4;
+    const int64_t nthr = (int64_t)gridDim.x * gridDim.y * NT;
+    for (int64_t i = ((int64_t)blockIdx.y * gridDim.x + blockIdx.x) * NT + threadIdx.x; i < total4; i += nthr) {
+        const int64_t e = i * 4;
+        if ((int)(e % j.ldw) >= j.K) continue;
+        *reinterpret_cast<f32x4*>(j.dst + e) = slab_sum_at<W>(j.ws, 0, j.splits, j.slab, e);
+    }
+}
+template <int NT, int W = 16>
+__device__ __forceinline__ void slab_job_in_prologue(const SlabJob& j) {
+    if (j.ws == nullptr) return;
+    slab_job_run<NT, W>(j);
+    wait_vmcnt<0>();
+}
+template <int NT, int W = 16>
+__device__ __forceinline__ void slab_job_of_padding_block(const SlabJob& j) {
+    if (j.ws != nullptr) slab_job_run<NT, W>(j);
+}
+#ifdef IIF_SLAB_JOB_FIRST
+#define IIF_SLAB_JOB_BEFORE_RING(j, NT, W) slab_job_in_prologue<NT, W>(j)
+#define IIF_SLAB_JOB_BEHIND_RING(j, NT, W)
+#else
+#define IIF_SLAB_JOB_BEFORE_RING(j, NT, W)
+#define IIF_SLAB_JOB_BEHIND_RING(j, NT, W) slab_job_in_prologue<NT, W>(j)
+#endif
+
 template <typename T, int BC, int WK = 2, int NST = 3>
-__global__ void __launch_bounds__(128 * WK) conv_wgrad_dma_kernel(WgArgs a, unsigned x_bytes, unsigned dy_bytes) {
+__global__ void __launch_bounds__(128 * WK) conv_wgrad_dma_kernel(WgArgs a, unsigned x_bytes, unsigned dy_bytes, SlabJob job) {
     constexpr int PE = WT<T>::PE, ROWS = WT<T>::ROWS;
     constexpr int BNW = 128;
     constexpr int NWV = 2 * WK;
@@ -269,7 +322,8 @@
     const int tiles = a.ktiles * a.ntiles;
     const int xcd = blockIdx.x & 7, jj = blockIdx.x >> 3;
     const int split = (jj / tiles) * 8 + xcd, tile = jj % tiles;
-    if (split >= a.nsplits) return;
+    constexpr int JW = BC == 64 ? 8 : 16;
+    if (split >= a.nsplits) { slab_job_of_padding_block<128 * WK, JW>(job); return; }
     const int kt = tile % a.ktiles, ntile = tile / a.ktiles;
     const int k0 = kt * BC, n0 = ntile * BNW;
     const int step0 = split * a.steps_per_split;
@@ -345,12 +399,14 @@
 
     const int g = lane >> 4, li = lane & 15;
     const int nst = step1 - step0;
+    IIF_SLAB_JOB_BEFORE_RING(job, 128 * WK, JW);
 #pragma unroll
     for (int s_ = 0; s_ < NST - 1; ++s_)
         if (s_ < nst) {
             if (s_ > 0) advance();
             issue(s_, step0 + s_);
         }
+    IIF_SLAB_JOB_BEHIND_RING(job, 128 * WK, JW);
     int stage = 0;
 #ifdef IIF_CONV_STAMPS
     unsigned long long w_wait = 0, w_issue = 0, w_rest = 0, w0, w1, w2, w3, wb;
@@ -461,7 +517,7 @@
 }
 
 template <int BC, int BNW, int NWV>
-__device__ __forceinline__ void wgrad1x1_body(const W1Args& a, unsigned x_bytes, unsigned dy_bytes) {
+__device__ __forceinline__ void wgrad1x1_body(const W1Args& a, unsigned x_bytes, unsigned dy_bytes, const SlabJob& job) {
     constexpr int NWN = BNW / 64, WK = NWV / NWN, CW = BC / WK, KJ = CW / 16;
     using SX = Swz<unsigned short, BNW>;
     using SY = Swz<unsigned short, BC>;
@@ -482,7 +538,7 @@
     const int tiles = a.ktiles * a.ntiles;
     const int xcd = blockIdx.x & 7, jj = blockIdx.x >> 3;
     const int split = (jj / tiles) * 8 + xcd, tile = jj % tiles;
-    if (split >= a.nsplits) return;
+    if (split >= a.nsplits) { slab_job_of_padding_block<NWV * 64>(job); return; }
     const int k0 = (tile % a.ktiles) * BC, n0 = (tile / a.ktiles) * BNW;
     const int step0 = split * a.steps_per_split;
     int step1 = step0 + a.steps_per_split;
@@ -575,8 +631,10 @@
                                                                       acc[ni][kj], 0, 0, 0);
         }
     };
+    IIF_SLAB_JOB_BEFORE_RING(job, NWV * 64, 16);
     if (nst > 0) issue(S0{});
     if (nst > 1) issue(S1{});
+    IIF_SLAB_JOB_BEHIND_RING(job, NWV * 64, 16);
     for (int t = 0; t < nst; t += 3) {
         step(S0{}, S2{}, t);
         if (t + 1 < nst) step(S1{}, S0{}, t + 1);
@@ -597,11 +655,11 @@
     }
 }
 
-__global__ void __launch_bounds__(512) wgrad1x1_256x128_kernel(W1Args a, unsigned xb, unsigned yb) { wgrad1x1_body<256, 128, 8>(a, xb, yb); }
-__global__ void __launch_bounds__(256) wgrad1x1_128x128_kernel(W1Args a, unsigned xb, unsigned yb) { wgrad1x1_body<128, 128, 4>(a, xb, yb); }
-__global__ void __launch_bounds__(256) wgrad1x1_64x128_kernel(W1Args a, unsigned xb, unsigned yb) { wgrad1x1_body<64, 128, 4>(a, xb, yb); }
-__global__ void __launch_bounds__(256) wgrad1x1_64x64_kernel(W1Args a, unsigned xb, unsigned yb) { wgrad1x1_body<64, 64, 4>(a, xb, yb); }
-__global__ void __launch_bounds__(512) wgrad1x1_64x256_kernel(W1Args a, unsigned xb, unsigned yb) { wgrad1x1_body<64, 256, 8>(a, xb, yb); }
+__global__ void __launch_bounds__(512) wgrad1x1_256x128_kernel(W1Args a, unsigned xb, unsigned yb, SlabJob job) { wgrad1x1_body<256, 128, 8>(a, xb, yb, job); }
+__global__ void __launch_bounds__(256) wgrad1x1_128x128_kernel(W1Args a, unsigned xb, unsigned yb, SlabJob job) { wgrad1x1_body<128, 128, 4>(a, xb, yb, job); }
+__global__ void __launch_bounds__(256) wgrad1x1_64x128_kernel(W1Args a, unsigned xb, unsigned yb, SlabJob job) { wgrad1x1_body<64, 128, 4>(a, xb, yb, job); }
+__global__ void __launch_bounds__(256) wgrad1x1_64x64_kernel(W1Args a, unsigned xb, unsigned yb, SlabJob job) { wgrad1x1_body<64, 64, 4>(a, xb, yb, job); }
+__global__ void __launch_bounds__(512) wgrad1x1_64x256_kernel(W1Args a, unsigned xb, unsigned yb, SlabJob job) { wgrad1x1_body<64, 256, 8>(a, xb, yb, job); }
 
 struct WgHaloArgs {
     const unsigned char* x; const unsigned char* dy; float* out;
@@ -612,7 +670,7 @@
 };
 
 template <int XB, int YB, int D>
-__global__ void __launch_bounds__(256) conv3x3_wgrad_halo_kernel(WgHaloArgs a, unsigned x_bytes, unsigned dy_bytes) {
+__global__ void __launch_bounds__(256) conv3x3_wgrad_halo_kernel(WgHaloArgs a, unsigned x_bytes, unsigned dy_bytes, SlabJob job) {
     constexpr int RB = 128;
     constexpr int XR = 32 * XB, YR = 32 * YB;
     constexpr unsigned OOB = 0xfffffff0u;
@@ -626,7 +684,7 @@
     const int tiles = a.ci_tiles * a.co_tiles;
     const int xcd = blockIdx.x & 7, jj = blockIdx.x >> 3;
     const int split = (jj / tiles) * 8 + xcd, tile = jj % tiles;
-    if (split >= a.nsplits) return;
+    if (split >= a.nsplits) { slab_job_of_padding_block<256>(job); return; }
     const int ci0 = a.grouped ? tile * 64 : (tile % a.ci_tiles) * 64, co0 = a.grouped ? tile * 64 : (tile / a.ci_tiles) * 64;
     const int step0 = split * a.steps_per_split;
     int step1 = step0 + a.steps_per_split;
@@ -673,9 +731,11 @@
 #pragma unroll
         for (int kj = 0; kj < 4; ++kj) acc[t][kj] = f32x4{0.f, 0.f, 0.f, 0.f};
 
+    IIF_SLAB_JOB_BEFORE_RING(job, 256, 16);
     for (int j = 0; j < LEAD; ++j) issue_x();
 #pragma unroll
     for (int j = 0; j < D; ++j) { issue_x(); issue_y(); }
+    IIF_SLAB_JOB_BEHIND_RING(job, 256, 16);
 
     const int g = lane >> 4, li = lane & 15, q = li >> 2, p = li & 3;
     int xo[9], yo[4];
@@ -755,7 +815,7 @@
     int64_t slab;
 };
 
-__global__ void __launch_bounds__(256) conv4x4_s2d_wgrad_kernel(WgStemArgs a, unsigned x_bytes, unsigned dy_bytes) {
+__global__ void __launch_bounds__(256) conv4x4_s2d_wgrad_kernel(WgStemArgs a, unsigned x_bytes, unsigned dy_bytes, SlabJob job) {
     constexpr int XRB = 32, YRB = 128;
     constexpr int XR = 512, YR = 128;
     constexpr int D = 2;
@@ -769,7 +829,7 @@
     const int wave = __builtin_amdgcn_readfirstlane(tid >> 6);
     const int xcd = blockIdx.x & 7, jj = blockIdx.x >> 3;
     const int split = jj * 8 + xcd;
-    if (split >= a.nsplits) return;
+    if (split >= a.nsplits) { slab_job_of_padding_block<256>(job); return; }
     const int step0 = split * a.steps_per_split;
     int step1 = step0 + a.steps_per_split;
     if (step1 > a.nsteps) step1 = a.nsteps;
@@ -814,9 +874,11 @@
 #pragma unroll
         for (int kj = 0; kj < 4; ++kj) acc[t][kj] = f32x4{0.f, 0.f, 0.f, 0.f};
 
+    IIF_SLAB_JOB_BEFORE_RING(job, 256, 16);
     if (wave == 0) for (int j = 0; j < a.LEAD; ++j) issue_x();
 #pragma unroll
     for (int j = 0; j < D; ++j) { if (wave == 0) issue_x(); issue_y(); }
+    IIF_SLAB_JOB_BEHIND_RING(job, 256, 16);
 
     const int g = lane >> 4, li = lane & 15, q = li >> 2, p = li & 3;
     int xo[4], yo[4];
@@ -870,11 +932,6 @@
     }
 }
 
-#ifdef IIF_NT_SLABS
-#define IIF_SLAB_LD(p) __builtin_nontemporal_load(reinterpret_cast<const f32x4*>(p))
-#else
-#define IIF_SLAB_LD(p) (*reinterpret_cast<const f32x4*>(p))
-#endif
 __global__ void __launch_bounds__(256) wgrad_reduce_kernel(const float* ws, int splits, int chunk, int64_t slab, int Cd,
                                                            int ldw, int K, float* out, int64_t out_stride) {
     const int64_t total4 = (int64_t)Cd * ldw / 4;
@@ -885,18 +942,7 @@
         const int64_t e = i * 4;
         const int n = (int)(e % ldw);
         if (n >= K) continue;
-        f32x4 s = f32x4{0.f, 0.f, 0.f, 0.f};
-        for (int j = s0; j < s1; j += 16) {
-            f32x4 t[16];
-#pragma unroll
-            for (int q = 0; q < 16; ++q) t[q] = IIF_SLAB_LD(ws + (int64_t)(j + q < s1 ? j + q : s0) * slab + e);
-#pragma unroll
-            for (int q = 0; q < 16; ++q) {
-                const f32x4 u = s + t[q];
-                if (j + q < s1) s = (j + q == s0) ? t[q] : u;
-            }
-        }
-        *reinterpret_cast<f32x4*>(dst + e) = s;
+        *reinterpret_cast<f32x4*>(dst + e) = slab_sum_at(ws, s0, s1, slab, e);
     }
 }
 
@@ -920,6 +966,47 @@
     return IIF_OK;
 }
 
+inline int flush_job(const SlabJob& j, hipStream_t st) {
+    if (j.ws == nullptr) return IIF_OK;
+    const int blocks = iif_plan::reduce_plan(j.splits, j.slab, 0).blocks;
+    hipLaunchKernelGGL(wgrad_reduce_kernel, dim3(blocks, 1), dim3(256), 0, st, j.ws, j.splits, j.splits, j.slab, j.rows, j.ldw, j.K, j.dst,
+                       (int64_t)0);
+    IIF_LAUNCH_CHECK();
+    return IIF_OK;
+}
+
+struct Deferral {
+    SlabJob carry{};
+    iif_slab_job* pend = nullptr;
+};
+
+inline int take_carry(const iif_slab_job* c, const WgPlan& p, const float* ws, int64_t ws_bytes, hipStream_t st, Deferral& d) {
+    d.carry = SlabJob{};
+    if (!c || !c->ws) return IIF_OK;
+    if (!c->dst || c->splits < 1 || c->rows < 1 || c->ldw < 4 || (c->ldw & 3) || c->K < 1 || c->K > c->ldw || (c->K & 3) ||
+        c->slab < (int64_t)c->rows * c->ldw ||
+        ((reinterpret_cast<uintptr_t>(c->ws) | reinterpret_cast<uintptr_t>(c->dst) | (uintptr_t)(c->slab * 4)) & 15))
+        return IIF_EINVAL;
+    const SlabJob j{c->ws, c->dst, c->slab, c->splits, c->rows, c->ldw, c->K};
+    const char* lo = (const char*)c->ws; const char* hi = lo + (int64_t)c->splits * c->slab * 4;
+    const bool writes_ws = p.splits > 1 && ws != nullptr;
+    const bool overlap = writes_ws && lo < (const char*)ws + ws_bytes && (const char*)ws < hi;
+    if (g_sw.no_deferred_slabs || p.family == IIF_WGRAD_REGSTAGE || overlap) return flush_job(j, st);
+    d.carry = j;
+    return IIF_OK;
+}
+
+inline int finish_slabs(float* ws, int64_t ws_bytes, const WgPlan& p, int ldw, int K, float* dw, hipStream_t st, const Deferral& d) {
+    if (d.pend) *d.pend = iif_slab_job{};
+    if (p.splits <= 1) return IIF_OK;
+    if (d.pend && p.stages == 1 && !g_sw.no_deferred_slabs) {
+        d.pend->ws = ws; d.pend->dst = dw; d.pend->slab = p.slab; d.pend->splits = p.splits; d.pend->rows = p.rows;
+        d.pend->ldw = ldw; d.pend->K = K;
+        return IIF_OK;
+    }
+    return reduce_slabs(ws, ws_bytes, p.splits, p.slab, p.rows, ldw, K, dw, st);
+}
+
 inline WgShape shape_of(const WgArgs& a, int esz, int64_t x_bytes, int64_t dy_bytes, bool stacked = false, int cd2 = 0) {
     WgShape s{};
     s.N = a.N; s.Hs = a.Hs; s.Ws = a.Ws; s.Cs = a.Cs; s.Hd = a.Hd; s.Wd = a.Wd; s.Cd = a.Cd; s.R = a.R; s.S = a.S;
@@ -930,7 +1017,7 @@
 }
 
 inline int launch_wgrad_halo(const WgArgs& a, const WgPlan& p, float* dw, float* ws, int64_t ws_bytes, int64_t x_bytes,
-                             int64_t dy_bytes, hipStream_t st) {
+                             int64_t dy_bytes, hipStream_t st, const Deferral& df) {
     WgHaloArgs h{};
     h.x = a.x; h.dy = a.dy; h.N = a.N; h.H = a.Hd; h.W = a.Wd; h.Cs = a.xpitch; h.Cd = a.ypitch; h.ldw = a.ldw;
     h.grouped = a.groups > 1;
@@ -943,14 +1030,14 @@
     h.out = splits > 1 ? ws : dw;
     h.nsplits = splits;
     const dim3 grid((unsigned)p.blocks);
-    hipLaunchKernelGGL((conv3x3_wgrad_halo_kernel<8, 4, 2>), grid, dim3(256), 0, st, h, (unsigned)x_bytes, (unsigned)dy_bytes);
+    hipLaunchKernelGGL((conv3x3_wgrad_halo_kernel<8, 4, 2>), grid, dim3(256), 0, st, h, (unsigned)x_bytes, (unsigned)dy_bytes,
+                       df.carry);
     IIF_LAUNCH_CHECK();
-    if (splits > 1) return reduce_slabs(ws, ws_bytes, splits, p.slab, p.rows, a.ldw, a.K, dw, st);
-    return IIF_OK;
+    return finish_slabs(ws, ws_bytes, p, a.ldw, a.K, dw, st, df);
 }
 
 inline int launch_wgrad_stem(const WgArgs& a, const WgPlan& p, float* dw, float* ws, int64_t ws_bytes, int64_t x_bytes,
-                             int64_t dy_bytes, hipStream_t st) {
+                             int64_t dy_bytes, hipStream_t st, const Deferral& df) {
     WgStemArgs h{};
     h.x = a.x; h.dy = a.dy; h.N = a.N; h.H = a.Hd; h.W = a.Wd; h.ldw = a.ldw;
     h.LB = p.LB;
@@ -962,14 +1049,13 @@
     h.out = splits > 1 ? ws : dw;
     h.nsplits = splits;
     hipLaunchKernelGGL(conv4x4_s2d_wgrad_kernel, dim3((unsigned)p.blocks), dim3(256), 0, st, h, (unsigned)x_bytes,
-                       (unsigned)dy_bytes);
+                       (unsigned)dy_bytes, df.carry);
     IIF_LAUNCH_CHECK();
-    if (splits > 1) return reduce_slabs(ws, ws_bytes, splits, p.slab, p.rows, a.ldw, a.K, dw, st);
-    return IIF_OK;
+    return finish_slabs(ws, ws_bytes, p, a.ldw, a.K, dw, st, df);
 }
 
 inline int launch_wgrad_1x1(const WgArgs& g, const WgPlan& p, float* dw, float* ws, int64_t ws_bytes, int64_t x_bytes, int64_t dy_bytes,
-                            hipStream_t st, const unsigned char* dy2 = nullptr, int cd2 = 0) {
+                            hipStream_t st, const Deferral& df, const unsigned char* dy2 = nullptr, int cd2 = 0) {
     W1Args a{};
     a.x = g.x; a.dy = g.dy; a.M = g.M; a.Cs = g.Cs; a.Cd = g.Cd; a.ldw = g.ldw;
     a.dy2 = dy2; a.Cd1 = dy2 ? g.Cd - cd2 : g.Cd; a.Cd2 = cd2;
@@ -985,26 +1071,30 @@
     a.nsplits = splits;
     const dim3 grid((unsigned)p.blocks);
     const unsigned xb = (unsigned)x_bytes, yb = (unsigned)dy_bytes;
-    if (bc == 256) hipLaunchKernelGGL(wgrad1x1_256x128_kernel, grid, dim3(512), 0, st, a, xb, yb);
-    else if (bc == 128) hipLaunchKernelGGL(wgrad1x1_128x128_kernel, grid, dim3(256), 0, st, a, xb, yb);
-    else if (bnw == 256) hipLaunchKernelGGL(wgrad1x1_64x256_kernel, grid, dim3(512), 0, st, a, xb, yb);
-    else if (bnw == 128) hipLaunchKernelGGL(wgrad1x1_64x128_kernel, grid, dim3(256), 0, st, a, xb, yb);
-    else hipLaunchKernelGGL(wgrad1x1_64x64_kernel, grid, dim3(256), 0, st, a, xb, yb);
+    const SlabJob& job = df.carry;
+    if (bc == 256) hipLaunchKernelGGL(wgrad1x1_256x128_kernel, grid, dim3(512), 0, st, a, xb, yb, job);
+    else if (bc == 128) hipLaunchKernelGGL(wgrad1x1_128x128_kernel, grid, dim3(256), 0, st, a, xb, yb, job);
+    else if (bnw == 256) hipLaunchKernelGGL(wgrad1x1_64x256_kernel, grid, dim3(512), 0, st, a, xb, yb, job);
+    else if (bnw == 128) hipLaunchKernelGGL(wgrad1x1_64x128_kernel, grid, dim3(256), 0, st, a, xb, yb, job);
+    else hipLaunchKernelGGL(wgrad1x1_64x64_kernel, grid, dim3(256), 0, st, a, xb, yb, job);
     IIF_LAUNCH_CHECK();
-    if (splits > 1) return reduce_slabs(ws, ws_bytes, splits, slab, g.Cd, g.ldw, g.Cs, dw, st);
-    return IIF_OK;
+    return finish_slabs(ws, ws_bytes, p, g.ldw, g.Cs, dw, st, df);
 }
 
 template <typename T>
 int launch_wgrad(WgArgs a, float* dw, float* ws, int64_t ws_bytes, int splits_req, int64_t x_bytes, int64_t dy_bytes,
-                 hipStream_t st) {
+                 hipStream_t st, const iif_slab_job* carry, iif_slab_job* pend) {
     if (!ws) ws_bytes = 0;
     const WgPlan p = iif_plan::wgrad_plan(shape_of(a, (int)sizeof(T), x_bytes, dy_bytes), ws_bytes, splits_req);
     if (p.rc != IIF_OK) return p.rc;
+    Deferral df;
+    df.pend = pend;
+    const int rcc = take_carry(carry, p, ws, ws_bytes, st, df);
+    if (rcc != IIF_OK) return rcc;
     if constexpr (sizeof(T) == 2) {
-        if (p.family == IIF_WGRAD_NINETAP) return launch_wgrad_halo(a, p, dw, ws, ws_bytes, x_bytes, dy_bytes, st);
-        if (p.family == IIF_WGRAD_STEM) return launch_wgrad_stem(a, p, dw, ws, ws_bytes, x_bytes, dy_bytes, st);
-        if (p.family == IIF_WGRAD_1X1) return launch_wgrad_1x1(a, p, dw, ws, ws_bytes, x_bytes, dy_bytes, st);
+        if (p.family == IIF_WGRAD_NINETAP) return launch_wgrad_halo(a, p, dw, ws, ws_bytes, x_bytes, dy_bytes, st, df);
+        if (p.family == IIF_WGRAD_STEM) return launch_wgrad_stem(a, p, dw, ws, ws_bytes, x_bytes, dy_bytes, st, df);
+        if (p.family == IIF_WGRAD_1X1) return launch_wgrad_1x1(a, p, dw, ws, ws_bytes, x_bytes, dy_bytes, st, df);
     }
     const int bc = p.bc;
     a.ktiles = p.ktiles;
@@ -1022,17 +1112,16 @@
     const bool dma = p.family == IIF_WGRAD_DMA;
     if (dma) {
         const unsigned xb = (unsigned)x_bytes, yb = (unsigned)dy_bytes;
-        if (bc == 64) hipLaunchKernelGGL((conv_wgrad_dma_kernel<T, 64>), grid1d, dim3(256), 0, st, a, xb, yb);
+        if (bc == 64) hipLaunchKernelGGL((conv_wgrad_dma_kernel<T, 64>), grid1d, dim3(256), 0, st, a, xb, yb, df.carry);
         else if (bc == 256) {
-            if constexpr (sizeof(T) == 2) hipLaunchKernelGGL((conv_wgrad_dma_kernel<T, 256, 4>), grid1d, dim3(512), 0, st, a, xb, yb);
-        } else hipLaunchKernelGGL((conv_wgrad_dma_kernel<T, 128>), grid1d, dim3(256), 0, st, a, xb, yb);
+            if constexpr (sizeof(T) == 2) hipLaunchKernelGGL((conv_wgrad_dma_kernel<T, 256, 4>), grid1d, dim3(512), 0, st, a, xb, yb, df.carry);
+        } else hipLaunchKernelGGL((conv_wgrad_dma_kernel<T, 128>), grid1d, dim3(256), 0, st, a, xb, yb, df.carry);
     } else {
         if (bc == 64) hipLaunchKernelGGL((conv_wgrad_kernel<T, 64>), grid, dim3(256), 0, st, a);
         else hipLaunchKernelGGL((conv_wgrad_kernel<T, 128>), grid, dim3(256), 0, st, a);
     }
     IIF_LAUNCH_CHECK();
-    if (splits > 1) return reduce_slabs(ws, ws_bytes, splits, slab, a.groups * a.Cd, a.ldw, a.K, dw, st);
-    return IIF_OK;
+    return finish_slabs(ws, ws_bytes, p, a.ldw, a.K, dw, st, df);
 }
 
 int wgrad_args_of(const iif_conv_desc* d, int64_t workspace_bytes, WgArgs& a, int64_t& x_bytes, int64_t& dy_bytes) {
@@ -1070,8 +1159,10 @@
 
 }
 
-extern "C" int iif_conv_wgrad(const iif_conv_desc* d, const void* x, const void* dy, float* dw, void* workspace,
-                              int64_t workspace_bytes, int splits, void* stream) {
+extern "C" int iif_conv_wgrad_deferred(const iif_conv_desc* d, const void* x, const void* dy, float* dw, void* workspace,
+                                       int64_t workspace_bytes, int splits, void* stream, const iif_slab_job* carry,
+                                       iif_slab_job* pending) {
+    if (pending) *pending = iif_slab_job{};
     if (!d || !x || !dy || !dw) return IIF_EINVAL;
     WgArgs a{};
     int64_t x_bytes = 0, dy_bytes = 0;
@@ -1083,12 +1174,19 @@
     a.x = (const unsigned char*)x; a.dy = (const unsigned char*)dy;
     hipStream_t st = as_stream(stream);
     if (d->dtype == IIF_BF16)
-        return launch_wgrad<unsigned short>(a, dw, (float*)workspace, workspace_bytes, splits, x_bytes, dy_bytes, st);
-    return launch_wgrad<float>(a, dw, (float*)workspace, workspace_bytes, splits, x_bytes, dy_bytes, st);
-}
-
-extern "C" int iif_wgrad1x1_stacked(const void* x, const void* dy, const void* dy2, int64_t m, int cs, int cd1, int cd2, int ldw,
-                                    float* out, void* workspace, int64_t workspace_bytes, int splits, void* stream) {
+        return launch_wgrad<unsigned short>(a, dw, (float*)workspace, workspace_bytes, splits, x_bytes, dy_bytes, st, carry, pending);
+    return launch_wgrad<float>(a, dw, (float*)workspace, workspace_bytes, splits, x_bytes, dy_bytes, st, carry, pending);
+}
+
+extern "C" int iif_conv_wgrad(const iif_conv_desc* d, const void* x, const void* dy, float* dw, void* workspace,
+                              int64_t workspace_bytes, int splits, void* stream) {
+    return iif_conv_wgrad_deferred(d, x, dy, dw, workspace, workspace_bytes, splits, stream, nullptr, nullptr);
+}
+
+extern "C" int iif_wgrad1x1_stacked_deferred(const void* x, const void* dy, const void* dy2, int64_t m, int cs, int cd1, int cd2,
+                                             int ldw, float* out, void* workspace, int64_t workspace_bytes, int splits, void* stream,
+                                             const iif_slab_job* carry, iif_slab_job* pending) {
+    if (pending) *pending = iif_slab_job{};
     if (!x || !dy || !dy2 || !out) return IIF_EINVAL;
     WgArgs a{};
     const int rc = stacked_args_of(m, cs, cd1, cd2, ldw, workspace_bytes, a);
@@ -1099,8 +1197,26 @@
     a.x = (const unsigned char*)x; a.dy = (const unsigned char*)dy;
     if (!workspace) workspace_bytes = 0;
     const WgPlan p = iif_plan::wgrad_plan(shape_of(a, 2, m * cs * 2, m * cd1 * 2, true, cd2), workspace_bytes, splits);
-    return launch_wgrad_1x1(a, p, out, (float*)workspace, workspace_bytes, m * cs * 2, m * cd1 * 2, as_stream(stream),
+    Deferral df;
+    df.pend = pending;
+    const int rcc = take_carry(carry, p, (const float*)workspace, workspace_bytes, as_stream(stream), df);
+    if (rcc != IIF_OK) return rcc;
+    return launch_wgrad_1x1(a, p, out, (float*)workspace, workspace_bytes, m * cs * 2, m * cd1 * 2, as_stream(stream), df,
                             (const unsigned char*)dy2, cd2);
+}
+
+extern "C" int iif_wgrad1x1_stacked(const void* x, const void* dy, const void* dy2, int64_t m, int cs, int cd1, int cd2, int ldw,
+                                    float* out, void* workspace, int64_t workspace_bytes, int splits, void* stream) {
+    return iif_wgrad1x1_stacked_deferred(x, dy, dy2, m, cs, cd1, cd2, ldw, out, workspace, workspace_bytes, splits, stream, nullptr,
+                                         nullptr);
+}
+
+extern "C" int iif_wgrad_flush(void* stream, const iif_slab_job* job) {
+    if (!job) return IIF_EINVAL;
+    Deferral df;
+    WgPlan none{};
+    none.family = IIF_WGRAD_REGSTAGE;
+    return take_carry(job, none, nullptr, 0, as_stream(stream), df);
 }
 
 extern "C" int iif_conv_wgrad_plan(const iif_conv_desc* d, int cd2, int64_t workspace_bytes, int splits, int32_t* out) {
diff --git a/iif_amd/ops.py b/iif_amd/ops.py
--- a/iif_amd/ops.py
+++ b/iif_amd/ops.py
@@ -148,7 +148,52 @@
     return out
 
 
+class WgradChain:
+
+    def __init__(self, workspace, other):
+        require_gpu(workspace, other)
+        self.workspaces = (workspace, other)
+        self.k = 0
+        self.job = None
+        self.readers = []
+
+    def _settled(self):
+        self.job = None
+        readers, self.readers = self.readers, []
+        for fn in readers:
+            fn()
+
+    def _launch(self, call):
+        new = _lib.SlabJob()
+        call(self.workspaces[self.k], ctypes.byref(self.job) if self.job is not None else None, ctypes.byref(new))
+        self._settled()
+        if new.ws:
+            self.job = new
+            self.k ^= 1
+
+    def then(self, fn):
+        if self.job is None:
+            fn()
+        else:
+            self.readers.append(fn)
+
+    def flush(self):
+        if self.job is not None:
+            check(lib().iif_wgrad_flush(stream_ptr(), ctypes.byref(self.job)), "iif_wgrad_flush")
+            self._settled()
+
+
+def wgrad_then(workspace, fn):
+    if isinstance(workspace, WgradChain):
+        workspace.then(fn)
+    else:
+        fn()
+
+
 def conv_wgrad(x, dy, r, s, stride, pad, ldw=None, out=None, workspace=None, splits=0, groups=1):
+    chain = workspace if isinstance(workspace, WgradChain) else None
+    if chain is not None:
+        workspace = None
     require_gpu(x, dy, out, workspace)
     n, h, w_, cin = x.shape
     _, ho, wo, cout = dy.shape
@@ -159,6 +204,11 @@
     elif not out.is_contiguous() or out.numel() < cout * ldw:
         raise ValueError("conv_wgrad: out must be a contiguous float32 [Cout, ldw] tensor (rows are written with pitch ldw)")
     d = _desc(n, h, w_, cin // groups, ho, wo, cout // groups, r, s, stride, pad, 0, ldw, dtype_code(x), _lib.IIF_F32, groups)
+    if chain is not None:
+        chain._launch(lambda ws, carry, pending: check(
+            lib().iif_conv_wgrad_deferred(ctypes.byref(d), ptr(x), ptr(dy), ptr(out), ptr(ws), ws.numel() * ws.element_size(), splits,
+                                          stream_ptr(), carry, pending), "iif_conv_wgrad_deferred"))
+        return out
     wsb = 0 if workspace is None else workspace.numel() * workspace.element_size()
     check(lib().iif_conv_wgrad(ctypes.byref(d), ptr(x), ptr(dy), ptr(out), ptr(workspace), wsb, splits, stream_ptr()),
           "iif_conv_wgrad")
@@ -178,11 +228,20 @@
 
 
 def wgrad1x1_stacked(x2d, dy2d, dy2_2d, out, workspace, splits=0):
+    chain = workspace if isinstance(workspace, WgradChain) else None
+    if chain is not None:
+        workspace = None
     require_gpu(x2d, dy2d, dy2_2d, out, workspace)
     m, cs = x2d.shape
     cd1, cd2 = dy2d.shape[1], dy2_2d.shape[1]
     if not out.is_contiguous() or out.shape[0] < cd1 + cd2:
         raise ValueError("wgrad1x1_stacked: out must be a contiguous float32 [cd1 + cd2, ldw] tensor")
+    if chain is not None:
+        chain._launch(lambda ws, carry, pending: check(
+            lib().iif_wgrad1x1_stacked_deferred(ptr(x2d), ptr(dy2d), ptr(dy2_2d), m, cs, cd1, cd2, out.shape[1], ptr(out), ptr(ws),
+                                                ws.numel() * ws.element_size(), splits, stream_ptr(), carry, pending),
+            "iif_wgrad1x1_stacked_deferred"))
+        return out
     wsb = 0 if workspace is None else workspace.numel() * workspace.element_size()
     check(lib().iif_wgrad1x1_stacked(ptr(x2d), ptr(dy2d), ptr(dy2_2d), m, cs, cd1, cd2, out.shape[1], ptr(out), ptr(workspace), wsb,
                                      splits, stream_ptr()), "iif_wgrad1x1_stacked")
diff --git a/iif_amd/resnet_engine.py b/iif_amd/resnet_engine.py
--- a/iif_amd/resnet_engine.py
+++ b/iif_amd/resnet_engine.py
@@ -403,6 +403,10 @@
             if ev is not None:
                 torch.cuda.current_stream().wait_event(ev)
                 plan._prep_bwd_done = None
+            if any(c.job is not None for c in plan.wg_chains):
+                plan._flush_wgrads()
+                for st in plan.wg_streams:
+                    torch.cuda.current_stream().wait_stream(st)
 
     def state_dict(self, *args, **kwargs):
         self._join_side_work()
@@ -852,6 +856,9 @@
             nws = int(os.environ.get("IIF_WG_STREAMS", "1"))
             self.wg_streams = [self.wg_stream] + [torch.cuda.Stream(device=dev) for _ in range(max(nws, 1) - 1)]
         self.wg_wss = [self.wg_ws] + [torch.empty_like(self.wg_ws) for _ in self.wg_streams[1:]]
+        deferred = not os.environ.get("IIF_NO_DEFERRED_SLABS")
+        self.bn3_dw_flush = bool(os.environ.get("IIF_BN3_DW_FLUSH"))
+        self.wg_chains = [ops.WgradChain(w, torch.empty_like(w) if deferred else w) for w in self.wg_wss[:len(self.wg_streams)]]
         self._wg_rr = 0
         self.stem_wgrad_main = self.wg_stream is not None
         self.wg_ws_stem = (torch.empty(64 << 20, dtype=torch.uint8, device=dev)
@@ -1391,7 +1398,13 @@
             st.wait_event(ev)
             if after is not None:
                 st.wait_event(after)
-            fn(self.wg_wss[k], -len(self.wg_streams) if len(self.wg_streams) > 1 else 0)
+            fn(self.wg_chains[k], -len(self.wg_streams) if len(self.wg_streams) > 1 else 0)
+
+    def _flush_wgrads(self):
+        for st, chain in zip(self.wg_streams, self.wg_chains):
+            if chain.job is not None:
+                with torch.cuda.stream(st):
+                    chain.flush()
 
     def _wgrad_fence(self, tag):
         if self.wg_stream is None:
@@ -1417,7 +1430,7 @@
 
             def stem(ws, sp):
                 ops.conv_wgrad(u.src, dx4, 4, 4, 1, 2, ldw=u.dwp.shape[1], out=u.dwp, workspace=ws, splits=sp)
-                ops.stem_s2d_unpack_grad(u.dwp, cv.cout, cv.cin, cv.k, S2D_CPAD, cv._g2d)
+                ops.wgrad_then(ws, lambda: ops.stem_s2d_unpack_grad(u.dwp, cv.cout, cv.cin, cv.k, S2D_CPAD, cv._g2d))
             self._wgrad_async(stem)
         else:
             self._wgrad_async(lambda ws, sp: ops.conv_wgrad(u.src, dx4, 1, 1, 1, 0, ldw=cv.ldw, out=cv._g2d, workspace=ws, splits=sp))
@@ -1482,7 +1495,7 @@
             def grouped(ws, sp):
                 ops.conv_wgrad(u.src, dx4, cv.k, cv.k, cv.stride, cv.pad, ldw=u.dwp.shape[1], out=u.dwp,
                                workspace=ws, groups=u.groups, splits=sp)
-                ops.group_unpack_grad(u.dwp, cv.cout, cv.cg, cv.chunk, cv.k * cv.k, cv._g2d)
+                ops.wgrad_then(ws, lambda: ops.group_unpack_grad(u.dwp, cv.cout, cv.cg, cv.chunk, cv.k * cv.k, cv._g2d))
             self._wgrad_async(grouped)
         else:
             self._wgrad_async(lambda ws, sp: ops.conv_wgrad(u.src, dx4, cv.k, cv.k, cv.stride, cv.pad, ldw=cv.ldw, out=cv._g2d,
@@ -1591,7 +1604,9 @@
                 gram = ext[C:]
             elif not pure:
                 ops.conv_wgrad(u.src, g4, 1, 1, 1, 0, ldw=cv.ldw, out=P, workspace=ws, splits=sp)
-            ops.bn3_algebra_dw(P, wb, c, gram, csum_a2, coef, cv._g2d)
+            if self.bn3_dw_flush and isinstance(ws, ops.WgradChain):
+                ws.flush()
+            ops.wgrad_then(ws, lambda: ops.bn3_algebra_dw(P, wb, c, gram, csum_a2, coef, cv._g2d))
         if self.wg_stream is None:
             finish_dw(self.a3_ws, 0)
         else:
@@ -1688,6 +1703,7 @@
         fh, fw, fc = self.final.shape[1], self.final.shape[2], self.final.shape[3]
         if net._head_only:
             if self.wg_stream is not None:
+                self._flush_wgrads()
                 for st in self.wg_streams:
                     torch.cuda.current_stream().wait_stream(st)
                 if self.ds_stream is not None:
@@ -1697,7 +1713,9 @@
             return
         g = self._gbuf(("g", self.final.shape), self.final.shape)
         ops.avgpool_backward(dpooled.view(n, D), fh * fw, out=g.view(n, fh * fw, fc))
-        if reducer is not None:
+        reducing = reducer is not None and (reducer.world > 1 or reducer.force)
+        if reducing:
+            self._flush_wgrads()
             reducer.gradients_ready_from(offs["head"])
         for bi in range(len(self.blocks) - 1, -1, -1):
             b = self.blocks[bi]
@@ -1773,7 +1791,8 @@
             else:
                 self._unit_backward(first, d, first.y, dgrad_out=gin, dgrad_res=g, par=par, fuse_up=up_in)
             g = gin
-            if reducer is not None:
+            if reducing:
+                self._flush_wgrads()
                 reducer.gradients_ready_from(offs["blocks"][bi])
         u = self.stem
         g_pooled = g
@@ -1814,6 +1833,7 @@
         else:
             self._unit_backward(u, g, u.y, need_dgrad=False)
         if self.wg_stream is not None:
+            self._flush_wgrads()
             for st in self.wg_streams:
                 torch.cuda.current_stream().wait_stream(st)
             if self.ds_stream is not None:
diff --git a/include/iif_amd.h b/include/iif_amd.h
--- a/include/iif_amd.h
+++ b/include/iif_amd.h
@@ -253,6 +253,20 @@
 int iif_wgrad1x1_stacked(const void* x, const void* dy, const void* dy2, int64_t m, int cs, int cd1, int cd2,
                          int ldw, float* out, void* workspace, int64_t workspace_bytes, int splits,
                          void* stream);
+
+typedef struct iif_slab_job {
+    const float* ws;
+    float* dst;
+    int64_t slab;
+    int32_t splits, rows, ldw, K;
+} iif_slab_job;
+int iif_conv_wgrad_deferred(const iif_conv_desc* d, const void* x, const void* dy, float* dw,
+                            void* workspace, int64_t workspace_bytes, int splits, void* stream,
+                            const iif_slab_job* carry, iif_slab_job* pending);
+int iif_wgrad1x1_stacked_deferred(const void* x, const void* dy, const void* dy2, int64_t m, int cs, int cd1, int cd2,
+                                  int ldw, float* out, void* workspace, int64_t workspace_bytes, int splits,
+                                  void* stream, const iif_slab_job* carry, iif_slab_job* pending);
+int iif_wgrad_flush(void* stream, const iif_slab_job* job);
 
 #define IIF_WGRAD_REGSTAGE 0
 #define IIF_WGRAD_DMA 1
```

Result: slower. 15020 (-1.9%).
